# johannesulf/TabCorr

Hardware: AMD Instinct MI355X
Metric: predict_calls_per_sec (higher is better)
Workload: dtype f64; 1 GPU; BASELINE configs[1]: Zheng07 predict(), synthetic auto table 50 mass bins x {cen,sat} (G=100, P=5050), 19 rp bins, n_gauss_prim=10, batch of 10000 draws per GPU per step, draws and results resident in HBM; n_tables=1, gather=none, gather_payload=ngal + xi (160 B per draw), gather_every_steps=32, lanes=4, rccl_ranks=0

## Files before the change

include/tabcorr_amd_testing.h:

```cpp
#ifndef TABCORR_AMD_TESTING_H
#define TABCORR_AMD_TESTING_H

#include "tabcorr_amd.h"

#ifdef __cplusplus
extern "C" {
#endif

int tc_debug_fastmath(int kind, int64_t n, const double* x, double* y);

int tc_debug_central_series(int n_gauss, double log_min, double log_max, double dist_index,
                            int64_t n, const double* log_m_min, const double* sigma,
                            double* series, double* nodes, int32_t* terms);

int tc_debug_satellite_series(int n_gauss, double log_min, double log_max, double dist_index,
                              int64_t n, const double* log_m0, const double* log_m1,
                              const double* alpha, double* series, double* nodes,
                              int32_t* terms);

int tc_plan_debug(int mode, int n_bins, const uint8_t* is_central, int n_chunks,
                  int64_t* n_entries, int32_t* entry_pair, int32_t* entry_chunk,
                  int32_t* entry_class);

int tc_debug_quad_schedule(int n_bins, int n_central, int by_type, int n_tiles, int n_rtiles,
                           int n_tables, int separate, int max_waves, int min_units,
                           int order ,
                           int* n_waves, int* n_runs, int* n_slabs, int64_t* units_min,
                           int64_t* units_max);
int tc_debug_triangle_parts(int n_rb, int n_parts, int32_t* rb0, int32_t* cb0, int32_t* count);
int tc_debug_node_groups(int n_bins, int n_central, const double* log_min,
                         const double* log_max, int32_t* begin, int32_t* member,
                         int* n_groups, int* n_central_groups);
int tc_debug_quad_emulate(int n_bins, int n_r, const double* tpcf_matrix,
                          const uint8_t* is_central, int by_type, int separate,
                          const double* densities, int64_t ldb, int64_t n_draws,
                          int max_waves, int min_units, int order, double* out);

int tc_debug_trace(tc_table* table, uint64_t* out, int64_t capacity, int64_t* n_blocks);
int tc_debug_wave_trace(tc_table* table, uint64_t* out, int64_t capacity,
                        int64_t* n_waves);
int tc_debug_resident_ticks(tc_table* table, uint64_t* out, int64_t capacity, int64_t* n_blocks);
int tc_debug_ensemble_stamps(tc_table* table, uint64_t* out);
#ifdef __cplusplus
}
#endif

#endif
```

tabcorr_amd/_lib.py:

```python

import ctypes
import os

import numpy as np

HERE = os.path.dirname(os.path.abspath(__file__))
LIBRARY = os.path.join(HERE, 'libtabcorr_hip.so')

TC_OK = 0
TC_ERR_INVALID = 1
TC_ERR_HIP = 2
TC_ERR_UNSUPPORTED = 3
TC_ERR_RCCL = 4

MODE = {'auto': 0, 'cross': 1}
DTYPE_F64 = 0
DTYPE_F32 = 1

FLAG_SEPARATE_GAL_TYPE = 1
FLAG_MODULATE_WITH_CENOCC = 2
FLAG_ASSEMBIAS = 4
FLAG_LEAUTHAUD11 = 16

UNIQUE_ID_BYTES = 128

c_double_p = ctypes.POINTER(ctypes.c_double)
c_int_p = ctypes.POINTER(ctypes.c_int)
c_int32_p = ctypes.POINTER(ctypes.c_int32)
c_int64_p = ctypes.POINTER(ctypes.c_int64)
c_uint8_p = ctypes.POINTER(ctypes.c_uint8)
c_float_p = ctypes.POINTER(ctypes.c_float)
c_void_pp = ctypes.POINTER(ctypes.c_void_p)

SIGNATURES = {
    'tc_device_count': [c_int_p],
    'tc_set_device': [ctypes.c_int],
    'tc_get_device': [c_int_p],
    'tc_runtime_version': [c_int_p],
    'tc_device_name': [ctypes.c_char_p, ctypes.c_size_t],
    'tc_device_synchronize': [],
    'tc_device_malloc': [c_void_pp, ctypes.c_size_t],
    'tc_device_free': [ctypes.c_void_p],
    'tc_memcpy_h2d': [ctypes.c_void_p, ctypes.c_void_p, ctypes.c_size_t],
    'tc_memcpy_d2h': [ctypes.c_void_p, ctypes.c_void_p, ctypes.c_size_t],
    'tc_host_alloc': [c_void_pp, ctypes.c_size_t],
    'tc_host_free': [ctypes.c_void_p],
    'tc_host_register': [ctypes.c_void_p, ctypes.c_size_t],
    'tc_host_unregister': [ctypes.c_void_p],
    'tc_host_is_pinned': [ctypes.c_void_p, ctypes.c_size_t, c_int_p],
    'tc_gauss_legendre': [ctypes.c_int, c_double_p, c_double_p],
    'tc_debug_fastmath': [ctypes.c_int, ctypes.c_int64, c_double_p,
                          c_double_p],
    'tc_pair_indices': [ctypes.c_int, c_int32_p, c_int32_p, c_int32_p],
    'tc_spline_interpolation_matrix': [ctypes.c_int, c_double_p, c_double_p],
    'tc_plan_debug': [ctypes.c_int, ctypes.c_int, c_uint8_p, ctypes.c_int,
                      c_int64_p, c_int32_p, c_int32_p, c_int32_p],
    'tc_debug_triangle_parts': [ctypes.c_int, ctypes.c_int, c_int_p, c_int_p, c_int_p],
    'tc_debug_central_series': [ctypes.c_int, ctypes.c_double, ctypes.c_double, ctypes.c_double,
                                ctypes.c_int64, c_double_p, c_double_p, c_double_p, c_double_p,
                                c_int32_p],
    'tc_debug_satellite_series': [ctypes.c_int, ctypes.c_double, ctypes.c_double,
                                  ctypes.c_double, ctypes.c_int64, c_double_p, c_double_p,
                                  c_double_p, c_double_p, c_double_p, c_int32_p],
    'tc_debug_node_groups': [ctypes.c_int, ctypes.c_int, c_double_p, c_double_p,
                             c_int32_p, c_int32_p, c_int_p, c_int_p],
    'tc_debug_quad_schedule': [ctypes.c_int] * 10 + [c_int_p, c_int_p, c_int_p,
                                                     c_int64_p, c_int64_p],
    'tc_debug_quad_emulate': [ctypes.c_int, ctypes.c_int, c_double_p, c_uint8_p,
                              ctypes.c_int, ctypes.c_int, c_double_p,
                              ctypes.c_int64, ctypes.c_int64, ctypes.c_int,
                              ctypes.c_int, ctypes.c_int, c_double_p],
    'tc_table_create': [
        ctypes.c_int, ctypes.c_int, ctypes.c_int, ctypes.c_int64,
        ctypes.c_void_p, ctypes.c_int, c_double_p, c_double_p, c_double_p,
        c_double_p, c_double_p, c_uint8_p, ctypes.c_int, c_void_pp],
    'tc_table_destroy': [ctypes.c_void_p],
    'tc_table_autotune_result': [ctypes.c_void_p, ctypes.c_uint, ctypes.c_int, c_int_p,
                                 c_int64_p, c_int_p, c_float_p],
    'tc_table_batch_invariant': [ctypes.c_void_p, ctypes.c_int, ctypes.c_uint, c_int_p],
    'tc_set_copy_threads': [ctypes.c_int, ctypes.c_int],
    'tc_table_resident_stats': [ctypes.c_void_p, c_int64_p, c_int64_p, c_int64_p, c_int_p],
    'tc_table_synchronize': [ctypes.c_void_p],
    'tc_table_info': [ctypes.c_void_p, c_int_p, c_int_p, c_int_p, c_int64_p,
                      c_int_p, c_int64_p],
    'tc_mean_occupation_zheng07_batch': [
        ctypes.c_void_p, c_double_p, ctypes.c_int, ctypes.c_int64,
        ctypes.c_int, ctypes.c_uint, c_double_p],
    'tc_predict_zheng07_batch': [
        ctypes.c_void_p, c_double_p, ctypes.c_int, ctypes.c_int64,
        ctypes.c_int, ctypes.c_uint, c_double_p, c_double_p],
    'tc_predict_zheng07_batch_device': [
        ctypes.c_void_p, ctypes.c_void_p, ctypes.c_int, ctypes.c_int64,
        ctypes.c_int, ctypes.c_uint, ctypes.c_void_p, ctypes.c_void_p],
    'tc_chi2_zheng07_batch': [
        ctypes.c_void_p, c_double_p, ctypes.c_int, ctypes.c_int64,
        ctypes.c_int, ctypes.c_uint, c_double_p, c_double_p, c_double_p,
        c_double_p],
    'tc_chi2_zheng07_batch_device': [
        ctypes.c_void_p, ctypes.c_void_p, ctypes.c_int, ctypes.c_int64,
        ctypes.c_int, ctypes.c_uint, c_double_p, c_double_p, ctypes.c_void_p,
        ctypes.c_void_p],
    'tc_predict_zheng07_many': [
        ctypes.c_void_p, c_double_p, ctypes.c_int, ctypes.c_int,
        ctypes.c_int, ctypes.c_uint, c_double_p, c_double_p],
    'tc_predict_zheng07_joint': [
        ctypes.POINTER(ctypes.c_void_p), ctypes.c_int, c_double_p, ctypes.c_int,
        ctypes.c_int, ctypes.c_uint, c_double_p, ctypes.POINTER(c_double_p)],
    'tc_predict_zheng07_batch_async': [
        ctypes.c_void_p, c_double_p, ctypes.c_int, ctypes.c_int64,
        ctypes.c_int, ctypes.c_uint, c_double_p, c_double_p, c_int64_p],
    'tc_chi2_zheng07_batch_async': [
        ctypes.c_void_p, c_double_p, ctypes.c_int, ctypes.c_int64,
        ctypes.c_int, ctypes.c_uint, c_double_p, c_double_p, c_double_p,
        c_double_p, c_int64_p],
    'tc_table_wait': [ctypes.c_void_p, ctypes.c_int64],
    'tc_table_query': [ctypes.c_void_p, ctypes.c_int64, c_int_p],
    'tc_interp_predict_zheng07_batch_async': [
        ctypes.c_void_p, c_double_p, ctypes.c_int, c_double_p,
        ctypes.c_int64, ctypes.c_int, ctypes.c_uint, c_double_p, c_double_p,
        c_int64_p],
    'tc_interp_chi2_zheng07_batch_async': [
        ctypes.c_void_p, c_double_p, ctypes.c_int, c_double_p,
        ctypes.c_int64, ctypes.c_int, ctypes.c_uint, c_double_p, c_double_p,
        c_double_p, c_double_p, c_int64_p],
    'tc_interp_wait': [ctypes.c_void_p, ctypes.c_int64],
    'tc_interp_query': [ctypes.c_void_p, ctypes.c_int64, c_int_p],
    'tc_predict_occupation_batch': [
        ctypes.c_void_p, c_double_p, ctypes.c_int64, ctypes.c_uint,
        c_double_p, c_double_p],
    'tc_interp_create': [c_void_pp, ctypes.c_int, ctypes.c_int, c_double_p,
                         c_void_pp],
    'tc_interp_destroy': [ctypes.c_void_p],
    'tc_interp_synchronize': [ctypes.c_void_p],
    'tc_interp_axis': [ctypes.c_void_p, ctypes.c_int, c_int_p, c_double_p,
                       ctypes.c_int],
    'tc_interp_predict_zheng07_batch': [
        ctypes.c_void_p, c_double_p, ctypes.c_int, c_double_p,
        ctypes.c_int64, ctypes.c_int, ctypes.c_uint, c_double_p, c_double_p],
    'tc_interp_predict_zheng07_batch_device': [
        ctypes.c_void_p, ctypes.c_void_p, ctypes.c_int, ctypes.c_void_p,
        ctypes.c_int64, ctypes.c_int, ctypes.c_uint, ctypes.c_void_p,
        ctypes.c_void_p],
    'tc_interp_chi2_zheng07_batch': [
        ctypes.c_void_p, c_double_p, ctypes.c_int, c_double_p,
        ctypes.c_int64, ctypes.c_int, ctypes.c_uint, c_double_p, c_double_p,
        c_double_p, c_double_p],
    'tc_interp_chi2_zheng07_batch_device': [
        ctypes.c_void_p, ctypes.c_void_p, ctypes.c_int, ctypes.c_void_p,
        ctypes.c_int64, ctypes.c_int, ctypes.c_uint, c_double_p, c_double_p,
        ctypes.c_void_p, ctypes.c_void_p],
    'tc_table_set_option': [ctypes.c_void_p, ctypes.c_char_p, ctypes.c_int],
    'tc_table_timer_begin': [ctypes.c_void_p, ctypes.c_int],
    'tc_table_timer_end': [ctypes.c_void_p, c_float_p],
    'tc_table_kernel_time': [ctypes.c_void_p, c_int_p, c_float_p],
    'tc_debug_trace': [ctypes.c_void_p, ctypes.POINTER(ctypes.c_uint64),
                       ctypes.c_int64, c_int64_p],
    'tc_debug_wave_trace': [ctypes.c_void_p, ctypes.POINTER(ctypes.c_uint64),
                            ctypes.c_int64, c_int64_p],
    'tc_debug_resident_ticks': [ctypes.c_void_p, ctypes.POINTER(ctypes.c_uint64),
                                ctypes.c_int64, c_int64_p],
    'tc_debug_ensemble_stamps': [ctypes.c_void_p,
                                 ctypes.POINTER(ctypes.c_uint64)],
    'tc_table_last_launch': [ctypes.c_void_p, c_int_p, c_int_p, c_int_p,
                             c_int_p],
    'tc_pair_count_rppi': [c_double_p, ctypes.c_int64, c_double_p,
                           ctypes.c_int64, c_double_p, c_double_p, ctypes.c_int,
                           ctypes.c_double, ctypes.c_int,
                           ctypes.POINTER(ctypes.c_uint64)],
    'tc_pair_count_smu': [c_double_p, ctypes.c_int64, c_double_p,
                          ctypes.c_int64, c_double_p, c_double_p, ctypes.c_int,
                          ctypes.c_int, ctypes.POINTER(ctypes.c_uint64)],
    'tc_pair_count_rppi_labelled': [c_double_p, c_int32_p, ctypes.c_int64,
                                    c_double_p, c_int32_p, ctypes.c_int64,
                                    ctypes.c_int, c_double_p, c_double_p,
                                    ctypes.c_int, ctypes.c_double,
                                    ctypes.POINTER(ctypes.c_uint64)],
    'tc_pair_count_smu_labelled': [c_double_p, c_int32_p, ctypes.c_int64,
                                   c_double_p, c_int32_p, ctypes.c_int64,
                                   ctypes.c_int, c_double_p, c_double_p,
                                   ctypes.c_int, ctypes.c_int,
                                   ctypes.POINTER(ctypes.c_uint64)],
    'tc_mass_in_cylinders': [c_double_p, ctypes.c_int64, c_double_p,
                             ctypes.c_int64, c_double_p, c_double_p, c_double_p,
                             ctypes.c_int, c_double_p],
    'tc_comm_unique_id': [ctypes.c_void_p],
    'tc_comm_create': [ctypes.c_void_p, ctypes.c_int, ctypes.c_int,
                       c_void_pp],
    'tc_comm_destroy': [ctypes.c_void_p],
    'tc_comm_gather': [ctypes.c_void_p, ctypes.c_void_p, ctypes.c_void_p,
                       ctypes.c_void_p, ctypes.c_int64, ctypes.c_int,
                       ctypes.c_int],
    'tc_comm_release': [ctypes.c_void_p, ctypes.c_void_p, ctypes.c_int],
    'tc_comm_gather_interp': [ctypes.c_void_p, ctypes.c_void_p, ctypes.c_void_p,
                              ctypes.c_void_p, ctypes.c_int64, ctypes.c_int,
                              ctypes.c_int],
    'tc_comm_release_interp': [ctypes.c_void_p, ctypes.c_void_p,
                               ctypes.c_int],
    'tc_comm_barrier': [ctypes.c_void_p],
    'tc_comm_synchronize': [ctypes.c_void_p],
}

_lib = None


class TabCorrHipError(RuntimeError):
    """The HIP backend failed (no device, launch error, RCCL error)."""


def load():
    global _lib
    if _lib is not None:
        return _lib
    library = os.environ.get('TABCORR_AMD_LIBRARY') or LIBRARY
    if not os.path.exists(library):
        raise TabCorrHipError(
            'libtabcorr_hip.so is missing: build it with '
            '`python -m tabcorr_amd.build` (needs hipcc). There is no CPU '
            'fallback.')
    mode = os.RTLD_NOW | os.RTLD_LOCAL | getattr(os, 'RTLD_DEEPBIND', 0)
    lib = ctypes.CDLL(library, mode=mode)
    lib.tc_last_error.restype = ctypes.c_char_p
    lib.tc_last_error.argtypes = []
    for name, argtypes in SIGNATURES.items():
        function = getattr(lib, name)
        function.restype = ctypes.c_int
        function.argtypes = argtypes
    _lib = lib
    return lib


def check(status):
    if status == TC_OK:
        return
    message = load().tc_last_error().decode(errors='replace')
    if status == TC_ERR_INVALID:
        raise ValueError(message)
    if status == TC_ERR_UNSUPPORTED:
        raise NotImplementedError(message)
    raise TabCorrHipError(message)


def as_double_p(array):
    try:
        return ctypes.byref(ctypes.c_double.from_buffer(array))
    except (TypeError, ValueError, BufferError):
        return array.ctypes.data_as(c_double_p)


def device_count():
    lib = load()
    count = ctypes.c_int(0)
    status = lib.tc_device_count(ctypes.byref(count))
    if status != TC_OK:
        return 0
    return count.value


def require_device():
    lib = load()
    count = ctypes.c_int(0)
    check(lib.tc_device_count(ctypes.byref(count)))
    if count.value < 1:
        raise TabCorrHipError('no HIP device found; tabcorr_amd has no CPU '
                              'fallback')
    return count.value


def runtime_version():
    version = ctypes.c_int(0)
    check(load().tc_runtime_version(ctypes.byref(version)))
    return version.value


def device_name():
    buffer = ctypes.create_string_buffer(256)
    check(load().tc_device_name(buffer, 256))
    return buffer.value.decode()


def contiguous(array, dtype=np.float64):
    return np.ascontiguousarray(array, dtype=dtype)
```

tabcorr_amd/csrc/inst_fused.hip:

```cpp
#include "inst_fused.h"

namespace tc {
namespace host {

int launch_fused_instance(const FusedInstance& in, int device, int n_u, dim3 grid, dim3 block,
                       int lds, hipStream_t stream, hipEvent_t k0, hipEvent_t k1,
                       const tc::FusedArgs& fa) {
  const bool assembias = in.assembias, modulate = in.modulate;
  if (in.draws == 40) return launch_fused_instance_40(in, TC_FUSED_ARGS);
  if (in.draws == 32) return launch_fused_instance_32(in, TC_FUSED_ARGS);
  if (in.waves == 16) return launch_fused_instance_16(in, TC_FUSED_ARGS);
#define TC_FUSED(NG, AB, MO, LE) launch_fused<NG, AB, MO, LE, 8>(TC_FUSED_ARGS)
#define TC_FUSED_GROUPED(AB, MO) launch_fused<10, AB, MO, false, 8, 64, true>(TC_FUSED_ARGS)
  if (in.grouped)
    return assembias ? (modulate ? TC_FUSED_GROUPED(true, true) : TC_FUSED_GROUPED(true, false))
                     : (modulate ? TC_FUSED_GROUPED(false, true) : TC_FUSED_GROUPED(false, false));
  if (in.leauthaud) return modulate ? TC_FUSED(0, false, true, true) : TC_FUSED(0, false, false, true);
  if (in.n_gauss != 10) return TC_FUSED(0, false, false, false);
  if (!assembias && !modulate && in.defer == 2)
    return launch_fused<10, false, false, false, 8, 64, false, 2>(TC_FUSED_ARGS);
  if (!assembias && !modulate && in.defer == 1)
    return launch_fused<10, false, false, false, 8, 64, false, 1>(TC_FUSED_ARGS);
  if (!assembias && !modulate) return TC_FUSED(10, false, false, false);
  if (!assembias) return TC_FUSED(10, false, true, false);
  if (!modulate) return TC_FUSED(10, true, false, false);
  return TC_FUSED(10, true, true, false);
#undef TC_FUSED
#undef TC_FUSED_GROUPED
}

}
}
```

tabcorr_amd/csrc/internal.h:

```cpp
#pragma once

#include <hip/hip_runtime.h>
#include <hip/hip_ext.h>

#include <algorithm>
#include <chrono>
#include <cmath>
#include <cstdarg>
#include <cstdio>
#include <cstdlib>
#include <cstring>
#include <map>
#include <memory>
#include <string>
#include <utility>
#include <vector>

#include "../../include/tabcorr_amd.h"
#include "../../include/tabcorr_amd_testing.h"
#include "fastmath.h"
#include "hostmath.h"
#include "kernel_args.h"

namespace tc {
// ... 80 lines not shown
  return fallback;
}
inline size_t stage_limit() {
  static const size_t limit = (size_t)env_int_early("TC_STAGE_LIMIT_MB", 1) << 20;
  return limit;
}

inline size_t zero_copy_limit() {
  static const size_t limit = (size_t)env_int_early("TC_ZERO_COPY_KB", 512) << 10;
  return limit;
}

int create_lane_streams(int count, hipStream_t* streams);

struct SingleWorkspace {
  PinnedBuffer buffer;
  unsigned long long epoch = 0;
  int jobs = 0, blocks = 0;
  size_t partial_offset = 0, theta_offset = 0, done_offset = 0;
  int prepare(int n_jobs, int n_blocks, int rt, int extra_doubles);
  double* ngal() const { return (double*)buffer.ptr; }
  double* partial() const { return (double*)buffer.ptr + partial_offset; }
  double* theta() const { return (double*)buffer.ptr + theta_offset; }
  unsigned long long* done() const {
    return (unsigned long long*)((double*)buffer.ptr + done_offset);
  }
};

template <typename T>
int upload(const std::vector<T>& host, void** device) {
  size_t bytes = std::max<size_t>(1, host.size()) * sizeof(T);
  TC_HIP(hipMalloc(device, bytes));
  if (!host.empty())
    TC_HIP(hipMemcpy(*device, host.data(), host.size() * sizeof(T),
                     hipMemcpyHostToDevice));
  return TC_OK;
}

struct DeviceChunking {
  tc::Chunking host;
  void* chunks = nullptr;
  void* groups = nullptr;
};

struct Quadrature {
  int n_gauss = 0;
  void* log_m = nullptr;
  void* m = nullptr;
  void* weight = nullptr;
  void* group_log_m = nullptr;
  void* group_m = nullptr;
  void* group_weight = nullptr;
  void* series = nullptr;
  void* series_thr = nullptr;
  void* group_series = nullptr;
  void* group_series_thr = nullptr;
  void* sat_series = nullptr;
  void* sat_series_thr = nullptr;
  void* group_sat_series = nullptr;
  void* group_sat_series_thr = nullptr;
  void* cen_records = nullptr;
  void* sat_records = nullptr;
  void* group_records = nullptr;
};

struct DeviceQuadSchedule {
  int n_waves = 0;
  int n_slabs = 0;
  int n_groups = 0;
  int n_runs = 0;
  void* runs = nullptr;
  void* wave_runs = nullptr;
  void* wave_head = nullptr;
  void* group_begin = nullptr;
  void* merge_range = nullptr;
  void* merges = nullptr;
  int lds_bytes = 0;
};

struct QuadTable {
  tc::QuadLayout layout;
  void* d_table = nullptr;
  void* d_comps = nullptr;
  bool finite = false;
  size_t rtile_bytes = 0;
  size_t bytes = 0;
  std::map<std::vector<int64_t>, std::unique_ptr<DeviceQuadSchedule>> schedules;
  void release();
  void drop_schedules();
};

struct CrossFused {
  bool tried = false;
  int rows = 0;
  int n_tables = 0;
  void* d_rows = nullptr;
  void* d_chunk_group = nullptr;
  void* d_chunk_block = nullptr;
  void* d_bin_operand = nullptr;
  std::vector<int32_t> chunk_group_host;
  int n_chunks = 0, n_central_chunks = 0;
  void release() {
    if (d_rows != nullptr) (void)hipFree(d_rows);
    if (d_chunk_group != nullptr) (void)hipFree(d_chunk_group);
    if (d_chunk_block != nullptr) (void)hipFree(d_chunk_block);
    if (d_bin_operand != nullptr) (void)hipFree(d_bin_operand);
    d_rows = d_chunk_group = d_chunk_block = d_bin_operand = nullptr;
    rows = 0;
    tried = false;
  }
};

inline int env_int(const char* name, int fallback) {
#ifdef TC_DEVELOPER_KNOBS
  const char* value = getenv(name);
  if (value == nullptr || *value == 0) return fallback;
  return atoi(value);
#else
  (void)name;
  return fallback;
#endif
}

struct Tuning {
  int lanes = 4;
  int pipeline = 1;
  int single_draw = 1;
  int many_blocks = 256;
  int single_round = 1;
  int poll_done = 1;
  int quad_waves = 0;
  int quad_waves_f32 = 3;
  int quad_merge = 1;
  int quad_order = -1;
  int prio_occ = 2, prio_contract = 1, prio_finalize = 3;
  int finalize_threads = 0;
  int finalize_row_blocks = 0;
  int occ_splits = 0;
  int occ_per_cu = 4;
  int n_groups = 0, n_waves = 0, lds_min = 0, min_chunk_entries = 32;
  int k_splits = 0;
  int trace = 0;
  int autotune_after = 0;
  int sync_chunks = 0;
  int sync_form = 32;
  int sync_stagger = 10;
  int sync_direct_out = 2;
  int async_direct_in = 1;
  int async_direct_out = 2;
  int series = -1;
  int cross_defer = 1;
  int fused_defer = 2;
  int fused_sat_cap = 6;
  int cross_wide_min_draws = 4096;
  int cross_target = 160;
  int resident_aperture = 1;
  int cross_min_draws = 192;
  int fused = 1;
  int fused_min_draws = 0;
  int fused_max_draws = 30720;
  int fused_waves = 0;
  int fused_draws = 0;
  int fused_spread = 1, fused_spread_min = 8192, fused_spread_rounds = 1;
  int prio_fused = 1, prio_fused_occ = 2, prio_fused_out = 3;
  int deterministic = 0;
  int skip_occ = 0, skip_finalize = 0;
  void load() {
    fused = env_int("TC_FUSED", fused);
    fused_min_draws = env_int("TC_FUSED_MIN_DRAWS", fused_min_draws);
    fused_max_draws = env_int("TC_FUSED_MAX_DRAWS", fused_max_draws);
    prio_fused = env_int("TC_PRIO_FUSED", prio_fused);
    prio_fused_occ = env_int("TC_PRIO_FUSED_OCC", prio_fused_occ);
    prio_fused_out = env_int("TC_PRIO_FUSED_OUT", prio_fused_out);
    lanes = env_int("TC_LANES", lanes);
    pipeline = env_int("TC_PIPELINE", pipeline);
    single_draw = env_int("TC_SINGLE_DRAW", single_draw);
    quad_waves = env_int("TC_QUAD_WAVES", quad_waves);
    quad_waves_f32 = env_int("TC_QUAD_WAVES_F32", quad_waves_f32);
    quad_merge = env_int("TC_QUAD_MERGE", quad_merge);
    prio_occ = env_int("TC_PRIO_O", prio_occ);
    prio_contract = env_int("TC_PRIO_C", prio_contract);
    prio_finalize = env_int("TC_PRIO_F", prio_finalize);
    finalize_threads = env_int("TC_FINALIZE_THREADS", finalize_threads);
    finalize_row_blocks = env_int("TC_FINALIZE_ROW_BLOCKS", finalize_row_blocks);
    occ_splits = env_int("TC_OCC_SPLITS", occ_splits);
    occ_per_cu = env_int("TC_OCC_PER_CU", occ_per_cu);
    n_groups = env_int("TC_NGROUPS", n_groups);
    n_waves = env_int("TC_NWAVES", n_waves);
    lds_min = env_int("TC_LDS_MIN", lds_min);
    min_chunk_entries = env_int("TC_MIN_CHUNK_ENTRIES", min_chunk_entries);
    k_splits = env_int("TC_KSPLITS", k_splits);
    trace = env_int("TC_TRACE", trace);
    skip_occ = env_int("TC_SKIP_OCC", skip_occ);
    skip_finalize = env_int("TC_SKIP_FINALIZE", skip_finalize);
  }
};

}
}

struct AutoChoice {
  static constexpr int kSizes = 9;
  static constexpr int64_t size(int i) { return (int64_t)256 << i; }
  int form[kSizes] = {};
  float us[kSizes][3] = {};
  int form_for(int64_t n_draws) const {
    if (n_draws <= size(0)) return form[0];
    if (n_draws >= size(kSizes - 1)) return form[kSizes - 1];
    int i = 0;
    while (size(i + 1) < n_draws) ++i;
    const double w = (double)(n_draws - size(i)) / (double)(size(i + 1) - size(i));
    static const int shape[3] = {0, 64, 32};
    int best = 0;
    double best_us = (1.0 - w) * us[i][0] + w * us[i + 1][0];
    for (int k = 1; k < 3; ++k) {
      if (us[i][k] <= 0.0f || us[i + 1][k] <= 0.0f) continue;
      const double value = (1.0 - w) * us[i][k] + w * us[i + 1][k];
      if (value < (best == 0 ? 0.98 : 1.0) * best_us) {
        best_us = value;
        best = shape[k];
      }
    }
    return best;
  }
};

struct tc_table {
  int device = 0;
  int mode = 0;
  int n_bins = 0;
  int n_r = 0;
  int64_t n_pairs = 0;
  int compute_dtype = TC_DTYPE_F64;
  bool legacy = false;
  tc::Plan plan;
  int rt = 0;
  int n_rtiles = 0;
  hipStream_t stream = nullptr;
  hipEvent_t ev_begin = nullptr, ev_end = nullptr;

  std::vector<double> n_h, log_min, log_max, percentile, dist_index;

  void* d_table = nullptr;
  size_t table_bytes = 0;
  void* d_n_h = nullptr;
  void* d_percentile = nullptr;
  void* d_perm = nullptr;
  tc::NodeGroups node_groups;
  void* d_group_begin = nullptr;
  void* d_group_member = nullptr;
  void* d_group_n_h = nullptr;
  void* d_group_percentile = nullptr;
  bool grouped = false;
  void* d_math_table = nullptr;
  void* d_pos_ij = nullptr;
  void* d_pos_off = nullptr;
  std::vector<double> cross_host;
  tc::host::CrossFused cross_fused, cross_fused_wide;
  int sync_cross_target = 0;
  std::vector<hipEvent_t> chunk_events;
  bool sync_spread = false;
  bool quad = false;
  tc::QuadTiling quad_tiling;
  tc::host::QuadTable quad_by_type, quad_total;
  int n_cus = 256;
  int n_xcds = 8;
  tc::host::Tuning tuning;
  std::map<unsigned, AutoChoice> autotuned;
  std::map<unsigned, int> pipelined_calls;
  bool autotuning = false;
  std::map<int, tc::host::Quadrature> quadrature;
  std::map<std::pair<int, int>, std::unique_ptr<tc::host::DeviceChunking>> chunkings;
  std::map<int64_t, tc::host::DeviceChunking*> choices;

  struct Lane {
    hipStream_t stream = nullptr;
    hipEvent_t finished = nullptr;
    tc::host::DeviceBuffer nbuf, ngal2, partial;
    tc::host::DeviceBuffer nbuf32;
    tc::host::DeviceBuffer xi;
    tc::host::DeviceBuffer in_theta, out;
    tc::host::DeviceBuffer cross_counters;
    int ngal_parts = 1;
  };
  static constexpr int kMaxLanes = 8;
  Lane lanes[kMaxLanes];
  int n_lanes = 2;
  int prev = -1;
  int cur = 0;
  int force_lane = -1;
  int async_lane = -1;
  bool chain = false;
  struct Ticket {
    hipEvent_t done = nullptr;
    int64_t id = -1;
  };
  static constexpr int kMaxTickets = 64;
  Ticket tickets[kMaxTickets];
  int64_t next_ticket = 0;
  const double* fuse_chi2_data = nullptr;
  double* fuse_chi2_out = nullptr;
  bool chi2_fused = false;
  uint64_t device_calls = 0;
  tc::host::DeviceBuffer theta, out_ngal, out_xi, occupation, trace, wave_trace;
  tc::host::DeviceBuffer chi2_data;
  std::vector<double> chi2_host;
  size_t wave_trace_count = 0;
  tc::host::PinnedBuffer h_in, h_out;
  tc::host::SingleWorkspace single_ws;
  struct Resident {
    int enabled = 0;
    int idle_us = 2000;
    int auto_mode = 1;
    int auto_idle_us = 250, auto_gap_us = 300, auto_streak_min = 8, auto_backoff_calls = 4096;
    int auto_streak = 0, auto_backoff = 0, auto_window = 0, auto_relaunches = 0;
    int auto_failures = 0;
    int inject_failures = 0;
    long long auto_last_ns = 0;
    bool auto_serving = false;
    unsigned long long relaunches = 0;
    int running_idle_us = 0;
    int poll_waves = 1;
    bool running = false;
    unsigned long long launch_id = 0;
    hipStream_t stream = nullptr;
    tc::host::PinnedBuffer mailbox;
    tc::host::DeviceBuffer single_aperture;
    bool single_aperture_decided = false;
    tc::host::SingleWorkspace ws;
    int n_theta = 0, n_gauss = 0, blocks = 0;
    unsigned flags = 0;
    bool ensemble = false;
    unsigned long long ens_epoch = 0;
    int ens_grid = 0;
    tc::host::PinnedBuffer ens_mailbox, ens_out;
    tc::host::DeviceBuffer ens_device;
    tc::host::DeviceBuffer ens_aperture;
    unsigned long long ens_host_ns[3] = {0, 0, 0};
    int wait_us = 20000;
    int min_walkers = 24;
    int ens_failures = 0;
    bool ens_disabled = false;
  } resident;
  size_t trace_blocks = 0;
  size_t trace_launches = 0;

  bool profile_kernels = false;
  int profile_every = 1;
  size_t profile_launches = 0;
  std::vector<std::pair<hipEvent_t, hipEvent_t>> kernel_events;
  size_t kernel_events_used = 0;
  int last_workgroups = 0, last_waves = 0, last_splits = 0, last_lds = 0;
};

namespace tc {
namespace host {

constexpr size_t kDirectOutBytes = 256 * 1024;
constexpr size_t kSyncDirectOutBytes = 1024 * 1024;
constexpr int kMaxLdsBytes = 160 * 1024;
constexpr int64_t kMaxSlab = 1 << 18;

int get_quadrature(tc_table* t, int n_gauss, Quadrature** out);
tc::GroupArgs group_args(const tc_table* t, const Quadrature& q);
int get_chunking(tc_table* t, int n_chunks, int waves, DeviceChunking** out);
int lds_bytes_for(const Chunking& chunking, int rt, int elem = 8);
int wave_slots(const tc_table* t, bool interp);
int blocks_per_cu(int lds_bytes, int waves, int slots);
int choose_chunking(tc_table* t, int64_t n_draws, int tables_per_block, DeviceChunking** out,
                    int* lds_bytes);
int launch_contract_rt(int rt, dim3 grid, dim3 block, int lds, hipStream_t stream,
                       const ContractArgs& args, hipEvent_t start = nullptr,
                       hipEvent_t stop = nullptr);
int set_lds_limit_rt(int rt, int lds);
int launch_contract_f32(dim3 grid, dim3 block, int lds, hipStream_t stream,
                        const ContractArgs& args, hipEvent_t start = nullptr,
                        hipEvent_t stop = nullptr);
int run_occupation(tc_table* t, const double* theta_device, int n_theta, int64_t n_draws,
                   int64_t ldb, int n_gauss, unsigned flags, double* occupation_device,
                   DeviceBuffer* nbuf = nullptr, DeviceBuffer* ngal2 = nullptr,
                   hipStream_t stream = nullptr, int* ngal_parts = nullptr,
                   DeviceBuffer* nbuf32 = nullptr);
int run_contraction(tc_table* t, int64_t n_draws, int64_t ldb, unsigned flags,
                    double* ngal_device, double* xi_device);
bool fused_eligible(const tc_table* t, int64_t n_draws, int n_gauss, unsigned flags);
bool batch_invariant_form(tc_table* t, int n_gauss, unsigned flags);
int fused_dens_rows(const tc_table* t, bool separate);
int fused_lds_bytes(const tc_table* t, bool separate, int waves, int draws);
int fused_waves(const tc_table* t, bool separate, unsigned flags);
int series_mask(const tc_table* t);
bool fused_half_tiles(const tc_table* t, bool separate, int64_t n_draws, int n_gauss,
                      unsigned flags);
bool fused_wide_tables(const tc_table* t, bool separate, int n_gauss, unsigned flags);
bool fused_spread_eligible(const tc_table* t, int64_t n_draws, int n_gauss, unsigned flags);
int run_fused(tc_table* t, const double* theta_device, int n_theta, int64_t n_draws, int n_gauss,
              unsigned flags, double* ngal_device, double* xi_device);
int check_predict_args(const tc_table* t, const void* theta, int n_theta, int64_t n_draws,
                       int n_gauss, unsigned flags);
int build_cross_fused(tc_table* const* tables, int n_tables, CrossFused* cf, bool wide = false);
CrossFused* choose_cross_fused(tc_table* const* tables, int n_tables, CrossFused* narrow,
                               CrossFused* wide, int64_t n_draws, unsigned flags, int* status);
bool cross_fused_eligible(const tc_table* t0, const CrossFused& cf, int64_t n_draws, int n_gauss,
                          unsigned flags, bool alone);
int run_cross_fused(tc_table* t0, const CrossFused& cf, const tc::CrossFusedArgs* interp,
                    const double* theta_device, int n_theta, int64_t n_draws, unsigned flags,
                    double* ngal_device, double* xi_device, hipStream_t stream,
                    DeviceBuffer* partial, DeviceBuffer* counters);
int launch_finalize(const FinalizeArgs& args, const Tuning& tuning, hipStream_t stream);
int build_quad_table(tc_table* t, bool by_type, const void* matrix, int matrix_dtype,
                     QuadTable* out);
int get_quad_schedule(tc_table* t, QuadTable* q, int64_t n_tiles, int n_tables, bool separate,
                      DeviceQuadSchedule** out);
int launch_contract_quad(int n_u, bool interp, const QuadArgs& args, int lds_bytes,
                         hipStream_t stream, hipEvent_t start, hipEvent_t stop);
int launch_finalize_quad(const FinalizeQuadArgs& args, const Tuning& tuning, hipStream_t stream,
                         bool f32 = false);
int launch_contract_quad_f32_interp(int n_u, const tc::QuadArgs& args, int lds_bytes,
                                    hipStream_t stream, hipEvent_t start, hipEvent_t stop);
int launch_contract_quad_f32(int n_u, const QuadArgs& args, int lds_bytes, hipStream_t stream,
                             hipEvent_t start, hipEvent_t stop);
hipStream_t interp_stream(tc_interp* interp);
int interp_join_lanes(tc_interp* interp, hipStream_t stream);
int interp_lanes_wait(tc_interp* interp, hipEvent_t event);
int next_kernel_events(tc_table* t, hipEvent_t* start, hipEvent_t* stop);
int64_t max_slab(const tc_table* t);
bool single_draw_eligible(const tc_table* t, int64_t n_draws, int n_gauss, unsigned flags);
constexpr int kSingleMaxBlocks = 64;
constexpr int kSingleMaxWalkers = 64;
inline int64_t many_walkers_limit() {
  static const int64_t limit =
      std::min<int64_t>(kSingleMaxWalkers, env_int_early("TC_MANY_WALKERS", 64));
  return limit;
}
int resident_predict(tc_table* t, const double* theta, int n_theta, int n_gauss, unsigned flags,
                     double* ngal, double* xi);
int resident_post(tc_table* t, const double* theta, int n_theta, int n_gauss, unsigned flags);
int resident_collect(tc_table* t, const double* theta, int n_theta, int n_gauss, unsigned flags,
                     double* ngal, double* xi);
int resident_stop(tc_table* t);
bool resident_eligible(const tc_table* t, int n_gauss);
bool other_resident_running(const tc_table* t);
bool ensemble_eligible(const tc_table* t, int64_t n_walkers, int n_gauss, unsigned flags);
int ensemble_predict(tc_table* t, const double* theta, int n_theta, int n_walkers, int n_gauss,
                     unsigned flags, double* ngal, double* xi);
int launch_single_draw(tc_table* t, const double* theta, int n_theta, int n_walkers, int n_gauss,
                       unsigned flags, SingleWorkspace* ws, hipStream_t stream);
int wait_single_done(SingleWorkspace* ws, hipStream_t stream, bool poll = true);
void combine_single_draw(const tc_table* t, const SingleWorkspace& ws, int walker, double* ngal,
                         double* xi);
int single_draw_blocks(const tc_table* t);
int launch_single_draw_tables(tc_table* t0, const SingleArgs& prepared, int n_tables,
                              int blocks_per_table, hipStream_t stream);
int launch_interp_coef(const InterpArgs& args, hipStream_t stream);
int launch_occ_from_array(tc_table* t, const double* occupation_device, int64_t n_draws,
                          int64_t ldb, double* nbuf, double* ngal2, hipStream_t stream);
int launch_chi2(const double* xi, int64_t n_draws, int n_r, const double* data,
                const double* precision, double* chi2, hipStream_t stream);

int launch_occupation(const tc::OccArgs& oa, unsigned flags, int n_gauss, bool grouped,
                      int64_t grid_blocks, hipStream_t stream);
int launch_occ_from_array_kernel(const double* occupation_device, int64_t n_draws, int64_t ldb,
                                 int n_bins, int n_central, const double* n_h,
                                 const int32_t* perm, double* nbuf, double* ngal2, float* nbuf32,
                                 hipStream_t stream);
struct FusedInstance {
  int n_gauss = 10;
  bool assembias = false, modulate = false, leauthaud = false, grouped = false;
  int waves = 8, draws = 64;
  int defer = 0;
};
int launch_fused_instance(const FusedInstance& instance, int device, int n_u, dim3 grid,
                          dim3 block, int lds, hipStream_t stream, hipEvent_t k0, hipEvent_t k1,
                          const tc::FusedArgs& fa);
int launch_cross_instance(bool assembias, bool modulate, bool defer, int device, int rows,
                          dim3 grid, dim3 block, int lds, hipStream_t stream, hipEvent_t k0,
                          hipEvent_t k1, const tc::CrossFusedArgs& ca);
int launch_single_kernel(int blocks, hipStream_t stream, const tc::SingleArgs& sa);
int launch_resident_kernel(int blocks, hipStream_t stream, const tc::SingleArgs& sa);
int launch_ensemble_kernel(int device, int grid, int lds_bytes, hipStream_t stream,
                           const tc::EnsembleArgs& ea);

int copy_in(PinnedBuffer* stage, void* device, const void* host, size_t bytes,
            hipStream_t stream);
int copy_out(PinnedBuffer* stage, double* ngal, size_t ngal_count, const void* d_ngal,
             double* xi, size_t xi_count, const void* d_xi, hipStream_t stream);

}
}
```

tabcorr_amd/csrc/kernel_args.h:

```cpp
#pragma once

#include <cstdint>

#include "hostmath.h"

namespace tc {

constexpr int kLanes = 64;
constexpr unsigned kFlagSeparate = 1u;
constexpr unsigned kFlagModulate = 2u;
constexpr unsigned kFlagAssembias = 4u;
constexpr int kOccWaves = 4;
constexpr int kF32Block = 8;
constexpr int kF64Block = 8;
constexpr int kF32Tile = 32;
constexpr int kFinalizeRows = 32;
constexpr int kMaxInterpDim = 8;
constexpr int kMaxInterpAxis = 32;

struct GroupArgs {
  const int32_t* begin;
  const int32_t* member;
  const double* log_m;
  const double* m;
// ... 107 lines not shown
  int dens_stride;
  double* dens;
  unsigned long long* flag_a;
  double* partial;
  unsigned long long* flag_b;
  unsigned long long* callword;
  const unsigned long long* mailbox;
  int direct;
  double* out;
  unsigned long long* done;
  unsigned long long* exited;
  unsigned long long epoch;
  unsigned long long launch_id;
  unsigned long long idle_ticks, life_ticks, call_ticks;
  int lds_area, lds_dens, lds_t, lds_ij;
  int skip;
};
constexpr int kEnsembleThreads = 512;
constexpr int kEnsembleMaxWalkers = 256;
constexpr int kEnsembleDensPad = 65;

struct ContractArgs {
  const double* nbuf;
  int64_t ldb;
  const void* table;
  int64_t n_positions;
  const Chunk* chunks;
  const Group* groups;
  int mode;
  int n_central;
  int r_stride;
  int n_tiles;
  int xcd_map;
  int n_slabs;
  const int32_t* pos_ij;
  const int32_t* pos_off;
  unsigned long long* trace;
  unsigned long long* wave_trace;
  double* partial;
  int n_tables;
  int k_splits;
  const double* const* tables;
  const double* const* nbufs;
  const int32_t* table_class;
  const double* coef;
};

constexpr int kQuadMaxU = 5;
constexpr int kQuadTile = 32;
constexpr int kQuadWavesPerBlock = 4;

struct QuadCompArgs {
  int32_t triangular;
  int32_t i_bin0;
  int32_t j_bin0;
  int32_t n_cb;
  uint32_t unit_base;
  int32_t pad[3];
};

constexpr int kQuadTileF32 = 64;
constexpr int kQuadMaxUF32 = 4;

struct QuadArgs {
  const float* nbuf32;
  const double* nbuf;
  const double* const* nbufs;
  const float* const* nbufs32;
  int64_t ldb;
  int n_bins;
  const void* table;
  const double* const* tables;
  const int32_t* table_class;
  const double* coef;
  uint32_t rtile_bytes;
  const QuadRun* runs;
  const QuadCompArgs* comps;
  const int32_t* wave_runs;
  const int32_t* wave_head;
  int n_waves;
  int priority;
  void* partial;
  const int32_t* merge_range;
  const int32_t* merges;
  unsigned long long* stamps;
};

struct FinalizeQuadArgs {
  const void* partial;
  const int32_t* group_begin;
  const double* ngal_part;
  int n_ngal_parts;
  int n_rtiles;
  int r_per_tile;
  int rt;
  int groups_per_rtile;
  int n_comp;
  int n_r;
  int mode;
  int priority;
  int64_t ldb;
  int64_t n_draws;
  double* ngal;
  double* xi;
  const double* chi2_data;
  double* chi2;
};

constexpr int kFusedWaves = 8;
constexpr int kFusedMaxParts = 8;

struct FusedArgs {
  const double* theta;
  int n_theta;
  int n_bins;
  int n_central;
  int n_gauss;
  int dens_rows;
  int part_rb0[kFusedMaxParts];
  int part_cb0[kFusedMaxParts];
  int part_count[kFusedMaxParts];
  int part_triangular[kFusedMaxParts];
  int part_n_cb[kFusedMaxParts];
  int part_i_row0[kFusedMaxParts];
  int part_j_row0[kFusedMaxParts];
  int part_unit_base[kFusedMaxParts];
  int separate;
  int n_r;
  int priority;
  int64_t n_draws;
  const double* log_m;
  const double* m;
  const double* weight;
  const double* n_h;
  const double* percentile;
  double split;
  const double* math_table;
  const void* table;
  uint32_t table_bytes;
  double* ngal;
  double* xi;
  const double* chi2_data;
  double* chi2;
  int n_groups;
  int n_central_groups;
  GroupArgs group;
  const double* series;
  const int32_t* series_thr;
  const double* sat_series;
  const int32_t* sat_series_thr;
  int sat_cap;
  const double* sat_records;
  const double* cen_records;
};

constexpr int kCrossWaves = 8;
constexpr int kCrossChunkBins = 48;
constexpr int kCrossMaxRows = 128;
constexpr int kCrossTableDoubles = 2306;
constexpr int kCrossSmallRows = 16, kCrossSmallChunk = 8;
constexpr int kCrossMaxSplits = 8;
constexpr int cross_small_lds_doubles(int n_comp) {
  return kCrossTableDoubles + kCrossWaves * kCrossSmallChunk * kLanes +
         n_comp * kCrossSmallRows * kLanes;
}
constexpr int cross_buffer_doubles(int rows) {
  return 2 * kCrossChunkBins * kLanes > rows * kLanes ? 2 * kCrossChunkBins * kLanes
                                                      : rows * kLanes;
}

struct CrossFusedArgs {
  const double* theta;
  int n_theta;
  int64_t n_draws;
  int n_bins;
  int n_groups, n_central_groups;
  GroupArgs group;
  const double* math_table;
  const double* rows;
  const int32_t* chunk_block;
  int defer;
  int lds_bitmap, lds_list;
  const int32_t* bin_operand;
  const int32_t* chunk_group;
  int n_chunks, n_central_chunks;
  int n_tables;
  int n_r;
  int separate;
  int row_stride;
  int cen_waves;
  int n_splits;
  int split_all[kCrossMaxSplits + 1], split_cen[kCrossMaxSplits + 1],
      split_sat[kCrossMaxSplits + 1];
  double* partial;
  int* counters;
  int lds_res0;
  int lds_tile;
  int interp;
  int n_dim;
  int n_axis[kMaxInterpDim];
  int axis_offset[kMaxInterpDim];
  int a_offset[kMaxInterpDim];
  const double* xp;
  const double* a;
  const int32_t* table_node;
  const double* x;
  double split;
  int priority;
  double* ngal;
  double* xi;
  const double* chi2_data;
  double* chi2;
};

struct FinalizeArgs {
  const double* partial;
  const Group* groups;
  const double* ngal_part;
  int n_ngal_parts;
  int n_groups;
  int k_splits;
  int n_comp;
  int r_stride;
  int n_r;
  int mode;
  int64_t ldb;
  int64_t n_draws;
  double* ngal;
  double* xi;
};

struct InterpArgs {
  int n_dim;
  int n_tables;
  int n_classes;
  int mode;
  int separate;
  int n_axis[kMaxInterpDim];
  int axis_offset[kMaxInterpDim];
  int a_offset[kMaxInterpDim];
  const double* xp;
  const double* a;
  const int32_t* table_node;
  const int32_t* table_class;
  const double* x;
  const double* const* ngal_parts;
  int n_ngal_parts;
  int64_t ldb;
  int64_t n_draws;
  double* coef;
  double* ngal;
};

}
```

tabcorr_amd/csrc/kernels.hip.h:

```cpp
#pragma once

#include <hip/hip_runtime.h>

#include <cstdint>
#include <utility>

#include "fastmath.h"
#include "hostmath.h"
#include "kernel_args.h"
#include "series.h"

#ifdef TC_DEVELOPER_KNOBS
#define TC_TRACE(pointer) ((pointer) != nullptr)
#else
#define TC_TRACE(pointer) false
#endif

namespace tc {

static_assert(sizeof(QuadRun) == 32 && sizeof(QuadCompArgs) == 32, "read as 8 x int32");

typedef const __attribute__((address_space(4))) double* sc_f64;
typedef const __attribute__((address_space(4))) float* sc_f32;
typedef const __attribute__((address_space(4))) int32_t* sc_i32;
// ... 1669 lines not shown
          for (int v = 0; v < 4; ++v) F[u][s] = fmaf(D[u][s][v], e[v][s], F[u][s]);
      ++rb;
      cb = 0;
    }
    if (slab != -1) {
      float* out = slab >= 0
                       ? (float*)a.partial + ((int64_t)slab * (4 * U) + kq) * kQuadTileF32 + 4 * c
                       : stage32 + ((-2 - slab) * (4 * U) + kq) * kQuadTileF32 + 4 * c;
#pragma unroll
      for (int u = 0; u < U; ++u) {
        const f32x4 value = {F[u][0], F[u][1], F[u][2], F[u][3]};
        *(f32x4*)(out + (4 * u) * kQuadTileF32) = value;
#pragma unroll
        for (int s = 0; s < 4; ++s) F[u][s] = 0.0f;
      }
    }
  }
  sc_i32 merge_range = (sc_i32)a.merge_range;
  const int merge_begin = merge_range[2 * blockIdx.x], merge_end = merge_range[2 * blockIdx.x + 1];
  if (merge_begin == merge_end) return;
  __syncthreads();
  sc_i32 merges = (sc_i32)a.merges;
  for (int e = merge_begin + wave_in_block; e < merge_end; e += kQuadWavesPerBlock) {
    const int slab = merges[4 * e], first = merges[4 * e + 1], n_slots = merges[4 * e + 2];
    float* out = (float*)a.partial + ((int64_t)slab * (4 * U) + kq) * kQuadTileF32 + 4 * c;
    const float* in = stage32 + (first * (4 * U) + kq) * kQuadTileF32 + 4 * c;
#pragma unroll
    for (int u = 0; u < U; ++u) {
      f32x4 sum = *(const f32x4*)(in + (4 * u) * kQuadTileF32);
      for (int s = 1; s < n_slots; ++s)
        sum += *(const f32x4*)(in + (s * (4 * U) + 4 * u) * kQuadTileF32);
      *(f32x4*)(out + (4 * u) * kQuadTileF32) = sum;
    }
  }
}

template <typename P, int TILE>
__global__ __launch_bounds__(1024) void finalize_quad_kernel(FinalizeQuadArgs a) {
  __shared__ double tile[kFinalizeRows][kLanes + 1];
  __shared__ double part_sum[16][kLanes];
  __shared__ double norm_inv[kLanes];
  __shared__ double chi2_lds[kFinalizeRows * (kFinalizeRows + 1)];
  set_priority(a.priority);
  if (a.chi2 != nullptr) {
    const int count = a.n_r * (a.n_r + 1);
    for (int idx = threadIdx.x; idx < count; idx += blockDim.x) chi2_lds[idx] = a.chi2_data[idx];
  }
  const int lane = threadIdx.x & 63;
  const int wave = __builtin_amdgcn_readfirstlane(threadIdx.x >> 6);
  const int64_t col = (int64_t)blockIdx.x * kLanes;
  const int64_t n_valid = a.n_draws - col < kLanes ? a.n_draws - col : kLanes;

  if (wave == 0 && a.ngal_part == nullptr) norm_inv[lane] = 1.0;
  if (wave == 0 && a.ngal_part != nullptr) {
    double n_cen = 0.0, n_sat = 0.0;
    for (int p = 0; p < a.n_ngal_parts; ++p) {
      n_cen += a.ngal_part[((int64_t)p * 2 + 0) * a.ldb + col + lane];
      n_sat += a.ngal_part[((int64_t)p * 2 + 1) * a.ldb + col + lane];
    }
    const double total = n_cen + n_sat;
    norm_inv[lane] = a.mode == 0 ? total * total : total;
    if (lane < n_valid && blockIdx.y == 0) {
      if (a.n_comp == 1) {
        a.ngal[col + lane] = total;
      } else {
        a.ngal[2 * (col + lane)] = n_cen;
        a.ngal[2 * (col + lane) + 1] = n_sat;
      }
    }
  }
  __syncthreads();
  const double norm = norm_inv[lane];
  const bool poisoned = a.n_comp > 1 && !(fabs(norm) <= 1.79769313486231570815e308);
  auto normalise = [&](double sum) { return poisoned ? __builtin_nan("") : sum / norm; };

  const int n_rows = a.n_comp * a.n_r;
  const int n_waves = blockDim.x >> 6;
  const int rows_per_block = (n_rows + gridDim.y - 1) / gridDim.y;
  const int row_begin = blockIdx.y * rows_per_block;
  const int row_end = row_begin + rows_per_block < n_rows ? row_begin + rows_per_block : n_rows;
  const int64_t tile32 = TILE == 32 ? (int64_t)blockIdx.x * 2 + (lane >> 5) : (int64_t)blockIdx.x;
  const int64_t slab_stride = (int64_t)a.rt * TILE;
  auto sum_slabs = [&](int row, int part, int parts) {
    const int comp = row / a.n_r, r = row % a.n_r;
    const int rtile = r / a.r_per_tile, r_local = r % a.r_per_tile;
    const int64_t group = (tile32 * a.n_rtiles + rtile) * a.groups_per_rtile +
                          (a.groups_per_rtile > 1 ? comp : 0);
    const int first = a.group_begin[group], count = a.group_begin[group + 1] - first;
    const int begin = first + (int)((int64_t)count * part / parts);
    const int end = first + (int)((int64_t)count * (part + 1) / parts);
    const P* src = (const P*)a.partial + ((int64_t)begin * a.rt + r_local) * TILE + (lane & (TILE - 1));
    double sum = 0.0;
    for (int s0 = begin; s0 < end; s0 += 8) {
      double v[8];
#pragma unroll
      for (int u = 0; u < 8; ++u)
        v[u] = s0 + u < end ? (double)src[(s0 - begin + u) * slab_stride] : 0.0;
#pragma unroll
      for (int u = 0; u < 8; ++u) sum += v[u];
    }
    return sum;
  };
  for (int row0 = row_begin; row0 < row_end; row0 += kFinalizeRows) {
    const int rows = row_end - row0 < kFinalizeRows ? row_end - row0 : kFinalizeRows;
    if (rows * 2 <= n_waves) {
      const int parts = n_waves / rows;
      const int rr = wave / parts, part = wave % parts;
      if (rr < rows) part_sum[wave][lane] = sum_slabs(row0 + rr, part, parts);
      __syncthreads();
      if (wave < rows) {
        double sum = 0.0;
        for (int p = 0; p < parts; ++p) sum += part_sum[wave * parts + p][lane];
        tile[wave][lane] = normalise(sum);
      }
    } else {
      for (int rr = wave; rr < rows; rr += n_waves)
        tile[rr][lane] = normalise(sum_slabs(row0 + rr, 0, 1));
    }
    __syncthreads();
    if (a.chi2 != nullptr) {
      const double* data = chi2_lds;
      const double* matrix = chi2_lds + rows;
      double part = 0.0;
      for (int i = wave; i < rows; i += n_waves) {
        double inner = 0.0;
        for (int j = 0; j < rows; ++j)
          inner = fma(matrix[i * rows + j], tile[j][lane] - data[j], inner);
        part = fma(tile[i][lane] - data[i], inner, part);
      }
      part_sum[wave][lane] = part;
      __syncthreads();
      if (wave == 0 && lane < n_valid) {
        double total = 0.0;
        for (int w = 0; w < n_waves; ++w) total += part_sum[w][lane];
        a.chi2[col + lane] = total;
      }
      __syncthreads();
      continue;
    }
    for (int idx = threadIdx.x; idx < rows * kLanes; idx += blockDim.x) {
      const int d = idx / rows, rr = idx % rows;
      if (d < n_valid) a.xi[(col + d) * (int64_t)n_rows + row0 + rr] = tile[rr][d];
    }
    __syncthreads();
  }
}

constexpr int fused_slot_doubles(int waves, int draws = 64) {
  return waves * 4 * kQuadMaxU * (draws == 40 ? 40 : kQuadTile);
}
__device__ __forceinline__ constexpr int dens40(int row, int draw) {
  return row * 40 + (draw & 3) * 10 + (draw >> 2);
}
constexpr int fused_scratch_doubles(int waves) { return fm::kTableDoubles + 2 * waves * kLanes; }
static_assert(kFusedWaves == 8 && kFusedMaxParts == 8, "8 or 16 waves: 4 or 8 parts per tile");
static_assert(20 * (kLanes + 1) + 20 * 21 <= fm::kTableDoubles,
              "results tile + likelihood data in the place of the math table");

template <int UU, int DL>
__device__ __forceinline__ void fused_quad_pass(__amdgpu_buffer_rsrc_t rs_t, unsigned off_a,
                                                unsigned unit_bytes, const double* dens_b,
                                                const double* dens_e, int rb, int cb, int left,
                                                bool triangular, int n_cb, unsigned unit_base,
                                                double (&F)[2][2]) {
  unsigned ua = (unit_base + (unsigned)(triangular ? rb * (rb + 1) / 2 + cb : rb * n_cb + cb)) *
                unit_bytes;
  f64x2 t0, t1, b0, b1;
  f64x4 D[UU][2];
  auto fetch = [&](f64x2& t, f64x2& b, int column) {
    t = buffer_load16<0>(rs_t, off_a, ua);
    b = *(const f64x2*)(dens_b + 4 * column * DL);
    ua += unit_bytes;
  };
  auto mma = [&](const f64x2& t, const f64x2& b, bool first) {
    if (first) {
      const f64x4 zero = {0.0, 0.0, 0.0, 0.0};
#pragma unroll
      for (int u = 0; u < UU; ++u) {
        const double av = u ? t.y : t.x;
        D[u][0] = __builtin_amdgcn_mfma_f64_16x16x4f64(av, b.x, zero, 0, 0, 0);
        D[u][1] = __builtin_amdgcn_mfma_f64_16x16x4f64(av, b.y, zero, 0, 0, 0);
      }
    } else {
#pragma unroll
      for (int u = 0; u < UU; ++u) {
        const double av = u ? t.y : t.x;
        D[u][0] = __builtin_amdgcn_mfma_f64_16x16x4f64(av, b.x, D[u][0], 0, 0, 0);
        D[u][1] = __builtin_amdgcn_mfma_f64_16x16x4f64(av, b.y, D[u][1], 0, 0, 0);
      }
    }
  };
  fetch(t0, b0, cb);
  while (left > 0) {
    const int row_length = triangular ? rb + 1 : n_cb;
    const int n = row_length - cb < left ? row_length - cb : left;
    left -= n;
    f64x2 e[4];
#pragma unroll
    for (int v = 0; v < 4; ++v) e[v] = *(const f64x2*)(dens_e + (4 * rb + v) * DL);
    fetch(t1, b1, n > 1 ? cb + 1 : 0);
    __builtin_amdgcn_sched_barrier(0);
    mma(t0, b0, true);
    __builtin_amdgcn_sched_barrier(0);
    int t = 1;
    for (; t + 1 < n; t += 2) {
      fetch(t0, b0, cb + t + 1);
      __builtin_amdgcn_sched_barrier(0);
      mma(t1, b1, false);
      __builtin_amdgcn_sched_barrier(0);
      fetch(t1, b1, t + 2 < n ? cb + t + 2 : 0);
      __builtin_amdgcn_sched_barrier(0);
      mma(t0, b0, false);
      __builtin_amdgcn_sched_barrier(0);
    }
    if (t < n) {
      fetch(t0, b0, 0);
      __builtin_amdgcn_sched_barrier(0);
      mma(t1, b1, false);
      __builtin_amdgcn_sched_barrier(0);
    } else {
      t0 = t1;
      b0 = b1;
    }
#pragma unroll
    for (int u = 0; u < UU; ++u)
#pragma unroll
      for (int v = 0; v < 4; ++v) {
        F[u][0] = fma(D[u][0][v], e[v].x, F[u][0]);
        F[u][1] = fma(D[u][1][v], e[v].y, F[u][1]);
      }
    ++rb;
    cb = 0;
  }
}

__device__ __forceinline__ int wave_prefix_sum(int value) {
  auto shifted = [](int x, auto control, auto rows) {
    return __builtin_amdgcn_update_dpp(0, x, decltype(control)::value, decltype(rows)::value, 0xf,
                                       false);
  };
  typedef std::integral_constant<int, 0xf> all_rows;
  value += shifted(value, std::integral_constant<int, 0x111>(), all_rows());
  value += shifted(value, std::integral_constant<int, 0x112>(), all_rows());
  value += shifted(value, std::integral_constant<int, 0x114>(), all_rows());
  value += shifted(value, std::integral_constant<int, 0x118>(), all_rows());
  value += shifted(value, std::integral_constant<int, 0x142>(), std::integral_constant<int, 0xa>());
  value += shifted(value, std::integral_constant<int, 0x143>(), std::integral_constant<int, 0xc>());
  return value;
}

__device__ __forceinline__ double fused_quad_rows40(double select, double value, double sums) {
  return __builtin_amdgcn_mfma_f64_4x4x4f64(select, value, sums, 0, 0, 0);
}

template <int S0, int NS>
__device__ __forceinline__ void fused_quad_pass40(__amdgpu_buffer_rsrc_t rs_t, unsigned off_a,
                                                  unsigned unit_bytes, const double* dens_b,
                                                  const double* dens_e, int rb, int cb, int left,
                                                  bool triangular, int n_cb, unsigned unit_base,
                                                  double (&F)[NS][10]) {
  unsigned ua = (unit_base + (unsigned)(triangular ? rb * (rb + 1) / 2 + cb : rb * n_cb + cb)) *
                unit_bytes;
  double ta[2][NS];
  f64x2 tb[2][5];
  double D[NS][10];
  auto fetch = [&](int set, int column) {
#pragma unroll
    for (int s = 0; s < NS; ++s) {
      constexpr int kPairBytes = 1024;
      const int sub = S0 + s;
      const bool first_of_pair = (sub & 1) == 0 && s + 1 < NS;
      const bool second_of_pair = (sub & 1) == 1 && s >= 1;
      if (first_of_pair) {
        const f64x2 word = __builtin_bit_cast(
            f64x2, __builtin_amdgcn_raw_buffer_load_b128(rs_t, off_a + (sub / 2) * kPairBytes, ua,
                                                         0));
        ta[set][s] = word.x;
        ta[set][s + 1 < NS ? s + 1 : s] = word.y;
      } else if (!second_of_pair) {
        ta[set][s] = __builtin_bit_cast(
            double, __builtin_amdgcn_raw_buffer_load_b64(
                        rs_t, off_a + (sub / 2) * kPairBytes + (sub & 1) * 8, ua, 0));
      }
    }
#pragma unroll
    for (int q = 0; q < 5; ++q) tb[set][q] = *(const f64x2*)(dens_b + 4 * column * 40 + 2 * q);
    ua += unit_bytes;
  };
  auto mma = [&](int set, bool first) {
    if (first) {
#pragma unroll
      for (int q = 0; q < 5; ++q)
#pragma unroll
        for (int s = 0; s < NS; ++s) {
          const double av = ta[set][s];
          D[s][2 * q] = __builtin_amdgcn_mfma_f64_4x4x4f64(av, tb[set][q].x, 0.0, 0, 0, 0);
          D[s][2 * q + 1] = __builtin_amdgcn_mfma_f64_4x4x4f64(av, tb[set][q].y, 0.0, 0, 0, 0);
        }
    } else {
#pragma unroll
      for (int q = 0; q < 5; ++q)
#pragma unroll
        for (int s = 0; s < NS; ++s) {
          const double av = ta[set][s];
          D[s][2 * q] = __builtin_amdgcn_mfma_f64_4x4x4f64(av, tb[set][q].x, D[s][2 * q], 0, 0, 0);
          D[s][2 * q + 1] =
              __builtin_amdgcn_mfma_f64_4x4x4f64(av, tb[set][q].y, D[s][2 * q + 1], 0, 0, 0);
        }
    }
  };
  fetch(0, cb);
  while (left > 0) {
    const int row_length = triangular ? rb + 1 : n_cb;
    const int n = row_length - cb < left ? row_length - cb : left;
    left -= n;
    f64x2 e[5];
#pragma unroll
    for (int q = 0; q < 5; ++q) e[q] = *(const f64x2*)(dens_e + 4 * rb * 40 + 2 * q);
    int t = 0;
    if (n > 1) {
      fetch(1, cb + 1);
      mma(0, true);
      fetch(0, 2 < n ? cb + 2 : 0);
      mma(1, false);
      t = 2;
    }
    for (; t + 1 < n; t += 2) {
      fetch(1, cb + t + 1);
      mma(0, false);
      fetch(0, t + 2 < n ? cb + t + 2 : 0);
      mma(1, false);
    }
    if (t < n) {
      fetch(1, 0);
      if (t == 0) mma(0, true); else mma(0, false);
#pragma unroll
      for (int s = 0; s < NS; ++s) ta[0][s] = ta[1][s];
#pragma unroll
      for (int q = 0; q < 5; ++q) tb[0][q] = tb[1][q];
    }
#pragma unroll
    for (int q = 0; q < 5; ++q)
#pragma unroll
      for (int s = 0; s < NS; ++s) {
        F[s][2 * q] = fma(D[s][2 * q], e[q].x, F[s][2 * q]);
        F[s][2 * q + 1] = fma(D[s][2 * q + 1], e[q].y, F[s][2 * q + 1]);
      }
    ++rb;
    cb = 0;
  }
}

template <int NGAUSS, int U, bool ASSEMBIAS, bool MODULATE, bool LEAUTHAUD = false,
          int W = kFusedWaves, int DL = 64, bool GROUPED = false, int SATDEFER = 0>
__global__ __launch_bounds__(64 * W, DL == 40 ? 2 : W == 8 ? (SATDEFER == 2 ? 4 : 2) : 1) void predict_fused_kernel(
    FusedArgs a) {
  static_assert(!SATDEFER || (NGAUSS == 10 && !ASSEMBIAS && !MODULATE && !LEAUTHAUD && DL != 32 &&
                              !GROUPED), "deferred pairs");
  static_assert(!GROUPED || (NGAUSS == 10 && !LEAUTHAUD), "groups of bins: Zheng07, ten nodes");
  static_assert((DL == 64 && (W == 8 || W == 16)) || ((DL == 32 || DL == 40) && W == 8),
                "workgroup shape");
  static_assert(DL == 64 || NGAUSS == 10 || LEAUTHAUD, "32 / 40 draws: ten nodes per bin");
  static_assert(DL != 40 || (!ASSEMBIAS && !MODULATE && !LEAUTHAUD && !GROUPED), "latency form");
  constexpr int PARTS = DL == 40 ? W : W * 32 / DL;
  static_assert(!LEAUTHAUD || (NGAUSS == 0 && !ASSEMBIAS), "Leauthaud11: any n_gauss, undecorated");
  constexpr int UP = (U + 1) / 2;
  extern __shared__ __attribute__((aligned(16))) double fused_lds[];
  constexpr int kSlotDoubles = fused_slot_doubles(W, DL);
  const int region_b = a.dens_rows * DL > kSlotDoubles ? a.dens_rows * DL : kSlotDoubles;
  double* dens = fused_lds;
  double* table = fused_lds + region_b;
  double(*red)[W][kLanes] = (double(*)[W][kLanes])(table + fm::kTableDoubles);
  const fm::Consts kc = fm::make_consts();
#ifdef TC_DEVELOPER_KNOBS
  const int skip = (a.priority >> 8) & 3;
  const int n_bins_occ = (skip & 1) ? 0 : a.n_bins;
  unsigned long long* const stamps =
      ((a.priority >> 10) & 1) && a.chi2 == nullptr ? (unsigned long long*)a.chi2_data : nullptr;
  auto wave_stamp = [&](int which) {
    if (stamps != nullptr && (threadIdx.x & 63) == 0 && W == 8 && ((threadIdx.x >> 6) & 3) == 0)
      stamps[blockIdx.x * 32 + 16 + 8 * (threadIdx.x >> 8) + which] =
          __builtin_amdgcn_s_memrealtime();
  };
  auto stamp = [&](int which) {
    if (stamps != nullptr && threadIdx.x == 0)
      stamps[blockIdx.x * 32 + which] = __builtin_amdgcn_s_memrealtime();
  };
  if (skip & 1)
    for (int idx = threadIdx.x; idx < a.n_bins * DL; idx += blockDim.x) fused_lds[idx] = 1e-3;
#else
  constexpr int skip = 0;
  const int n_bins_occ = a.n_bins;
  auto stamp = [](int) {};
  auto wave_stamp = [](int) {};
#endif
  stamp(0);
  set_priority((a.priority >> 2) & 3);
  const int lane = threadIdx.x & 63;
  const int wave = __builtin_amdgcn_readfirstlane(threadIdx.x >> 6);
  const int n_gauss = NGAUSS > 0 ? NGAUSS : a.n_gauss;
  {
    typedef double __attribute__((ext_vector_type(2))) double2v;
    const int hi = fm::kTableDoubles / 2;
    const double2v* src = (const double2v*)a.math_table;
    double2v* dst = (double2v*)table;
    for (int i = threadIdx.x; i < hi; i += blockDim.x) dst[i] = src[i];
  }
  for (int idx = a.n_bins * DL + threadIdx.x; idx < a.dens_rows * DL; idx += blockDim.x)
    dens[idx] = 0.0;
  __syncthreads();
  stamp(1);

  const int draw = DL != 32 ? lane : (lane & 31);
  const int half = DL != 32 ? 0 : (lane >> 5);
  const bool live = DL != 40 || lane < 40;
  auto dens_at = [&](int row, int d) -> double& {
    return dens[DL == 40 ? dens40(row, d) : row * DL + d];
  };
  const int64_t col = (int64_t)blockIdx.x * DL;
  const int64_t b0 = col + draw;
  const int64_t b = b0 < a.n_draws ? b0 : a.n_draws - 1;
  double norm;
  {
    const double* th = a.theta + b * a.n_theta;
    LeauthaudDraw ld;
    if (LEAUTHAUD) ld = prepare_leauthaud(table, kc, th);
    const DrawSetup d =
        LEAUTHAUD ? prepare_draw(table, kc, 12.0, 1.0, 12.0, 13.0, 1.0, 0.0, 0.0)
                  : prepare_draw(table, kc, th[0], th[1], th[2], th[3], th[4],
                                 ASSEMBIAS ? th[5] : 0.0, ASSEMBIAS ? th[6] : 0.0);
    DrawParams dp;
    dp.log_m_min = d.log_m_min;
    dp.inv_sigma = d.inv_sigma;
    dp.m0 = d.m0;
    dp.log2_m1 = d.log2_m1;
    dp.sat_scale = d.sat_scale;
    dp.alpha = d.alpha;
    dp.a_cen = d.a_cen;
    dp.a_sat = d.a_sat;
    dp.bad = d.bad;
    dp.any_bad = __builtin_amdgcn_ballot_w64(dp.bad != 0) != 0;
    series_setup<MODULATE>(dp, (GROUPED ? a.group.series : a.series) != nullptr && DL != 32,
                           (GROUPED ? a.group.sat_series : a.sat_series) != nullptr && DL != 32);
    sc_f64 log_m = (sc_f64)a.log_m;
    sc_f64 mass = (sc_f64)a.m;
    sc_f64 weight = (sc_f64)a.weight;
    sc_f64 weight_sum = weight + a.n_bins * n_gauss;
    sc_f64 n_h = (sc_f64)a.n_h;
    sc_f64 percentile = (sc_f64)a.percentile;
    const double f1 = (1.0 - a.split) / a.split, f2 = a.split / (1.0 - a.split);
    double sum_cen = 0.0, sum_sat = 0.0;
    stamp(2);
    if (GROUPED) {
      sc_i32 group_begin = (sc_i32)a.group.begin;
      sc_f64 n_h_m = (sc_f64)a.group.n_h;
      const GroupConsts gq{(sc_f64)a.group.log_m, (sc_f64)a.group.m, (sc_f64)a.group.weight,
                           (sc_f64)a.group.weight + a.n_bins * 10, (sc_f64)a.group.percentile,
                           (sc_i32)a.group.member,
                             SeriesConsts{(sc_f64)a.group.series, (sc_i32)a.group.series_thr,
                                          (sc_f64)a.group.sat_series, (sc_i32)a.group.sat_series_thr}};
      for (int gr = wave; gr < a.n_groups; gr += W) {
        const bool central = gr < a.n_central_groups;
        auto emit = [&](int mi, int g, double acc) {
          const double value = acc * n_h_m[mi];
          if (half == 0) dens[g * DL + draw] = value;
          if (central) sum_cen += value; else sum_sat += value;
        };
        if (DL == 32)
          occ_group_zheng07_halves<ASSEMBIAS, MODULATE>(
              table, kc, gr, group_begin[gr], group_begin[gr + 1], central, half, a.group.log_m,
              a.group.m, a.group.weight, gq, a.split, dp, emit);
        else
          occ_group_zheng07<ASSEMBIAS, MODULATE>(table, kc, gr, group_begin[gr],
                                                 group_begin[gr + 1], central, gq, a.split, dp,
                                                 emit);
      }
    }
    unsigned mine = 0;
    for (int g = wave; g < (GROUPED ? 0 : n_bins_occ); g += W) {
      const bool central = g < a.n_central;
      const bool above = ASSEMBIAS ? percentile[g] > a.split : false;
      bool deferred = false;
      const double acc =
          SATDEFER == 2 && central
              ? occ_cen_record(table, kc,
                               (sc_f64)a.cen_records + g * series::cen_record::kStride, dp,
                               &deferred) :
          SATDEFER && !central && (SATDEFER == 2 || a.sat_cap == series::sat::kShortest)
              ? occ_sat_record(table, kc,
                               (sc_f64)a.sat_records + g * series::sat_record::kStride, dp,
                               &deferred) :
          DL == 32 && LEAUTHAUD
              ? occ_bin_leauthaud11_halves<MODULATE>(table, kc, g, central, half, a.log_m, a.m,
                                                     a.weight, ld)
          : DL == 32  ? occ_bin_zheng07_halves<ASSEMBIAS, MODULATE>(table, kc, g, central, above,
                                                                    half, a.log_m, a.m, a.weight,
                                                                    log_m, weight_sum, dp)
          : LEAUTHAUD ? occ_bin_leauthaud11<MODULATE>(table, kc, g, n_gauss, central, log_m, mass,
                                                      weight, ld)
                      : occ_bin_zheng07<NGAUSS, ASSEMBIAS, MODULATE>(
                            table, kc, g, n_gauss, central, above, log_m, mass, weight,
                            weight_sum, dp, f1, f2,
                            SeriesConsts{(sc_f64)a.series, (sc_i32)a.series_thr, (sc_f64)a.sat_series,
                              (sc_i32)a.sat_series_thr,
                              SATDEFER ? a.sat_cap : series::sat::kSteps - 1},
                            SATDEFER ? &deferred : nullptr);
      if (SATDEFER && deferred && live) mine |= 1u << ((g - wave) / W);
      const double value = acc * n_h[g];
      if (half == 0 && live) dens_at(g, draw) = value;
      if (central) sum_cen += value; else sum_sat += value;
    }
    wave_stamp(0);
    if (SATDEFER) {
      unsigned* list = (unsigned*)&red[1][wave][0];
      const int count = __builtin_popcount(mine);
      const int inclusive = wave_prefix_sum(count);
      const int total = __builtin_amdgcn_readlane(inclusive, 63);
      wave_stamp(2);
      for (int base = 0; base < total; base += 64) {
        {
          unsigned left = mine;
          int position = inclusive - count - base;
          while (__builtin_amdgcn_ballot_w64(left != 0) != 0) {
            if (left != 0) {
              const int j = __builtin_ctz(left);
              left &= left - 1;
              if (position >= 0 && position < 64) list[position] = ((unsigned)j << 6) | (unsigned)lane;
              ++position;
            }
          }
        }
        wave_stamp(3);
        const int n = total - base < 64 ? total - base : 64;
        const bool active = lane < n;
        const unsigned entry = list[active ? lane : 0];
        const int g = wave + W * (int)(entry >> 6), from = (int)(entry & 63);
        const double m0 = __shfl(dp.m0, from, 64);
        const double log2_m1 = __shfl(dp.log2_m1, from, 64);
        const double sat_scale = __shfl(dp.sat_scale, from, 64);
        const double alpha = __shfl(dp.alpha, from, 64);
        const int bad = __shfl(dp.bad, from, 64);
        double acc = 0.0;
        const bool cen_pair = SATDEFER == 2 && g < a.n_central;
        if (SATDEFER == 2 && __builtin_amdgcn_ballot_w64(active && cen_pair) != 0) {
          const double log_m_min = __shfl(dp.log_m_min, from, 64);
          const double inv_sigma = __shfl(dp.inv_sigma, from, 64);
          double sum = 0.0;
          bool tie = false;
#pragma unroll 1
          for (int k0 = 0; k0 < 10; k0 += 5) {
            double node[5], w[5];
#pragma unroll
            for (int k = 0; k < 5; ++k) {
              node[k] = a.log_m[g * 10 + k0 + k];
              w[k] = a.weight[g * 10 + k0 + k];
            }
#pragma unroll
            for (int k = 0; k < 5; ++k) {
              sum = fma(w[k], fm::erf_fast(table, kc, (node[k] - log_m_min) * inv_sigma), sum);
              tie = tie || node[k] == log_m_min;
            }
          }
          sum = fma(0.5, sum, 0.5 * a.weight[a.n_bins * 10 + g]);
          if ((bad & kBadCen) || ((bad & kTieCen) && tie)) sum = __builtin_nan("");
          if (cen_pair) acc = sum;
        }
        if (SATDEFER != 2 || __builtin_amdgcn_ballot_w64(active && !cen_pair) != 0) {
        double sat = 0.0;
#pragma unroll 1
        for (int k0 = 0; k0 < 10; k0 += 5) {
          double node[5], w[5];
#pragma unroll
          for (int k = 0; k < 5; ++k) {
            node[k] = a.m[g * 10 + k0 + k];
            w[k] = a.weight[g * 10 + k0 + k];
          }
#pragma unroll
          for (int k = 0; k < 5; ++k) {
            const double x = node[k] - m0;
            sat = fma(w[k],
                      fm::exp2_fast(table, kc,
                                    alpha * fm::log2_fast_offset(
                                                table, kc, x > 1e-300 ? x : 1e-300, log2_m1),
                                    x > 0.0),
                      sat);
          }
        }
        sat *= sat_scale;
        if (bad != 0) {
          if ((bad & kInfSat) && sat != 0.0) sat = __builtin_huge_val();
          if ((bad & kBadSat) && sat != 0.0) sat = __builtin_nan("");
        }
        if (!cen_pair) acc = sat;
        }
        if (active) dens_at(g, from) = acc * a.n_h[g];
        wave_stamp(4);
      }
      for (unsigned left = mine; __builtin_amdgcn_ballot_w64(left != 0) != 0;) {
        if (left != 0) {
          const int j = __builtin_ctz(left);
          left &= left - 1;
          const double value = dens_at(wave + W * j, draw);
          if (SATDEFER == 2 && wave + W * j < a.n_central) sum_cen += value;
          else sum_sat += value;
        }
      }
    }
    wave_stamp(1);
    stamp(3);
    red[0][wave][lane] = sum_cen;
    red[1][wave][lane] = sum_sat;
    __syncthreads();
    stamp(4);
    double n_cen = 0.0, n_sat = 0.0;
#pragma unroll
    for (int w = 0; w < W; ++w) {
      n_cen += red[0][w][lane];
      n_sat += red[1][w][lane];
    }
    const double total = (skip & 1) ? 1.0 : n_cen + n_sat;
    norm = total * total;
    if (wave == 0 && half == 0 && live && b0 < a.n_draws) {
      if (a.separate) {
        a.ngal[2 * b0] = n_cen;
        a.ngal[2 * b0 + 1] = n_sat;
      } else {
        a.ngal[b0] = total;
      }
    }
  }

  set_priority(a.priority & 3);
  const int c = lane & 15, kq = lane >> 4;
  double F[UP][2][2];
  constexpr int UA = DL == 40 ? (U > 3 ? 3 : U) : 1, UB = DL == 40 && U > 3 ? U - 3 : 1;
  double F40a[UA][10], F40b[UB][10];
  if (DL == 40) {
    const int part = wave;
    const unsigned off_a = ((lane & 0x30) | ((lane & 3) << 2) | ((lane >> 2) & 3)) * 16;
    const double* dens_b = dens + (a.part_j_row0[part] + (lane >> 4)) * 40 + (lane & 3) * 10;
    const double* dens_e = dens + (a.part_i_row0[part] + (lane >> 4)) * 40 + (lane & 3) * 10;
    const __amdgpu_buffer_rsrc_t rs_t =
        __builtin_amdgcn_make_buffer_rsrc((void*)a.table, 0, a.table_bytes, kBufferFlags);
    const int rb = a.part_rb0[part], cb = a.part_cb0[part], count = a.part_count[part];
    const bool triangular = a.part_triangular[part] != 0;
    const int n_cb = a.part_n_cb[part];
    const unsigned unit_base = (unsigned)a.part_unit_base[part];
#pragma unroll
    for (int s = 0; s < UA; ++s)
#pragma unroll
      for (int g = 0; g < 10; ++g) F40a[s][g] = 0.0;
#pragma unroll
    for (int s = 0; s < UB; ++s)
#pragma unroll
      for (int g = 0; g < 10; ++g) F40b[s][g] = 0.0;
#ifdef TC_DEVELOPER_KNOBS
    const unsigned unit_bytes = ((a.priority >> 12) & 1) ? 0u : UP * 1024u;
    const unsigned first_unit = ((a.priority >> 12) & 1) ? 0u : unit_base;
#else
    constexpr unsigned unit_bytes = UP * 1024u;
    const unsigned first_unit = unit_base;
#endif
    if (!(skip & 2))
    fused_quad_pass40<0, UA>(rs_t, off_a, unit_bytes, dens_b, dens_e, rb, cb, count, triangular,
                             n_cb, first_unit, F40a);
    if (U > 3 && !(skip & 2))
      fused_quad_pass40<(U > 3 ? 3 : 0), UB>(rs_t, off_a, unit_bytes, dens_b, dens_e, rb, cb,
                                             count, triangular, n_cb, first_unit, F40b);
  } else {
    const int sub = wave / PARTS, part = wave % PARTS;
    const unsigned off_a = lane * 16;
    const double* dens_b =
        dens + (a.part_j_row0[part] + kq) * DL + sub * kQuadTile + 2 * c;
    const double* dens_e = dens + a.part_i_row0[part] * DL + sub * kQuadTile + 2 * c;
    const __amdgpu_buffer_rsrc_t rs_t =
        __builtin_amdgcn_make_buffer_rsrc((void*)a.table, 0, a.table_bytes, kBufferFlags);
    const int rb = a.part_rb0[part], cb = a.part_cb0[part], count = a.part_count[part];
    const bool triangular = a.part_triangular[part] != 0;
    const int n_cb = a.part_n_cb[part];
    const unsigned unit_base = (unsigned)a.part_unit_base[part];
#pragma unroll
    for (int p = 0; p < UP; ++p) {
      F[p][0][0] = F[p][0][1] = F[p][1][0] = F[p][1][1] = 0.0;
      if (skip & 2) continue;
      if (2 * p + 1 < U)
        fused_quad_pass<2, DL>(rs_t, off_a + p * 1024, UP * 1024, dens_b, dens_e, rb, cb, count,
                               triangular, n_cb, unit_base, F[p]);
      else
        fused_quad_pass<1, DL>(rs_t, off_a + p * 1024, UP * 1024, dens_b, dens_e, rb, cb, count,
                               triangular, n_cb, unit_base, F[p]);
    }
  }
  stamp(5);
  __syncthreads();
  stamp(8);
  if (DL == 40) {
    const int q = lane >> 4;
    auto share = [&](int sub, int g) {
      return sub < UA ? F40a[sub < UA ? sub : 0][g] : F40b[sub >= UA ? sub - UA : 0][g];
    };
    double* out = dens + (wave * (4 * U) + ((lane >> 2) & 3)) * 40 + (lane & 3);
    if (((a.priority >> 11) & 1) && __builtin_amdgcn_ballot_w64(!(norm < 1e280)) == 0) {
      double select[4];
#pragma unroll
      for (int m = 0; m < 4; ++m) select[m] = (lane & 3) == m ? 1.0 : 0.0;
#pragma unroll
      for (int sub = 0; sub < U; ++sub)
#pragma unroll
        for (int t = 0; t < 3; ++t) {
          double sums = 0.0;
#pragma unroll
          for (int m = 0; m < (t < 2 ? 4 : 2); ++m)
            sums = fused_quad_rows40(select[m], share(sub, 4 * t + m), sums);
          if (t < 2 || q < 2) out[(4 * sub) * 40 + 16 * t + 4 * q] = sums;
        }
    } else {
#pragma unroll
      for (int sub = 0; sub < U; ++sub)
#pragma unroll
        for (int g = 0; g < 10; ++g) {
          const double sum = fused_quad_rows40(1.0, share(sub, g), 0.0);
          if (q == 0) out[(4 * sub) * 40 + 4 * g] = sum;
        }
    }
  } else {
    double* out = dens + (wave * (4 * U) + kq) * kQuadTile + 2 * c;
#pragma unroll
    for (int u = 0; u < U; ++u) {
      const f64x2 value = {F[u >> 1][u & 1][0], F[u >> 1][u & 1][1]};
      *(f64x2*)(out + (4 * u) * kQuadTile) = value;
    }
  }
  stamp(9);
  set_priority((a.priority >> 4) & 3);
  double(*tile)[kLanes + 1] = (double(*)[kLanes + 1])table;
  if (a.separate) {
    const bool poisoned = !(fabs(norm) <= 1.79769313486231570815e308);
    const int64_t n_valid = a.n_draws - col < DL ? a.n_draws - col : DL;
    const int sub = lane >> 5, d = lane & 31;
    for (int comp = 0; comp < 3; ++comp) {
      __syncthreads();
      constexpr int Q = PARTS / 4;
      const int p_begin = comp == 0 ? 0 : comp == 1 ? Q : 3 * Q;
      const int p_count = comp == 1 ? 2 * Q : Q;
      for (int rr = wave; rr < a.n_r && lane < DL; rr += W) {
        const double* first = dens + ((PARTS * sub + p_begin) * (4 * U) + rr) * kQuadTile + d;
        double sum = first[0];
        for (int p = 1; p < p_count; ++p) sum += first[p * (4 * U) * kQuadTile];
        tile[rr][lane] = poisoned ? __builtin_nan("") : sum / norm;
      }
      __syncthreads();
      for (int idx = threadIdx.x; idx < a.n_r * DL; idx += blockDim.x) {
        const int dd = idx / a.n_r, rr = idx % a.n_r;
        if (dd < n_valid) a.xi[((col + dd) * 3 + comp) * (int64_t)a.n_r + rr] = tile[rr][dd];
      }
    }
    return;
  }
  double* chi2_lds = table + 20 * (kLanes + 1);
  if (a.chi2 != nullptr) {
    const int count = a.n_r * (a.n_r + 1);
    for (int idx = threadIdx.x; idx < count; idx += blockDim.x) chi2_lds[idx] = a.chi2_data[idx];
  }
  __syncthreads();
  stamp(10);
  if (DL == 40) {
    for (int rr = wave; rr < a.n_r && lane < DL; rr += W) {
      const double* first = dens + rr * 40 + lane;
      double sum = first[0];
#pragma unroll
      for (int part = 1; part < W; ++part) sum += first[part * (4 * U) * 40];
      tile[rr][lane] = sum / norm;
    }
  } else {
    const int sub = lane >> 5, d = lane & 31;
    for (int rr = wave; rr < a.n_r && lane < DL; rr += W) {
      const double* first = dens + ((PARTS * sub) * (4 * U) + rr) * kQuadTile + d;
      double sum = first[0];
#pragma unroll
      for (int part = 1; part < PARTS; ++part) sum += first[part * (4 * U) * kQuadTile];
      tile[rr][lane] = sum / norm;
    }
  }
  __syncthreads();
  stamp(6);
  const int64_t n_valid = a.n_draws - col < DL ? a.n_draws - col : DL;
  if (a.chi2 != nullptr) {
    const int rows = a.n_r;
    const double* data = chi2_lds;
    const double* matrix = chi2_lds + rows;
    double part = 0.0;
    for (int i = wave; i < rows; i += W) {
      double inner = 0.0;
      for (int j = 0; j < rows; ++j)
        inner = fma(matrix[i * rows + j], tile[j][lane] - data[j], inner);
      part = fma(tile[i][lane] - data[i], inner, part);
    }
    red[0][wave][lane] = part;
    __syncthreads();
    if (wave == 0 && lane < n_valid) {
      double total = 0.0;
      for (int w = 0; w < W; ++w) total += red[0][w][lane];
      a.chi2[col + lane] = total;
    }
    return;
  }
  for (int idx = threadIdx.x; idx < a.n_r * DL; idx += blockDim.x) {
    const int d = idx / a.n_r, rr = idx % a.n_r;
    if (d < n_valid) a.xi[(col + d) * (int64_t)a.n_r + rr] = tile[rr][d];
  }
  stamp(7);
}

template <int ROW_LANES, typename Coefficient>
__device__ __forceinline__ void cross_deferred_pairs(
    const CrossFusedArgs& a, const double* table, const fm::Consts& kc, const DrawParams& dp,
    const unsigned long long* bitmap, unsigned* list, int wave, int lane, int g_first, int g_last,
    int type, Coefficient&& coefficient, double* res) {
  constexpr int SHARES = 64 / ROW_LANES;
  constexpr int SLOTS = 8 / SHARES;
  const int row = lane % ROW_LANES, share = lane / ROW_LANES;
  const unsigned long long owner = 0x0101010101010101ull << wave;
  double extra[SLOTS];
#pragma unroll
  for (int slot = 0; slot < SLOTS; ++slot) extra[slot] = 0.0;
  auto evaluate = [&](int total) {
#ifdef TC_DEVELOPER_KNOBS
    if (((a.priority >> 10) & 1) && a.chi2 == nullptr && lane == 0) {
      atomicAdd((unsigned long long*)a.chi2_data + blockIdx.x * 16 + 12, (unsigned long long)total);
      atomicAdd((unsigned long long*)a.chi2_data + blockIdx.x * 16 + 13,
                (unsigned long long)((total + 63) / 64));
    }
#endif
    for (int e0 = 0; e0 < total; e0 += 64) {
      const int n = total - e0 < 64 ? total - e0 : 64;
      const bool active = lane < n;
      const unsigned entry = list[e0 + (active ? lane : 0)];
      const int g = (int)(entry >> 6), draw = (int)(entry & 63);
      const bool central = g < a.n_central_groups;
      const int m_begin = a.group.begin[g], m_end = a.group.begin[g + 1];
      const double log_m_min = __shfl(dp.log_m_min, draw, 64);
      const double inv_sigma = __shfl(dp.inv_sigma, draw, 64);
      const double m0 = __shfl(dp.m0, draw, 64);
      const double log2_m1 = __shfl(dp.log2_m1, draw, 64);
      const double sat_scale = __shfl(dp.sat_scale, draw, 64);
      const double alpha = __shfl(dp.alpha, draw, 64);
      const int bad = __shfl(dp.bad, draw, 64);
      for (int t = 0; __builtin_amdgcn_ballot_w64(active && m_begin + t < m_end) != 0; ++t) {
        const int mi = m_begin + t;
        const bool valid = active && mi < m_end && (type < 0 || central == (type == 0));
        const int mi_safe = valid ? mi : m_begin;
        const double* weight = a.group.weight + (int64_t)mi_safe * 10;
        double acc = 0.0;
        bool tie = false;
#pragma unroll 1
        for (int k0 = 0; k0 < 10; k0 += 5) {
          double node[5], w[5];
#pragma unroll
          for (int k = 0; k < 5; ++k) {
            node[k] = central ? a.group.log_m[g * 10 + k0 + k] : a.group.m[g * 10 + k0 + k];
            w[k] = weight[k0 + k];
          }
#pragma unroll
          for (int k = 0; k < 5; ++k) {
            double value;
            if (central) {
              value = fm::erf_fast(table, kc, (node[k] - log_m_min) * inv_sigma);
              tie = tie || node[k] == log_m_min;
            } else {
              const double x = node[k] - m0;
              value = fm::exp2_fast(
                  table, kc,
                  alpha * fm::log2_fast_offset(table, kc, x > 1e-300 ? x : 1e-300, log2_m1),
                  x > 0.0);
            }
            acc = fma(w[k], value, acc);
          }
        }
        const bool cen_nan = (bad & kBadCen) || ((bad & kTieCen) && tie);
        if (central) acc = fma(0.5, acc, 0.5 * a.group.weight[(int64_t)a.n_bins * 10 + mi_safe]);
        else acc *= sat_scale;
        if (bad != 0) {
          if (!central && (bad & kInfSat) && acc != 0.0) acc = __builtin_huge_val();
          if (central ? cen_nan : ((bad & kBadSat) && acc != 0.0)) acc = __builtin_nan("");
        }
        const double nbar_lane = valid ? acc : 0.0;
        for (int p0 = 0; p0 < n; p0 += 8) {
          double c[8];
#pragma unroll
          for (int u = 0; u < 8; ++u)
            c[u] = coefficient(__builtin_amdgcn_readlane(mi_safe, (p0 + u) & 63), row);
#pragma unroll
          for (int u = 0; u < 8; ++u) {
            if (p0 + u >= n) break;
            const double nbar = readlane_f64(nbar_lane, (p0 + u) & 63);
            const int j = __builtin_amdgcn_readlane(draw, (p0 + u) & 63) >> 3;
            const double mine = share == j % SHARES ? nbar : 0.0;
            const int slot_of_pair = j / SHARES;
            switch (slot_of_pair) {
#define TC_SLOT(K)                                                     \
  case K:                                                              \
    if constexpr (K < SLOTS) extra[K < SLOTS ? K : 0] = fma(c[u], mine, extra[K < SLOTS ? K : 0]); \
    break;
              TC_SLOT(0) TC_SLOT(1) TC_SLOT(2) TC_SLOT(3) TC_SLOT(4) TC_SLOT(5) TC_SLOT(6) TC_SLOT(7)
#undef TC_SLOT
              default: break;
            }
          }
        }
      }
    }
  };
  int gb = g_first;
  while (gb < g_last) {
    int filled = 0;
    for (; gb < g_last; gb += 64) {
      const int g_lane = gb + lane;
      unsigned long long word = g_lane < g_last ? bitmap[g_lane] & owner : 0ull;
      if (__builtin_amdgcn_ballot_w64(word != 0) == 0) continue;
      const int count = __builtin_popcountll(word);
      const int inclusive = wave_prefix_sum(count);
      const int total = __builtin_amdgcn_readlane(inclusive, 63);
      if (filled + total > 512) break;
      int slot_out = filled + inclusive - count;
      while (word != 0) {
        list[slot_out++] = (unsigned)(g_lane << 6) | (unsigned)__builtin_ctzll(word);
        word &= word - 1;
      }
      filled += total;
    }
    evaluate(filled);
  }
#pragma unroll
  for (int slot = 0; slot < SLOTS; ++slot)
    res[row * kLanes + wave + 8 * (share + SHARES * slot)] += extra[slot];
}

template <int RW, bool ASSEMBIAS, bool MODULATE, bool DEFER = false>
__global__ __launch_bounds__(64 * kCrossWaves, RW <= 8 ? 4 : 2) void predict_cross_fused_kernel(
    CrossFusedArgs a) {
  constexpr int W = kCrossWaves, ROWS = W * RW;
  constexpr int NT = ROWS / 16;
  constexpr int N_RB = RW >= 16 ? 2 : 1;
  constexpr int N_DB = RW >= 8 ? 2 : 1;
  constexpr int PF = 6;
  static_assert(ROWS <= kCrossMaxRows && fm::kTableDoubles == kCrossTableDoubles, "kernel_args.h");
  static_assert(N_RB * N_DB * 4 == RW && kCrossChunkBins % 4 == 0, "tiles per wave");
  extern __shared__ __attribute__((aligned(16))) double cross_lds[];
  double* table = cross_lds;
  double* buffers = cross_lds + kCrossTableDoubles;
  const fm::Consts kc = fm::make_consts();
#ifdef TC_DEVELOPER_KNOBS
  unsigned long long* const stamps =
      ((a.priority >> 10) & 1) && a.chi2 == nullptr ? (unsigned long long*)a.chi2_data : nullptr;
  auto stamp = [&](int which) {
    if (stamps != nullptr && threadIdx.x == 0)
      stamps[blockIdx.x * 16 + which] = __builtin_amdgcn_s_memrealtime();
  };
  unsigned long long ticks_a = 0, ticks_wait = 0, ticks_b = 0, lap_from = 0;
  auto lap = [&](unsigned long long& into) {
    if (stamps != nullptr) {
      const unsigned long long now = __builtin_amdgcn_s_memrealtime();
// ... 1679 lines not shown
```

tabcorr_amd/csrc/launch.hip:

```cpp
#include <immintrin.h>

#include <atomic>
#include <mutex>

#include "internal.h"
#include "kernels.hip.h"
#include "series.h"

namespace tc {
namespace host {

int get_quadrature(tc_table* t, int n_gauss, Quadrature** out) {
  auto it = t->quadrature.find(n_gauss);
  if (it != t->quadrature.end()) {
    *out = &it->second;
    return TC_OK;
  }
  std::vector<double> x, w;
  tc::gauss_legendre(n_gauss, x, w);
  const int g = t->n_bins;
  std::vector<double> log_m((size_t)g * n_gauss), m((size_t)g * n_gauss),
      weight((size_t)g * n_gauss + g);
  for (int i = 0; i < g; ++i) {
    const double d_log = t->log_max[i] - t->log_min[i];
// ... 755 lines not shown
  if (t->tuning.fused == 0) return false;
  const bool tuned_flags = n_gauss == 10 && t->tuning.fused == 1 &&
                           t->tuning.fused_min_draws == 0 && t->autotuned.count(flags) != 0;
  const bool invariant = t->tuning.deterministic >= 2;
  if (n_draws > t->tuning.fused_max_draws && t->async_lane < 0 && !tuned_flags && !invariant)
    return false;
  if (!t->quad || t->compute_dtype != TC_DTYPE_F64 || t->quad_total.d_table == nullptr)
    return false;
  if (t->quad_tiling.n_rtiles != 1 || t->n_r > 20 || t->chain || t->tuning.trace) return false;
  const bool leauthaud = (flags & TC_FLAG_LEAUTHAUD11) != 0;
  const bool separate = (flags & TC_FLAG_SEPARATE_GAL_TYPE) != 0;
  if (separate) {
    const tc::QuadLayout& layout = t->quad_by_type.layout;
    if (t->quad_by_type.d_table == nullptr || layout.comps.size() != 3 ||
        t->fuse_chi2_out != nullptr)
      return false;
    for (const tc::QuadComp& comp : layout.comps)
      if (comp.n_units <= 0) return false;
  }
  if (!leauthaud && (flags & (TC_FLAG_ASSEMBIAS | TC_FLAG_MODULATE_WITH_CENOCC)) && n_gauss != 10)
    return false;
  if (t->quad_total.layout.comps.size() != 1 || !t->quad_total.layout.comps[0].triangular)
    return false;
  if (!invariant && fused_spread_eligible(t, n_draws, n_gauss, flags)) return true;
  const bool wide = fused_wide_tables(t, separate, n_gauss, flags);
  if (n_gauss < 1 || (!wide && fused_waves(t, separate, flags) == 0)) return false;
  if (invariant) return true;
  if (n_gauss == 10 && t->tuning.fused == 1 && t->tuning.fused_min_draws == 0) {
    auto tuned = t->autotuned.find(flags);
    const bool alone = t->force_lane >= 0 || !t->tuning.pipeline || t->n_lanes == 1;
    if (tuned != t->autotuned.end() && !alone) return tuned->second.form_for(n_draws) != 0;
  }
  const bool alone = t->force_lane >= 0 || !t->tuning.pipeline || t->n_lanes == 1;
  {
    const tc::QuadLayout& layout = separate ? t->quad_by_type.layout : t->quad_total.layout;
    const double estimate = (5.0 + 10.0 * (t->n_bins / 100.0) * (n_gauss / 10.0) +
                             60.0 * ((double)layout.n_units / 325.0) * (t->quad_tiling.n_u / 5.0)) *
                            8.0 / (wide ? 16 : fused_waves(t, separate, flags));
    if (leauthaud && (flags & TC_FLAG_MODULATE_WITH_CENOCC) && t->tuning.fused < 2) return false;
    const int64_t min_draws = t->tuning.fused_min_draws > 0 ? t->tuning.fused_min_draws
                              : wide                        ? 15 * (int64_t)t->n_bins
                              : leauthaud && fused_half_tiles(t, separate, n_draws, n_gauss, flags)
                                  ? 3000
                              : fused_half_tiles(t, separate, n_draws, n_gauss, flags)
                                  ? (estimate <= 50.0 ? 256 : 12 * (int64_t)t->n_bins)
                              : leauthaud                   ? 8192
                              : estimate <= 28.0            ? 512
                                                            : (int64_t)(90.0 * estimate);
    if (alone && t->tuning.fused < 2) {
      if (leauthaud) return false;
      if (n_draws < 2048) return false;
      const double three = 22.0 + 0.0044 * (double)n_draws * estimate / 75.0;
      if (n_draws <= (int64_t)32 * t->n_cus && t->tuning.fused_draws == 0 && !wide &&
          fused_half_tiles(t, separate, n_draws, n_gauss, flags))
        return 0.56 * estimate < three;
      if (n_draws > (int64_t)40 * t->n_cus && n_draws <= (int64_t)64 * t->n_cus && !wide &&
          t->tuning.fused_draws == 0 && fused_waves(t, separate, flags) == 8)
        return 0.95 * estimate < three;
      return false;
    }
    if (n_draws < min_draws) return false;
  }
  return true;
}

bool batch_invariant_form(tc_table* t, int n_gauss, unsigned flags) {
  if (t->tuning.deterministic < 2) return false;
  if (t->mode == TC_MODE_CROSS && !t->cross_host.empty() && t->tuning.fused != 0) {
    int status = TC_OK;
    tc_table* self = t;
    const CrossFused& cf =
        *choose_cross_fused(&self, 1, &t->cross_fused, &t->cross_fused_wide, 1, flags, &status);
    return status == TC_OK && cross_fused_eligible(t, cf, 1, n_gauss, flags, true);
  }
  return fused_eligible(t, 1, n_gauss, flags);
}

int fused_dens_rows(const tc_table* t, bool separate) {
  if (!separate) return 4 * t->quad_total.layout.comps[0].n_rb;
  int rows = 0;
  for (const tc::QuadComp& comp : t->quad_by_type.layout.comps)
    rows = std::max(rows, std::max(comp.i_bin0 + 4 * comp.n_rb, comp.j_bin0 + 4 * comp.n_cb));
  return (rows + 3) / 4 * 4;
}

int fused_lds_bytes(const tc_table* t, bool separate, int waves, int draws) {
  const int dens_rows = fused_dens_rows(t, separate);
  return (std::max(dens_rows * draws, tc::fused_slot_doubles(waves, draws)) +
          tc::fused_scratch_doubles(waves)) * 8;
}

bool fused_spread_eligible(const tc_table* t, int64_t n_draws, int n_gauss, unsigned flags) {
  if (t->tuning.fused_spread == 0 || n_gauss != 10 || t->tuning.deterministic >= 2) return false;
  if (t->tuning.fused == 0 || !t->quad || t->compute_dtype != TC_DTYPE_F64 ||
      t->quad_total.d_table == nullptr || t->quad_tiling.n_rtiles != 1 || t->n_r > 20 ||
      t->chain || t->tuning.trace || t->quad_total.layout.comps.size() != 1 ||
      !t->quad_total.layout.comps[0].triangular)
    return false;
  if (flags & (TC_FLAG_SEPARATE_GAL_TYPE | TC_FLAG_ASSEMBIAS | TC_FLAG_MODULATE_WITH_CENOCC |
               TC_FLAG_LEAUTHAUD11))
    return false;
  if (t->grouped) return false;
  if (t->tuning.fused_draws != 0 && t->tuning.fused_draws != 40) return false;
  if (fused_lds_bytes(t, false, 8, 40) > kMaxLdsBytes) return false;
  if (t->tuning.fused_draws == 40) return true;
  const bool alone = t->force_lane >= 0 || !t->tuning.pipeline || t->n_lanes == 1 ||
                     t->sync_spread;
  if (alone && !t->sync_spread && n_draws <= (int64_t)32 * t->n_cus &&
      t->tuning.fused_draws == 0 && fused_half_tiles(t, false, n_draws, n_gauss, flags))
    return false;
  return alone && n_draws >= t->tuning.fused_spread_min &&
         n_draws <= (int64_t)40 * t->n_cus * std::max(1, t->tuning.fused_spread_rounds);
}

bool fused_half_tiles(const tc_table* t, bool separate, int64_t n_draws, int n_gauss,
                      unsigned flags) {
  if (t->tuning.deterministic >= 2)
    return t->tuning.fused_draws == 32 && n_gauss == 10 &&
           (t->tuning.fused_waves == 0 || t->tuning.fused_waves == 8) &&
           fused_lds_bytes(t, separate, 8, 32) <= 80 * 1024;
  if (t->tuning.fused_draws == 0 && n_gauss == 10 && t->tuning.fused == 1 &&
      t->tuning.fused_min_draws == 0) {
    auto tuned = t->autotuned.find(flags);
    if (tuned != t->autotuned.end() && tuned->second.form_for(n_draws) != 0)
      return tuned->second.form_for(n_draws) == 32 &&
             fused_lds_bytes(t, separate, 8, 32) <= 80 * 1024;
  }
  const bool alone = t->force_lane >= 0 || !t->tuning.pipeline || t->n_lanes == 1;
  if (t->tuning.fused_draws == 64 ||
      (t->tuning.fused_draws == 0 && n_draws >= 8192 && !(alone && n_draws <= (int64_t)32 * t->n_cus)))
    return false;
  if (n_gauss != 10) return false;
  if (t->tuning.fused_waves != 0 && t->tuning.fused_waves != 8) return false;
  return fused_lds_bytes(t, separate, 8, 32) <= 80 * 1024;
}

bool fused_wide_tables(const tc_table* t, bool separate, int n_gauss, unsigned flags) {
  if (n_gauss != 10) return false;
  if (t->tuning.fused_draws == 64 || t->tuning.fused_waves != 0) return false;
  return fused_lds_bytes(t, separate, 8, 64) > 80 * 1024 &&
         fused_lds_bytes(t, separate, 8, 32) <= 80 * 1024;
}

int fused_waves(const tc_table* t, bool separate, unsigned flags) {
  const bool fits8 = fused_lds_bytes(t, separate, 8, 64) <= 80 * 1024;
  const bool fits16 = fused_lds_bytes(t, separate, 16, 64) <= 160 * 1024;
  if (t->tuning.fused_waves == 8 && fused_lds_bytes(t, separate, 8, 64) <= 160 * 1024) return 8;
  if (t->tuning.fused_waves == 16 && fits16) return 16;
  return fits8 ? 8
               : (fits16 && (t->tuning.fused >= 2 || t->autotuned.count(flags) != 0 ||
                             t->tuning.deterministic >= 2)) ? 16 : 0;
}

int run_fused(tc_table* t, const double* theta_device, int n_theta, int64_t n_draws,
              int n_gauss, unsigned flags, double* ngal_device, double* xi_device) {
  Range range("occupation + contraction + finalisation (one launch)");
  tc_table::Lane& lane = t->lanes[t->cur];
  hipStream_t stream = lane.stream;
  Quadrature* q = nullptr;
  int status = get_quadrature(t, n_gauss, &q);
  if (status != TC_OK) return status;
  const bool separate = (flags & TC_FLAG_SEPARATE_GAL_TYPE) != 0;
  const QuadTable& q_table = separate ? t->quad_by_type : t->quad_total;
  tc::FusedArgs fa{};
  fa.theta = theta_device;
  fa.n_theta = n_theta;
  fa.n_bins = t->n_bins;
  fa.n_central = t->plan.n_central;
  fa.n_gauss = n_gauss;
  fa.dens_rows = fused_dens_rows(t, separate);
  fa.separate = separate ? 1 : 0;
  const bool spread = fused_spread_eligible(t, n_draws, n_gauss, flags);
  const bool wide = !spread && fused_wide_tables(t, separate, n_gauss, flags);
  const bool half_tiles = !spread && !wide && fused_half_tiles(t, separate, n_draws, n_gauss, flags);
  const int waves = spread || wide || half_tiles ? 8 : fused_waves(t, separate, flags);
  const int draws = spread ? 40 : wide || half_tiles ? 32 : 64;
  const int n_parts = spread ? 8 : waves * 32 / draws;
  if (!separate) {
    const tc::QuadComp& comp = q_table.layout.comps[0];
    tc::triangle_parts(comp.n_rb, n_parts, fa.part_rb0, fa.part_cb0, fa.part_count);
    for (int part = 0; part < n_parts; ++part) {
      fa.part_triangular[part] = 1;
      fa.part_n_cb[part] = comp.n_cb;
      fa.part_i_row0[part] = comp.i_bin0;
      fa.part_j_row0[part] = comp.j_bin0;
      fa.part_unit_base[part] = (int)comp.unit_base;
    }
  } else {
    const int quarter = n_parts / 4;
    for (int part = 0; part < n_parts; ++part) {
      const int c = part < quarter ? 0 : part < 3 * quarter ? 1 : 2;
      const int first = c == 0 ? 0 : c == 1 ? quarter : 3 * quarter;
      const int pieces = c == 1 ? 2 * quarter : quarter, piece = part - first;
      const tc::QuadComp& comp = q_table.layout.comps[c];
      fa.part_triangular[part] = comp.triangular;
      fa.part_n_cb[part] = comp.n_cb;
      fa.part_i_row0[part] = comp.i_bin0;
      fa.part_j_row0[part] = comp.j_bin0;
      fa.part_unit_base[part] = (int)comp.unit_base;
      if (comp.triangular) {
        int32_t rb0[tc::kFusedMaxParts], cb0[tc::kFusedMaxParts], count[tc::kFusedMaxParts];
        tc::triangle_parts(comp.n_rb, pieces, rb0, cb0, count);
        fa.part_rb0[part] = rb0[piece];
        fa.part_cb0[part] = cb0[piece];
        fa.part_count[part] = count[piece];
      } else {
        const int64_t begin = comp.n_units * piece / pieces;
        const int64_t end = comp.n_units * (piece + 1) / pieces;
        fa.part_rb0[part] = (int)(begin / comp.n_cb);
        fa.part_cb0[part] = (int)(begin % comp.n_cb);
        fa.part_count[part] = (int)(end - begin);
      }
    }
  }
  fa.n_r = t->n_r;
  fa.priority = (t->tuning.prio_fused & 3) | ((t->tuning.prio_fused_occ & 3) << 2) |
                ((t->tuning.prio_fused_out & 3) << 4) |
                ((env_int_early("TC_FUSED_SKIP", 0) & 3) << 8) |
                (q_table.finite ? 1 << 11 : 0);
  fa.n_draws = n_draws;
  fa.n_groups = t->node_groups.n_groups;
  fa.n_central_groups = t->node_groups.n_central_groups;
  fa.group = group_args(t, *q);
  fa.series = (series_mask(t) & 1) ? (const double*)q->series : nullptr;
  fa.series_thr = (const int32_t*)q->series_thr;
  fa.sat_series = (series_mask(t) & 2) ? (const double*)q->sat_series : nullptr;
  fa.sat_series_thr = (const int32_t*)q->sat_series_thr;
  fa.log_m = (const double*)q->log_m;
  fa.m = (const double*)q->m;
  fa.weight = (const double*)q->weight;
  fa.n_h = (const double*)t->d_n_h;
  fa.percentile = (const double*)t->d_percentile;
  fa.split = 0.5;
  fa.math_table = (const double*)t->d_math_table;
  fa.table = q_table.d_table;
  fa.table_bytes =
      (uint32_t)((size_t)q_table.layout.n_units * (size_t)((t->quad_tiling.n_u + 1) / 2) * 1024);
  fa.ngal = ngal_device;
  fa.xi = xi_device;
  t->chi2_fused = false;
  if (t->fuse_chi2_out != nullptr) {
    fa.chi2_data = t->fuse_chi2_data;
    fa.chi2 = t->fuse_chi2_out;
    fa.xi = nullptr;
    t->chi2_fused = true;
  }
  const int lds = fused_lds_bytes(t, separate, waves, draws);
  const dim3 grid((unsigned)((n_draws + draws - 1) / draws)), block(64 * waves);
#ifdef TC_DEVELOPER_KNOBS
  if (fa.chi2 == nullptr && env_int_early("TC_FUSED_STAMPS", 0) != 0) {
    t->trace_blocks = ((size_t)grid.x * 32 + 5) / 6;
    status = t->trace.reserve(t->trace_blocks * 6 * sizeof(unsigned long long), stream);
    if (status != TC_OK) return status;
    fa.chi2_data = (const double*)t->trace.ptr;
    fa.priority |= 1 << 10;
  }
  if (env_int_early("TC_FUSED_SAME_UNIT", 0) != 0) fa.priority |= 1 << 12;
#endif
  hipEvent_t k0 = nullptr, k1 = nullptr;
  status = next_kernel_events(t, &k0, &k1);
  if (status != TC_OK) return status;
  const bool assembias = (flags & TC_FLAG_ASSEMBIAS) != 0;
  const bool modulate = (flags & TC_FLAG_MODULATE_WITH_CENOCC) != 0;
  const bool sat_defer = t->tuning.fused_defer != 0 && !assembias && !modulate &&
                         !(flags & TC_FLAG_LEAUTHAUD11) && n_gauss == 10 && !wide &&
                         !half_tiles && waves == 8 && t->n_bins <= 256 &&
                         !(t->grouped && n_gauss == 10) && t->tuning.series != 0 &&
                         q->sat_series != nullptr && q->sat_records != nullptr;
  if (sat_defer) fa.sat_series = (const double*)q->sat_series;
  fa.sat_records = (const double*)q->sat_records;
  fa.cen_records = (const double*)q->cen_records;
  const bool cen_defer = sat_defer && t->tuning.fused_defer >= 2 && (series_mask(t) & 1) != 0 &&
                         q->cen_records != nullptr;
  fa.sat_cap = t->tuning.fused_sat_cap;
  tc::host::FusedInstance instance{};
  instance.n_gauss = n_gauss == 10 ? 10 : 0;
  instance.assembias = assembias;
  instance.modulate = modulate;
  instance.leauthaud = (flags & TC_FLAG_LEAUTHAUD11) != 0;
  instance.waves = waves;
  instance.draws = draws;
  instance.grouped = t->grouped && n_gauss == 10 && !(flags & TC_FLAG_LEAUTHAUD11);
  instance.defer = cen_defer ? 2 : sat_defer ? 1 : 0;
  status = launch_fused_instance(instance, t->device, t->quad_tiling.n_u, grid, block, lds, stream,
                                 k0, k1, fa);
  if (status != TC_OK) return status;
  t->last_workgroups = (int)grid.x;
  t->last_waves = waves;
  t->last_splits = 0;
  t->last_lds = lds;
  t->prev = t->force_lane >= 0 ? -1 : t->cur;
  return TC_OK;
}


CrossFused* choose_cross_fused(tc_table* const* tables, int n_tables, CrossFused* narrow,
                               CrossFused* wide, int64_t n_draws, unsigned flags, int* status) {
  const tc_table* t0 = tables[0];
  *status = TC_OK;
  if (!narrow->tried) *status = build_cross_fused(tables, n_tables, narrow);
  if (*status != TC_OK || narrow->rows == 0 || narrow->rows > tc::kCrossSmallRows) return narrow;
  const bool undecorated =
      !(flags & (TC_FLAG_ASSEMBIAS | TC_FLAG_MODULATE_WITH_CENOCC | TC_FLAG_LEAUTHAUD11));
  if (t0->tuning.deterministic >= 2) return narrow;
  if (!undecorated || t0->tuning.cross_defer == 0 || (series_mask(t0) & 1) == 0 ||
      t0->node_groups.largest > 2 || t0->tuning.cross_wide_min_draws <= 0 ||
      n_draws < t0->tuning.cross_wide_min_draws)
    return narrow;
  if (!wide->tried) *status = build_cross_fused(tables, n_tables, wide, true);
  return *status == TC_OK && wide->rows > 0 ? wide : narrow;
}

int build_cross_fused(tc_table* const* tables, int n_tables, CrossFused* cf, bool wide) {
  cf->tried = true;
  cf->rows = 0;
  cf->n_tables = n_tables;
  const tc_table* t0 = tables[0];
  if (t0->mode != TC_MODE_CROSS || t0->compute_dtype != TC_DTYPE_F64) return TC_OK;
  const int per_table = t0->n_r + 1;
  if ((int64_t)n_tables * per_table > tc::kCrossMaxRows) return TC_OK;
  for (int k = 0; k < n_tables; ++k) {
    const tc_table* t = tables[k];
    if (t->cross_host.empty() || t->n_bins != t0->n_bins || t->n_r != t0->n_r ||
        t->plan.perm != t0->plan.perm || t->log_min != t0->log_min ||
        t->log_max != t0->log_max || t->percentile != t0->percentile ||
        t->dist_index != t0->dist_index || t->legacy != t0->legacy)
      return TC_OK;
  }
  const int rows = n_tables * per_table;
  const int instance = rows <= 16 && !wide ? 16 : rows <= 32 ? 32 : rows <= 64 ? 64 : 128;
  const tc::NodeGroups& groups = t0->node_groups;
  if (groups.largest > tc::kCrossChunkBins) return TC_OK;
  std::vector<int32_t> chunk_group{0};
  cf->n_central_chunks = 0;
  for (int g = 0, members = 0; g < groups.n_groups; ++g) {
    const int size = groups.begin[g + 1] - groups.begin[g];
    if (g > chunk_group.back() &&
        (members + size > tc::kCrossChunkBins || g == groups.n_central_groups)) {
      chunk_group.push_back(g);
      members = 0;
    }
    if (g == groups.n_central_groups) cf->n_central_chunks = (int)chunk_group.size() - 1;
    members += size;
  }
  if (groups.n_central_groups == groups.n_groups) cf->n_central_chunks = (int)chunk_group.size();
  chunk_group.push_back(groups.n_groups);
  cf->n_chunks = (int)chunk_group.size() - 1;
  cf->chunk_group_host = chunk_group;
  std::vector<double> host((size_t)t0->n_bins * instance, 0.0);
  for (int mi = 0; mi < t0->n_bins; ++mi) {
    const int g = groups.member[mi];
    for (int k = 0; k < n_tables; ++k) {
      const tc_table* t = tables[k];
      double* row = host.data() + (size_t)mi * instance + (size_t)k * per_table;
      for (int r = 0; r < t->n_r; ++r) row[r] = t->cross_host[(size_t)g * t->n_r + r] * t->n_h[g];
      row[t->n_r] = t->n_h[g];
    }
  }
  std::vector<int32_t> chunk_block(cf->n_chunks + 1, 0);
  if (instance > tc::kCrossSmallRows) {
    const int row_blocks = instance / 16;
    for (int c = 0; c < cf->n_chunks; ++c) {
      const int bins = groups.begin[chunk_group[c + 1]] - groups.begin[chunk_group[c]];
      chunk_block[c + 1] = chunk_block[c] + (bins + 3) / 4;
    }
    std::vector<double> operands((size_t)chunk_block[cf->n_chunks] * row_blocks * 64, 0.0);
    for (int c = 0; c < cf->n_chunks; ++c) {
      const int m0 = groups.begin[chunk_group[c]], m1 = groups.begin[chunk_group[c + 1]];
      for (int mi = m0; mi < m1; ++mi) {
        const int step = chunk_block[c] + (mi - m0) / 4, k = (mi - m0) % 4;
        for (int row = 0; row < instance; ++row)
          operands[((size_t)step * row_blocks + row / 16) * 64 + k * 16 + row % 16] =
              host[(size_t)mi * instance + row];
      }
    }
    host.swap(operands);
    std::vector<int32_t> bin_operand(t0->n_bins, 0);
    for (int c = 0; c < cf->n_chunks; ++c) {
      const int m0 = groups.begin[chunk_group[c]], m1 = groups.begin[chunk_group[c + 1]];
      for (int mi = m0; mi < m1; ++mi)
        bin_operand[mi] = ((chunk_block[c] + (mi - m0) / 4) * row_blocks) * 64 + ((mi - m0) % 4) * 16;
    }
    const int uploaded = upload(bin_operand, &cf->d_bin_operand);
    if (uploaded != TC_OK) return uploaded;
  }
  int status = upload(host, &cf->d_rows);
  if (status == TC_OK) status = upload(chunk_group, &cf->d_chunk_group);
  if (status == TC_OK) status = upload(chunk_block, &cf->d_chunk_block);
  if (status != TC_OK) return status;
  cf->rows = instance;
  return TC_OK;
}

namespace {
struct CrossLds {
  int res0 = 0, tile = 0, bitmap = 0, list = 0, bytes = 0;
};
CrossLds cross_lds_layout(const CrossFused& cf, int n_r, bool separate, int defer_groups = 0) {
  CrossLds lds;
  int end = tc::kCrossTableDoubles + tc::cross_buffer_doubles(cf.rows);
  if (defer_groups > 0) {
    lds.list = tc::kCrossTableDoubles + cf.rows * 64;
    lds.bitmap = end;
    end += (defer_groups + 1) / 2 * 2;
  }
  if (separate) {
    lds.res0 = end;
    end += cf.rows * 64;
  }
  const int tile = cf.n_tables * 64 + (separate ? 2 : 1) * n_r * 65;
  if (tile <= tc::kCrossTableDoubles) {
    lds.tile = 0;
  } else {
    lds.tile = end;
    end += tile;
  }
  lds.bytes = end * 8;
  return lds;
}
}

bool cross_fused_eligible(const tc_table* t0, const CrossFused& cf, int64_t n_draws, int n_gauss,
                          unsigned flags, bool alone) {
  if (cf.rows == 0 || t0->tuning.fused == 0 || n_gauss != 10 || t0->chain || t0->tuning.trace)
    return false;
  if (flags & TC_FLAG_LEAUTHAUD11) return false;
  const bool separate = (flags & TC_FLAG_SEPARATE_GAL_TYPE) != 0;
  const tc::NodeGroups& groups = t0->node_groups;
  if (separate && (groups.n_central_groups == 0 || groups.n_central_groups == groups.n_groups ||
                   t0->fuse_chi2_out != nullptr))
    return false;
  if (cf.rows > tc::kCrossSmallRows &&
      cross_lds_layout(cf, t0->n_r, separate).bytes > kMaxLdsBytes - 256)
    return false;
  if (t0->fuse_chi2_out != nullptr && t0->n_r > 32) return false;
  if (t0->tuning.deterministic >= 2) return true;
// ... 792 lines not shown
```

tabcorr_amd/csrc/table.cpp:

```cpp
#include <cmath>

#include "internal.h"

using namespace tc::host;

extern "C" {

int tc_table_create(int mode, int n_bins, int n_r, int64_t n_pairs,
                    const void* tpcf_matrix, int matrix_dtype, const double* n_h,
                    const double* log_min, const double* log_max,
                    const double* percentile, const double* dist_index,
                    const uint8_t* is_central, int compute_dtype, tc_table** out) {
  TC_CHECK(out != nullptr, "table output pointer is NULL");
  *out = nullptr;
  TC_CHECK(mode == TC_MODE_AUTO || mode == TC_MODE_CROSS, "invalid mode %d", mode);
  TC_CHECK(n_bins >= 1 && n_bins < (1 << 20), "invalid number of bins %d", n_bins);
  TC_CHECK(n_r >= 1, "invalid number of correlation function bins %d", n_r);
  const int64_t expect =
      mode == TC_MODE_AUTO ? (int64_t)n_bins * (n_bins + 1) / 2 : n_bins;
  TC_CHECK(n_pairs == expect,
           "tpcf_matrix has %lld columns but %d bins in mode '%s' need %lld",
           (long long)n_pairs, n_bins, mode == TC_MODE_AUTO ? "auto" : "cross",
           (long long)expect);
  TC_CHECK(n_pairs < (1LL << 31), "too many pair columns");
// ... 31 lines not shown
    tc::build_plan(mode, n_bins, is_central, tc::kF32Block,
                   env_int("TC_ROW_BUDGET_F32", 128), t->plan);
  } else {
    int rt = (n_r + t->n_rtiles - 1) / t->n_rtiles;
    t->rt = (rt + 3) / 4 * 4;
    const int budget = std::max(56, std::min(128, n_bins / 2 + 6));
    tc::build_plan(mode, n_bins, is_central, tc::kF64Block,
                   env_int("TC_ROW_BUDGET", budget), t->plan);
  }

  for (int g = 0; g < n_bins; ++g) {
    const int src = t->plan.perm[g];
    t->n_h.push_back(n_h[src]);
    t->log_min.push_back(log_min[src]);
    t->log_max.push_back(log_max[src]);
    t->percentile.push_back(percentile[src]);
    t->dist_index.push_back(dist_index ? dist_index[src] : -1.0);
  }

  const int rt = t->rt;
  const int64_t n_positions = t->plan.n_positions;
  const size_t count = (size_t)t->n_rtiles * n_positions * rt;
  auto source = [&](int r, int64_t column) {
    return matrix_dtype == TC_DTYPE_F64
               ? ((const double*)tpcf_matrix)[(size_t)r * n_pairs + column]
               : (double)((const float*)tpcf_matrix)[(size_t)r * n_pairs + column];
  };
  std::vector<double> tmp64;
  std::vector<float> tmp32;
  std::vector<int32_t> pos_ij;
  if (compute_dtype == TC_DTYPE_F64) {
    t->table_bytes = count * sizeof(double);
    tmp64.assign(count, 0.0);
    for (int r = 0; r < n_r; ++r) {
      const int tile = r / rt, rr = r % rt;
      for (int64_t q = 0; q < n_positions; ++q) {
        const int64_t column = t->plan.column[q];
        if (column < 0) continue;
        const size_t index = ((size_t)tile * n_positions + q / 8 * 8) * rt +
                             (((rr / 4) * 16 + (q % 4) * 4 + rr % 4) * 2 + (q / 4) % 2);
        tmp64[index] = source(r, column) * t->plan.prefactor[q];
      }
    }
    pos_ij.assign((size_t)n_positions * 2, 0);
    for (int64_t q = 0; q < n_positions; ++q) {
      const size_t slot = ((size_t)(q / 8) * 4 + q % 4) * 4 + ((q / 4) % 2) * 2;
      pos_ij[slot] = std::max(t->plan.pos_i[q], 0) * 512;
      pos_ij[slot + 1] = t->plan.pos_j[q] * 512;
    }
  } else {
    t->table_bytes = count * sizeof(float);
    tmp32.assign(count, 0.0f);
    for (int r = 0; r < n_r; ++r) {
      const int tile = r / rt, rr = r % rt;
      for (int64_t q = 0; q < n_positions; ++q) {
        const int64_t column = t->plan.column[q];
        if (column < 0) continue;
        const int64_t block = q / 8;
        const int p = (int)(q % 8) / 2, k = (int)(q % 2);
        tmp32[((size_t)tile * n_positions + block * 8) * rt + (k * 32 + rr) * 4 + p] =
            (float)(source(r, column) * t->plan.prefactor[q]);
      }
    }
    pos_ij.assign((size_t)n_positions, 0);
    for (int64_t q = 0; q < n_positions; ++q) {
      const int64_t block = q / 8;
      const int p = (int)(q % 8) / 2, k = (int)(q % 2);
      const int i = t->plan.pos_i[q] < 0 ? 0 : t->plan.pos_i[q];
      pos_ij[(size_t)block * 8 + k * 4 + p] = (i << 16) | t->plan.pos_j[q];
    }
  }
  if (mode == TC_MODE_CROSS && compute_dtype == TC_DTYPE_F64 &&
      (int64_t)n_r + 1 <= tc::kCrossMaxRows) {
    t->cross_host.resize((size_t)n_bins * n_r);
    for (int g = 0; g < n_bins; ++g)
      for (int r = 0; r < n_r; ++r)
        t->cross_host[(size_t)g * n_r + r] = source(r, t->plan.perm[g]);
  }
  t->n_lanes = std::max(1, std::min(t->tuning.lanes, (int)tc_table::kMaxLanes));
  {
    hipStream_t streams[tc_table::kMaxLanes] = {};
    const int created = create_lane_streams(t->n_lanes, streams);
    for (int l = 0; l < t->n_lanes; ++l) t->lanes[l].stream = streams[l];
    if (created != TC_OK) return created;
    for (int l = 0; l < t->n_lanes; ++l)
      TC_HIP(hipEventCreateWithFlags(&t->lanes[l].finished, hipEventDisableTiming));
  }
  t->stream = t->lanes[0].stream;
  TC_HIP(hipEventCreate(&t->ev_begin));
  TC_HIP(hipEventCreate(&t->ev_end));
  int status = compute_dtype == TC_DTYPE_F64 ? upload(tmp64, &t->d_table)
                                             : upload(tmp32, &t->d_table);
  if (status == TC_OK && compute_dtype == TC_DTYPE_F32)
    status = upload(pos_ij, &t->d_pos_ij);
  if (status == TC_OK && compute_dtype == TC_DTYPE_F64)
    status = upload(pos_ij, &t->d_pos_off);
  if (status == TC_OK) status = upload(t->n_h, &t->d_n_h);
  if (status == TC_OK) status = upload(t->percentile, &t->d_percentile);
  if (status == TC_OK) status = upload(t->plan.perm, &t->d_perm);
  tc::find_node_groups(n_bins, t->plan.n_central, t->log_min.data(), t->log_max.data(),
                       t->node_groups);
  t->grouped = t->node_groups.largest > 1;
  if (status == TC_OK) status = upload(t->node_groups.begin, &t->d_group_begin);
  if (status == TC_OK) status = upload(t->node_groups.member, &t->d_group_member);
  {
    std::vector<double> n_h_m, percentile_m;
    for (int32_t g : t->node_groups.member) {
      n_h_m.push_back(t->n_h[g]);
      percentile_m.push_back(t->percentile[g]);
    }
    if (status == TC_OK) status = upload(n_h_m, &t->d_group_n_h);
    if (status == TC_OK) status = upload(percentile_m, &t->d_group_percentile);
  }
  if (status == TC_OK) {
    std::vector<double> math_table(tc::fm::kTableDoubles);
    tc::fm::build_tables(math_table.data());
    status = upload(math_table, &t->d_math_table);
  }
  const tc::QuadTiling quad_tiling = tc::quad_tiling(n_r);
  const double quad_blocks = (n_bins / 4.0 + 1.0) * (n_bins / 4.0 + 2.0) / 2.0;
  const double quad_bytes =
      quad_blocks * ((quad_tiling.n_u + 1) / 2) * 1024.0 * quad_tiling.n_rtiles;
  const tc::QuadTiling quad_tiling_f32 = tc::quad_tiling_f32(n_r);
  const bool quad_f32 = compute_dtype == TC_DTYPE_F32 && quad_blocks * 1024.0 <= 3.0 * 1024 * 1024;
  if (status == TC_OK && mode == TC_MODE_AUTO &&
      ((compute_dtype == TC_DTYPE_F64 && quad_bytes <= 256.0 * 1024 * 1024) || quad_f32)) {
    t->quad = true;
    t->quad_tiling = quad_f32 ? quad_tiling_f32 : quad_tiling;
    status = build_quad_table(t.get(), true, tpcf_matrix, matrix_dtype, &t->quad_by_type);
    const int n_central = t->plan.n_central;
    const bool fusable = !quad_f32 && quad_tiling.n_rtiles == 1 && n_r <= 20 && n_bins <= 248;
    if (status == TC_OK && ((n_central % 4 != 0 && n_central < n_bins) || fusable))
      status = build_quad_table(t.get(), false, tpcf_matrix, matrix_dtype, &t->quad_total);
  }
  if (status != TC_OK) return status;
  *out = t.release();
  return TC_OK;
}

int tc_table_destroy(tc_table* t) {
  if (t == nullptr) return TC_OK;
  (void)hipSetDevice(t->device);
  (void)resident_stop(t);
  if (t->resident.stream) (void)hipStreamDestroy(t->resident.stream);
  t->resident.mailbox.release();
  t->resident.ens_mailbox.release();
  t->resident.ens_out.release();
  t->resident.ens_device.release();
  t->resident.ens_aperture.release();
  t->resident.single_aperture.release();
  t->resident.ws.buffer.release();
  for (tc_table::Lane& lane : t->lanes)
    if (lane.stream) (void)hipStreamSynchronize(lane.stream);
  for (void* p : {t->d_table, t->d_n_h, t->d_percentile, t->d_perm, t->d_math_table,
                  t->d_pos_ij, t->d_pos_off, t->d_group_begin, t->d_group_member,
                  t->d_group_n_h, t->d_group_percentile})
    if (p) (void)hipFree(p);
  for (auto& kv : t->quadrature)
    for (void* p : {kv.second.log_m, kv.second.m, kv.second.weight, kv.second.group_log_m,
                    kv.second.group_m, kv.second.group_weight, kv.second.series,
                    kv.second.series_thr, kv.second.group_series, kv.second.group_series_thr,
                    kv.second.sat_series, kv.second.sat_series_thr, kv.second.group_sat_series,
                    kv.second.group_sat_series_thr, kv.second.group_records, kv.second.sat_records, kv.second.cen_records})
      if (p) (void)hipFree(p);
  for (auto& kv : t->chunkings)
    for (void* p : {kv.second->chunks, kv.second->groups})
      if (p) (void)hipFree(p);
  t->quad_by_type.release();
  t->quad_total.release();
  t->cross_fused.release();
  t->cross_fused_wide.release();
  for (DeviceBuffer* b : {&t->theta, &t->out_ngal, &t->out_xi, &t->occupation,
                          &t->trace, &t->wave_trace, &t->chi2_data})
    b->release();
  for (tc_table::Lane& lane : t->lanes) {
    lane.nbuf.release();
    lane.ngal2.release();
    lane.partial.release();
    lane.xi.release();
    lane.nbuf32.release();
    lane.in_theta.release();
    lane.out.release();
    lane.cross_counters.release();
    if (lane.finished) (void)hipEventDestroy(lane.finished);
  }
  for (tc_table::Ticket& ticket : t->tickets)
    if (ticket.done) (void)hipEventDestroy(ticket.done);
  t->h_in.release();
  t->h_out.release();
  t->single_ws.buffer.release();
  for (auto& ev : t->kernel_events) {
    (void)hipEventDestroy(ev.first);
    (void)hipEventDestroy(ev.second);
  }
  for (hipEvent_t event : t->chunk_events) (void)hipEventDestroy(event);
  if (t->ev_begin) (void)hipEventDestroy(t->ev_begin);
  if (t->ev_end) (void)hipEventDestroy(t->ev_end);
  for (tc_table::Lane& lane : t->lanes)
    if (lane.stream) (void)hipStreamDestroy(lane.stream);
  delete t;
  return TC_OK;
}

int tc_table_synchronize(tc_table* t) {
  TC_CHECK(t != nullptr, "table handle is NULL");
  for (tc_table::Lane& lane : t->lanes)
    if (lane.stream) TC_HIP(hipStreamSynchronize(lane.stream));
  return TC_OK;
}

int tc_table_info(const tc_table* t, int* mode, int* n_bins, int* n_r,
                  int64_t* n_pairs, int* n_components, int64_t* device_bytes) {
  TC_CHECK(t != nullptr, "table handle is NULL");
  if (mode) *mode = t->mode;
  if (n_bins) *n_bins = t->n_bins;
  if (n_r) *n_r = t->n_r;
  if (n_pairs) *n_pairs = t->n_pairs;
  if (n_components) *n_components = t->plan.n_components;
  if (device_bytes) *device_bytes = (int64_t)t->table_bytes;
  return TC_OK;
}

}

namespace {
int autotune(tc_table* t, unsigned flags);

int maybe_autotune(tc_table* t, int n_gauss, unsigned flags) {
  if (t->autotuning || t->tuning.autotune_after <= 0 || t->tuning.deterministic != 0 ||
      n_gauss != 10 || t->tuning.fused != 1 ||
      t->tuning.fused_min_draws != 0 || t->tuning.fused_draws != 0 || t->tuning.fused_waves != 0)
    return TC_OK;
  const bool pipelined = t->async_lane >= 0 || (t->force_lane < 0 && t->tuning.pipeline &&
                                                t->n_lanes > 1);
  if (!pipelined || !t->quad || t->compute_dtype != TC_DTYPE_F64 || t->mode != TC_MODE_AUTO ||
      t->quad_tiling.n_rtiles != 1 || t->n_r > 20 || t->chain || t->tuning.trace ||
      t->fuse_chi2_out != nullptr)
    return TC_OK;
  const unsigned key = flags & (TC_FLAG_SEPARATE_GAL_TYPE | TC_FLAG_MODULATE_WITH_CENOCC |
                                TC_FLAG_ASSEMBIAS | TC_FLAG_LEAUTHAUD11);
  if (t->autotuned.count(key) != 0) return TC_OK;
  if (++t->pipelined_calls[key] < t->tuning.autotune_after) return TC_OK;
  t->pipelined_calls[key] = 0;
  const int saved_force = t->force_lane, saved_async = t->async_lane, saved_cur = t->cur;
  t->autotuning = true;
  t->force_lane = t->async_lane = -1;
  const int status = autotune(t, key);
  t->autotuning = false;
  t->force_lane = saved_force;
  t->async_lane = saved_async;
  t->cur = saved_cur;
  if (status != TC_OK) {
    t->tuning.autotune_after = 0;
    (void)tc_table_synchronize(t);
  }
  return TC_OK;
}
}

extern "C" {

int tc_predict_zheng07_batch_device(tc_table* t, const double* theta_device,
                                    int n_theta, int64_t n_draws, int n_gauss,
                                    unsigned flags, double* ngal_device,
                                    double* xi_device) {
  int status = check_predict_args(t, theta_device, n_theta, n_draws, n_gauss, flags);
  if (status != TC_OK) return status;
  if (n_draws == 0) return TC_OK;
  TC_CHECK(ngal_device && xi_device, "output pointer is NULL");
  TC_HIP(hipSetDevice(t->device));
  if (t->resident.running && (status = resident_stop(t)) != TC_OK) return status;
  const bool separate = (flags & TC_FLAG_SEPARATE_GAL_TYPE) != 0;
  const int n_comp = separate ? t->plan.n_components : 1;
  t->chi2_fused = false;
  if (t->force_lane >= 0)
    t->cur = t->force_lane;
  else if (t->async_lane >= 0)
    t->cur = t->async_lane;
  else
    t->cur = t->tuning.pipeline ? (int)(t->device_calls++ % t->n_lanes) : 0;
  if ((status = maybe_autotune(t, n_gauss, flags)) != TC_OK) return status;
  const int64_t slab = max_slab(t);
  for (int64_t begin = 0; begin < n_draws; begin += slab) {
    const int64_t n = std::min(slab, n_draws - begin);
    const int64_t ldb = (n + 63) / 64 * 64;
    if (t->mode == TC_MODE_CROSS && !t->cross_host.empty() && t->tuning.fused != 0) {
      tc_table* self = t;
      const CrossFused& cf = *choose_cross_fused(&self, 1, &t->cross_fused, &t->cross_fused_wide,
                                                 n, flags, &status);
      if (status != TC_OK) return status;
      const bool alone = t->force_lane >= 0 || !t->tuning.pipeline || t->n_lanes == 1;
      if (cross_fused_eligible(t, cf, n, n_gauss, flags, alone)) {
        status = run_cross_fused(t, cf, nullptr, theta_device + begin * n_theta,
                                 n_theta, n, flags, ngal_device + begin * (separate ? 2 : 1),
                                 xi_device + begin * n_comp * t->n_r, t->lanes[t->cur].stream,
                                 &t->lanes[t->cur].partial, &t->lanes[t->cur].cross_counters);
        if (status != TC_OK) return status;
        t->prev = t->force_lane >= 0 ? -1 : t->cur;
        continue;
      }
    }
    if (fused_eligible(t, n, n_gauss, flags)) {
      status = run_fused(t, theta_device + begin * n_theta, n_theta, n, n_gauss, flags,
                         ngal_device + begin * (separate ? 2 : 1),
                         xi_device + begin * n_comp * t->n_r);
      if (status != TC_OK) return status;
      continue;
    }
    status = run_occupation(t, theta_device + begin * n_theta, n_theta, n, ldb,
                            n_gauss, flags, nullptr);
    if (status != TC_OK) return status;
    status = run_contraction(t, n, ldb, flags,
                             ngal_device + begin * (separate ? 2 : 1),
                             xi_device + begin * n_comp * t->n_r);
    if (status != TC_OK) return status;
  }
  return TC_OK;
}

}

namespace tc {
namespace host {

int copy_in(PinnedBuffer* stage, void* device, const void* host, size_t bytes,
            hipStream_t stream) {
  Range range("upload");
  if (bytes <= stage_limit() && stage->reserve(bytes) == TC_OK) {
    memcpy(stage->ptr, host, bytes);
    host = stage->ptr;
  }
  TC_HIP(hipMemcpyAsync(device, host, bytes, hipMemcpyHostToDevice, stream));
  return TC_OK;
}

int copy_out(PinnedBuffer* stage, double* ngal, size_t ngal_count, const void* d_ngal,
// ... 409 lines not shown
                           : 0;
  tc_table::Lane& lane = t->lanes[lane_index];
  status = lane.xi.reserve((size_t)n_draws * t->n_r * 8, lane.stream);
  if (status != TC_OK) return status;
  const double* d_data = (const double*)t->chi2_data.ptr;
  t->fuse_chi2_data = d_data;
  t->fuse_chi2_out = chi2_device;
  status = tc_predict_zheng07_batch_device(t, theta_device, n_theta, n_draws, n_gauss, flags,
                                           ngal_device, (double*)lane.xi.ptr);
  t->fuse_chi2_out = nullptr;
  if (status != TC_OK) return status;
  if (t->chi2_fused) return TC_OK;
  status = launch_chi2((const double*)lane.xi.ptr, n_draws, t->n_r, d_data, d_data + t->n_r,
                       chi2_device, lane.stream);
  if (status != TC_OK) return status;
  if (t->force_lane < 0 && t->chain) TC_HIP(hipEventRecord(lane.finished, lane.stream));
  return TC_OK;
}

int tc_chi2_zheng07_batch(tc_table* t, const double* theta, int n_theta,
                          int64_t n_draws, int n_gauss, unsigned flags,
                          const double* data, const double* precision, double* ngal,
                          double* chi2) {
  int status = check_predict_args(t, theta, n_theta, n_draws, n_gauss, flags);
  if (status != TC_OK) return status;
  TC_CHECK(!(flags & TC_FLAG_SEPARATE_GAL_TYPE),
           "chi2 is defined for the total correlation function only");
  if (n_draws == 0) return TC_OK;
  TC_CHECK(data && precision && ngal && chi2, "NULL pointer");
  TC_HIP(hipSetDevice(t->device));
  const int n_r = t->n_r;
  const size_t xi_count = (size_t)n_draws * n_r;
  const size_t theta_bytes = (size_t)n_draws * n_theta * sizeof(double);
  status = t->out_xi.reserve(xi_count * 8, t->stream);
  if (status == TC_OK) status = upload_chi2_data(t, data, precision);
  if (status != TC_OK) return status;
  double* d_data = (double*)t->chi2_data.ptr;
  double* d_precision = d_data + n_r;
  const bool direct = theta_bytes + (size_t)n_draws * 16 <= zero_copy_limit() &&
                      t->h_in.reserve(theta_bytes) == TC_OK &&
                      t->h_out.reserve((size_t)n_draws * 16) == TC_OK;
  const double* theta_device = nullptr;
  double* d_ngal = nullptr;
  if (direct) {
    memcpy(t->h_in.ptr, theta, theta_bytes);
    theta_device = (const double*)t->h_in.ptr;
    d_ngal = (double*)t->h_out.ptr;
  } else {
    status = t->theta.reserve(theta_bytes, t->stream);
    if (status == TC_OK) status = t->out_ngal.reserve((size_t)n_draws * 2 * 8, t->stream);
    if (status != TC_OK) return status;
    status = copy_in(&t->h_in, t->theta.ptr, theta, theta_bytes, t->stream);
    if (status != TC_OK) return status;
    theta_device = (const double*)t->theta.ptr;
    d_ngal = (double*)t->out_ngal.ptr;
  }
  double* d_chi2 = d_ngal + n_draws;
  const bool fuse = n_draws <= max_slab(t);
  t->force_lane = 0;
  t->fuse_chi2_data = d_data;
  t->fuse_chi2_out = fuse ? d_chi2 : nullptr;
  status = tc_predict_zheng07_batch_device(t, theta_device, n_theta, n_draws, n_gauss, flags,
                                           d_ngal, (double*)t->out_xi.ptr);
  t->fuse_chi2_out = nullptr;
  t->force_lane = -1;
  if (status != TC_OK) return status;
  if (!(fuse && t->chi2_fused))
    status = launch_chi2((const double*)t->out_xi.ptr, n_draws, n_r, d_data, d_precision,
                         d_chi2, t->stream);
  if (status != TC_OK) return status;
  if (direct) {
    TC_HIP(hipStreamSynchronize(t->stream));
    memcpy(ngal, d_ngal, (size_t)n_draws * 8);
    memcpy(chi2, d_chi2, (size_t)n_draws * 8);
    return TC_OK;
  }
  return copy_out(&t->h_out, ngal, (size_t)n_draws, d_ngal, chi2, (size_t)n_draws,
                  d_chi2, t->stream);
}

namespace {

int next_ticket(tc_table* t, tc_table::Ticket** out) {
  tc_table::Ticket& slot = t->tickets[t->next_ticket % tc_table::kMaxTickets];
  if (slot.done == nullptr)
    TC_HIP(hipEventCreateWithFlags(&slot.done, hipEventDisableTiming));
  slot.id = t->next_ticket++;
  *out = &slot;
  return TC_OK;
}

int predict_async(tc_table* t, const double* theta, int n_theta, int64_t n_draws, int n_gauss,
                  unsigned flags, const double* data, const double* precision, double* ngal,
                  double* second, bool chi2, int64_t* ticket_out, bool staging,
                  hipEvent_t wait_for, hipEvent_t kernels_done) {
  int status = check_predict_args(t, theta, n_theta, n_draws, n_gauss, flags);
  if (status != TC_OK) return status;
  TC_CHECK(ticket_out != nullptr, "ticket is NULL");
  TC_CHECK(n_draws == 0 || (ngal && second), "output pointer is NULL");
  const bool separate = (flags & TC_FLAG_SEPARATE_GAL_TYPE) != 0;
  TC_CHECK(!(chi2 && separate), "chi2 is defined for the total correlation function only");
  TC_CHECK(!chi2 || (data && precision), "NULL pointer");
  TC_CHECK(!chi2 || n_draws <= max_slab(t), "at most %lld draws per call",
           (long long)max_slab(t));
  const int n_comp = separate ? t->plan.n_components : 1;
  const size_t ngal_count = (size_t)n_draws * (separate ? 2 : 1);
  const size_t second_count = chi2 ? (size_t)n_draws : (size_t)n_draws * n_comp * t->n_r;
  const size_t theta_bytes = (size_t)n_draws * n_theta * sizeof(double);
  void *theta_seen = nullptr, *ngal_seen = nullptr, *second_seen = nullptr;
  if (staging) {
    theta_seen = (void*)theta;
    ngal_seen = ngal;
    second_seen = second;
  } else {
    TC_CHECK(n_draws == 0 || (is_pinned(theta, theta_bytes, &theta_seen) &&
                              is_pinned(ngal, ngal_count * 8, &ngal_seen) &&
                              is_pinned(second, second_count * 8, &second_seen)),
             "asynchronous calls need page-locked buffers (tc_host_alloc / tc_host_register)");
  }
  TC_HIP(hipSetDevice(t->device));
  if (t->resident.running) {
    const int stopped = resident_stop(t);
    if (stopped != TC_OK) return stopped;
  }
  tc_table::Ticket* ticket = nullptr;
  const int lane_index = t->tuning.pipeline ? (int)(t->device_calls++ % t->n_lanes) : 0;
  tc_table::Lane& lane = t->lanes[lane_index];
  if (n_draws > 0) {
    const int mode = staging ? t->tuning.sync_direct_out : t->tuning.async_direct_out;
    const size_t direct_bytes = staging ? kSyncDirectOutBytes : kDirectOutBytes;
    auto direct = [mode, direct_bytes](void* seen, size_t count) {
      return seen != nullptr && (mode == 1 || (mode == 2 && count * 8 <= direct_bytes));
    };
    const bool direct_in = t->tuning.async_direct_in && theta_seen != nullptr;
    const bool direct_ngal = direct(ngal_seen, ngal_count);
    const bool direct_second = direct(second_seen, second_count);
    if (!direct_in) status = lane.in_theta.reserve(theta_bytes, lane.stream);
    if (status == TC_OK && !(direct_ngal && direct_second))
      status = lane.out.reserve((ngal_count + second_count) * 8, lane.stream);
    if (status != TC_OK) return status;
    const double* d_theta = direct_in ? (const double*)theta_seen
                                      : (const double*)lane.in_theta.ptr;
    double* d_ngal = direct_ngal ? (double*)ngal_seen : (double*)lane.out.ptr;
    double* d_second = direct_second ? (double*)second_seen
                                     : (double*)lane.out.ptr + ngal_count;
    if (!direct_in) {
      Range range("upload");
      TC_HIP(hipMemcpyAsync(lane.in_theta.ptr, theta, theta_bytes, hipMemcpyHostToDevice,
                            lane.stream));
    }
    if (wait_for != nullptr) TC_HIP(hipStreamWaitEvent(lane.stream, wait_for, 0));
    const bool saved_chain = t->chain;
    t->async_lane = lane_index;
    t->chain = false;
    status = chi2 ? tc_chi2_zheng07_batch_device(t, d_theta, n_theta, n_draws, n_gauss, flags,
                                                 data, precision, d_ngal, d_second)
                  : tc_predict_zheng07_batch_device(t, d_theta, n_theta, n_draws, n_gauss,
                                                    flags, d_ngal, d_second);
    t->async_lane = -1;
    t->chain = saved_chain;
    if (status != TC_OK) return status;
    if (kernels_done != nullptr) TC_HIP(hipEventRecord(kernels_done, lane.stream));
    Range range("download");
    if (!direct_ngal && !direct_second && second == ngal + ngal_count) {
      TC_HIP(hipMemcpyAsync(ngal, d_ngal, (ngal_count + second_count) * 8,
                            hipMemcpyDeviceToHost, lane.stream));
    } else {
      if (!direct_ngal)
        TC_HIP(hipMemcpyAsync(ngal, d_ngal, ngal_count * 8, hipMemcpyDeviceToHost,
                              lane.stream));
      if (!direct_second)
        TC_HIP(hipMemcpyAsync(second, d_second, second_count * 8, hipMemcpyDeviceToHost,
                              lane.stream));
    }
  }
  status = next_ticket(t, &ticket);
  if (status != TC_OK) return status;
  TC_HIP(hipEventRecord(ticket->done, lane.stream));
  *ticket_out = ticket->id;
  return TC_OK;
}

}

int tc_predict_zheng07_batch_async(tc_table* t, const double* theta, int n_theta,
                                   int64_t n_draws, int n_gauss, unsigned flags, double* ngal,
                                   double* xi, int64_t* ticket) {
  return predict_async(t, theta, n_theta, n_draws, n_gauss, flags, nullptr, nullptr, ngal, xi,
                       false, ticket, false);
}

int tc_chi2_zheng07_batch_async(tc_table* t, const double* theta, int n_theta, int64_t n_draws,
                                int n_gauss, unsigned flags, const double* data,
                                const double* precision, double* ngal, double* chi2,
                                int64_t* ticket) {
  return predict_async(t, theta, n_theta, n_draws, n_gauss, flags, data, precision, ngal, chi2,
                       true, ticket, false);
}

int tc_table_wait(tc_table* t, int64_t ticket) {
  TC_CHECK(t != nullptr, "table handle is NULL");
  TC_CHECK(ticket >= 0 && ticket < t->next_ticket, "unknown ticket %lld", (long long)ticket);
  const tc_table::Ticket& slot = t->tickets[ticket % tc_table::kMaxTickets];
  if (slot.id == ticket) {
    TC_HIP(hipEventSynchronize(slot.done));
    return TC_OK;
  }
  return tc_table_synchronize(t);
}

int tc_table_query(tc_table* t, int64_t ticket, int* done) {
  TC_CHECK(t != nullptr && done != nullptr, "NULL argument");
  TC_CHECK(ticket >= 0 && ticket < t->next_ticket, "unknown ticket %lld", (long long)ticket);
  const tc_table::Ticket& slot = t->tickets[ticket % tc_table::kMaxTickets];
  *done = 0;
  if (slot.id == ticket) {
    const hipError_t state = hipEventQuery(slot.done);
    if (state == hipSuccess) *done = 1;
    else if (state != hipErrorNotReady)
      return fail(TC_ERR_HIP, "hipEventQuery failed: %s", hipGetErrorString(state));
    return TC_OK;
  }
  *done = 1;
  for (tc_table::Lane& lane : t->lanes) {
    if (lane.stream == nullptr) continue;
    const hipError_t state = hipStreamQuery(lane.stream);
    if (state == hipErrorNotReady) *done = 0;
    else if (state != hipSuccess)
      return fail(TC_ERR_HIP, "hipStreamQuery failed: %s", hipGetErrorString(state));
  }
  return TC_OK;
}

int tc_mean_occupation_zheng07_batch(tc_table* t, const double* theta, int n_theta,
                                     int64_t n_draws, int n_gauss, unsigned flags,
                                     double* occupation) {
  int status = check_predict_args(t, theta, n_theta, n_draws, n_gauss, flags);
  if (status != TC_OK) return status;
  if (n_draws == 0) return TC_OK;
  TC_CHECK(occupation != nullptr, "output pointer is NULL");
  TC_HIP(hipSetDevice(t->device));
  if (t->resident.running) {
    const int stopped = resident_stop(t);
    if (stopped != TC_OK) return stopped;
  }
  const int64_t slab = max_slab(t);
  for (int64_t begin = 0; begin < n_draws; begin += slab) {
    const int64_t n = std::min(slab, n_draws - begin);
    const int64_t ldb = (n + 63) / 64 * 64;
    const size_t occ_bytes = (size_t)n * t->n_bins * 8;
    status = t->theta.reserve((size_t)n * n_theta * 8, t->stream);
    if (status == TC_OK) status = t->occupation.reserve(occ_bytes, t->stream);
    if (status != TC_OK) return status;
    TC_HIP(hipMemcpyAsync(t->theta.ptr, theta + begin * n_theta,
                          (size_t)n * n_theta * 8, hipMemcpyHostToDevice, t->stream));
    t->cur = 0;
    status = run_occupation(t, (const double*)t->theta.ptr, n_theta, n, ldb, n_gauss,
                            flags, (double*)t->occupation.ptr);
    if (status != TC_OK) return status;
    TC_HIP(hipMemcpyAsync(occupation + begin * t->n_bins, t->occupation.ptr,
                          occ_bytes, hipMemcpyDeviceToHost, t->stream));
    TC_HIP(hipStreamSynchronize(t->stream));
  }
  return TC_OK;
}

int tc_predict_occupation_batch(tc_table* t, const double* occupation,
                                int64_t n_draws, unsigned flags, double* ngal,
                                double* xi) {
  TC_CHECK(t != nullptr, "table handle is NULL");
  TC_CHECK(n_draws >= 0, "n_draws must be non-negative");
  if (n_draws == 0) return TC_OK;
  TC_CHECK(occupation && ngal && xi, "NULL array");
  TC_HIP(hipSetDevice(t->device));
  if (t->resident.running) {
    const int stopped = resident_stop(t);
    if (stopped != TC_OK) return stopped;
  }
  const bool separate = (flags & TC_FLAG_SEPARATE_GAL_TYPE) != 0;
  const int n_comp = separate ? t->plan.n_components : 1;
  const int64_t slab = max_slab(t);
  for (int64_t begin = 0; begin < n_draws; begin += slab) {
    const int64_t n = std::min(slab, n_draws - begin);
    const int64_t ldb = (n + 63) / 64 * 64;
    const size_t occ_bytes = (size_t)n * t->n_bins * 8;
    const size_t ngal_count = (size_t)n * (separate ? 2 : 1);
    const size_t xi_count = (size_t)n * n_comp * t->n_r;
    int status = t->occupation.reserve(occ_bytes, t->stream);
    if (status == TC_OK)
      status = t->lanes[0].nbuf.reserve((size_t)t->n_bins * ldb * 8, t->stream);
    if (status == TC_OK)
      status = t->lanes[0].ngal2.reserve(2 * ldb * 8, t->stream);
    if (status == TC_OK) status = t->out_ngal.reserve(ngal_count * 8, t->stream);
    if (status == TC_OK) status = t->out_xi.reserve(xi_count * 8, t->stream);
    if (status != TC_OK) return status;
    status = copy_in(&t->h_in, t->occupation.ptr, occupation + begin * t->n_bins,
                     occ_bytes, t->stream);
    if (status != TC_OK) return status;
    status = launch_occ_from_array(t, (const double*)t->occupation.ptr, n, ldb,
                                   (double*)t->lanes[0].nbuf.ptr,
                                   (double*)t->lanes[0].ngal2.ptr, t->stream);
    if (status != TC_OK) return status;
    t->cur = 0;
    t->lanes[0].ngal_parts = 1;
    status = run_contraction(t, n, ldb, flags, (double*)t->out_ngal.ptr,
                             (double*)t->out_xi.ptr);
    if (status != TC_OK) return status;
    status = copy_out(&t->h_out, ngal + begin * (separate ? 2 : 1), ngal_count,
                      t->out_ngal.ptr, xi + begin * n_comp * t->n_r, xi_count,
                      t->out_xi.ptr, t->stream);
    if (status != TC_OK) return status;
  }
// ... 47 lines not shown
  if (status != TC_OK) return status;
  TC_HIP(hipMemcpy(d_theta.ptr, theta.data(), theta.size() * 8, hipMemcpyHostToDevice));

  const Tuning saved = t->tuning;
  struct Restore {
    tc_table* t;
    Tuning saved;
    ~Restore() { t->tuning = saved; }
  } restore{t, saved};
  t->tuning.fused_min_draws = 1;
  t->tuning.fused_max_draws = 1 << 30;
  auto time_form = [&](int64_t n, float* us) -> int {
    auto call = [&]() {
      return tc_predict_zheng07_batch_device(t, (const double*)d_theta.ptr, n_theta, n, 10, flags,
                                             (double*)d_ngal.ptr, (double*)d_xi.ptr);
    };
    int st = TC_OK;
    for (int k = 0; k < 4 && st == TC_OK; ++k) st = call();
    if (st == TC_OK) st = tc_table_synchronize(t);
    if (st != TC_OK) return st;
    int calls = 8;
    double seconds = 0.0;
    for (;;) {
      const auto t0 = std::chrono::steady_clock::now();
      for (int k = 0; k < calls && st == TC_OK; ++k) st = call();
      if (st == TC_OK) st = tc_table_synchronize(t);
      if (st != TC_OK) return st;
      seconds = std::chrono::duration<double>(std::chrono::steady_clock::now() - t0).count();
      if (seconds >= 8e-3 || calls >= 400) break;
      calls = (int)std::min<double>(400.0, std::max<double>(calls * 2.0,
                                                            calls * 1e-2 / std::max(seconds, 1e-6)));
    }
    *us = (float)(seconds / calls * 1e6);
    return TC_OK;
  };
  AutoChoice choice;
  for (int i = 0; i < AutoChoice::kSizes; ++i) {
    const int64_t n = AutoChoice::size(i);
    t->tuning.fused = 0;
    status = time_form(n, &choice.us[i][0]);
    if (status != TC_OK) return status;
    choice.form[i] = 0;
    float best = choice.us[i][0];
    const int shapes[2] = {64, 32};
    for (int k = 0; k < 2; ++k) {
      t->tuning.fused = 2;
      t->tuning.fused_draws = shapes[k];
      choice.us[i][1 + k] = 0.0f;
      if (!fused_eligible(t, n, 10, flags)) continue;
      const bool half = fused_wide_tables(t, separate, 10, flags) ||
                        fused_half_tiles(t, separate, n, 10, flags);
      if (half != (shapes[k] == 32)) continue;
      status = time_form(n, &choice.us[i][1 + k]);
      if (status != TC_OK) return status;
      if (choice.us[i][1 + k] < 0.98f * best) {
        best = choice.us[i][1 + k];
        choice.form[i] = shapes[k];
      }
    }
  }
  t->autotuned[flags] = choice;
  return TC_OK;
}

}

int tc_table_autotune_result(const tc_table* t, unsigned flags, int capacity, int* count,
                             int64_t* sizes, int* forms, float* us) {
  TC_CHECK(t != nullptr && count && sizes && forms && us, "NULL argument");
  *count = 0;
  auto it = t->autotuned.find(flags);
  TC_CHECK(it != t->autotuned.end(), "no autotune result for these flags");
  TC_CHECK(capacity >= AutoChoice::kSizes, "capacity below %d", (int)AutoChoice::kSizes);
  for (int i = 0; i < AutoChoice::kSizes; ++i) {
    sizes[i] = AutoChoice::size(i);
    forms[i] = it->second.form[i];
    for (int k = 0; k < 3; ++k) us[3 * i + k] = it->second.us[i][k];
  }
  *count = AutoChoice::kSizes;
  return TC_OK;
}

int tc_table_resident_stats(const tc_table* t, int64_t* launches, int64_t* relaunches,
                            int64_t* failures, int* running) {
  TC_CHECK(t != nullptr, "table handle is NULL");
  const tc_table::Resident& r = t->resident;
  if (launches) *launches = (int64_t)r.launch_id;
  if (relaunches) *relaunches = (int64_t)r.relaunches;
  if (failures) *failures = (int64_t)r.auto_failures;
  if (running) *running = r.running ? (r.ensemble ? 2 : 1) : 0;
  return TC_OK;
}

int tc_table_batch_invariant(tc_table* t, int n_gauss, unsigned flags, int* out) {
  TC_CHECK(t != nullptr && out != nullptr, "NULL argument");
  TC_HIP(hipSetDevice(t->device));
  *out = batch_invariant_form(t, n_gauss, flags) ? 1 : 0;
  return TC_OK;
}

int tc_table_set_option(tc_table* t, const char* name, int value) {
  TC_CHECK(t != nullptr && name != nullptr, "NULL argument");
  TC_HIP(hipSetDevice(t->device));
  const std::string key(name);
  if (key == "pipeline") {
    t->tuning.pipeline = value != 0;
  } else if (key == "deterministic") {
    TC_CHECK(value >= 0 && value <= 2, "deterministic must be 0, 1 or 2");
    int status = resident_stop(t);
    if (status != TC_OK) return status;
    for (tc_table::Lane& lane : t->lanes)
      if (lane.stream) TC_HIP(hipStreamSynchronize(lane.stream));
    t->tuning.deterministic = value;
    if (value != 0) {
      t->autotuned.clear();
      t->tuning.autotune_after = 0;
    }
  } else if (key == "autotune_after") {
    TC_CHECK(value == 0 || t->tuning.deterministic == 0,
             "autotune_after: the measured dispatch is not available while \"deterministic\" is set");
    TC_CHECK(value >= 0, "autotune_after must be non-negative");
    t->tuning.autotune_after = value;
  } else if (key == "autotune") {
    if (value < 0) {
      t->autotuned.clear();
      return TC_OK;
    }
    TC_CHECK(t->tuning.deterministic == 0,
             "autotune: the measured dispatch is not available while \"deterministic\" is set");
    return autotune(t, (unsigned)value);
  } else if (key == "resident_min_walkers") {
    TC_CHECK(value >= 2 && value <= 256, "resident_min_walkers must be in [2, 256]");
    t->resident.min_walkers = value;
  } else if (key == "resident_wait_us") {
    TC_CHECK(value >= 1 && value <= 1000000, "resident_wait_us must be in [1, 1000000]");
    const int status = resident_stop(t);
    if (status != TC_OK) return status;
    t->resident.wait_us = value;
  } else if (key == "resident_aperture") {
    TC_CHECK(value == 0 || value == 1, "resident_aperture must be 0 or 1");
    const int status = resident_stop(t);
    if (status != TC_OK) return status;
    t->tuning.resident_aperture = value;
    t->resident.ens_grid = 0;
    t->resident.single_aperture_decided = false;
  } else if (key == "cross_min_draws") {
    TC_CHECK(value >= 1, "cross_min_draws must be positive");
    t->tuning.cross_min_draws = value;
  } else if (key == "cross_defer") {
    t->tuning.cross_defer = value != 0;
  } else if (key == "fused_defer") {
    TC_CHECK(value >= 0 && value <= 2, "fused_defer must be 0, 1 or 2");
    t->tuning.fused_defer = value;
  } else if (key == "fused_sat_cap") {
    TC_CHECK(value >= 0 && value <= 6, "fused_sat_cap must be in [0, 6]");
    t->tuning.fused_sat_cap = value;
  } else if (key == "cross_wide_min_draws") {
    TC_CHECK(value >= 0, "cross_wide_min_draws must not be negative");
    t->tuning.cross_wide_min_draws = value;
  } else if (key == "cross_target") {
    TC_CHECK(value >= 1 && value <= 4096, "cross_target must be in [1, 4096]");
    t->tuning.cross_target = value;
  } else if (key == "series") {
    TC_CHECK(value >= -1 && value <= 3, "series must be -1 .. 3");
    t->tuning.series = value;
  } else if (key == "grouped") {
    t->grouped = value != 0 && t->node_groups.largest > 1;
  } else if (key == "lanes") {
    TC_CHECK(value >= 1 && value <= (int)tc_table::kMaxLanes, "lanes must be in [1, %d]",
             (int)tc_table::kMaxLanes);
    for (tc_table::Lane& lane : t->lanes)
      if (lane.stream) TC_HIP(hipStreamSynchronize(lane.stream));
    for (int l = 0; l < value; ++l) {
      if (t->lanes[l].stream != nullptr) continue;
      TC_HIP(hipStreamCreateWithFlags(&t->lanes[l].stream, hipStreamNonBlocking));
      TC_HIP(hipEventCreateWithFlags(&t->lanes[l].finished, hipEventDisableTiming));
    }
    t->tuning.lanes = t->n_lanes = value;
    t->prev = -1;
  } else if (key == "ordered") {
    for (tc_table::Lane& lane : t->lanes)
      if (lane.stream) TC_HIP(hipStreamSynchronize(lane.stream));
    t->chain = value != 0;
    t->prev = -1;
  } else if (key == "sync_chunks") {
    TC_CHECK(value >= -1 && value <= 64, "sync_chunks must be in [-1, 64]");
    t->tuning.sync_chunks = value;
  } else if (key == "sync_stagger") {
    TC_CHECK(value >= 0 && value <= 100, "sync_stagger must be in [0, 100]");
    t->tuning.sync_stagger = value;
  } else if (key == "sync_form") {
    TC_CHECK(value == 0 || value == 32 || value == 64, "sync_form must be 0, 32 or 64");
    t->tuning.sync_form = value;
  } else if (key == "sync_direct_out") {
    TC_CHECK(value >= 0 && value <= 2, "sync_direct_out must be 0, 1 or 2");
    t->tuning.sync_direct_out = value;
  } else if (key == "async_direct_in" || key == "async_direct_out") {
    (key == "async_direct_in" ? t->tuning.async_direct_in : t->tuning.async_direct_out) =
        value;
  } else if (key == "fused") {
    TC_CHECK(value >= 0 && value <= 2, "fused must be 0, 1 or 2");
    t->tuning.fused = value;
  } else if (key == "fused_min_draws" || key == "fused_max_draws") {
    TC_CHECK(value >= (key == "fused_min_draws" ? 0 : 1), "%s must be positive", name);
    (key == "fused_min_draws" ? t->tuning.fused_min_draws : t->tuning.fused_max_draws) = value;
  } else if (key == "resident") {
    TC_CHECK(value >= 0 && value <= 2, "resident must be 0, 1 or 2");
    t->resident.enabled = value == 1;
    t->resident.auto_mode = value == 2;
    t->resident.auto_streak = t->resident.auto_backoff = 0;
    t->resident.auto_window = t->resident.auto_relaunches = 0;
    t->resident.auto_failures = 0;
    t->resident.ens_disabled = false;
    t->resident.ens_failures = 0;
    if (value != 1) return resident_stop(t);
  } else if (key == "resident_inject_failures") {
    TC_CHECK(value >= 0, "resident_inject_failures must not be negative");
    t->resident.inject_failures = value;
  } else if (key == "resident_auto_idle_us") {
    TC_CHECK(value >= 10 && value <= 100000, "resident_auto_idle_us must be in [10, 100000]");
    const int status = resident_stop(t);
    if (status != TC_OK) return status;
    t->resident.auto_idle_us = value;
  } else if (key == "resident_poll_waves") {
    TC_CHECK(value >= 1 && value <= 4, "resident_poll_waves must be in [1, 4]");
    const int status = resident_stop(t);
    if (status != TC_OK) return status;
    t->resident.poll_waves = value;
  } else if (key == "resident_idle_us") {
    TC_CHECK(value >= 10 && value <= 1000000, "resident_idle_us must be in [10, 1000000]");
    const int status = resident_stop(t);
    if (status != TC_OK) return status;
    t->resident.idle_us = value;
  } else if (key == "fused_draws") {
    TC_CHECK(value == 0 || value == 32 || value == 40 || value == 64,
             "fused_draws must be 0, 32, 40 or 64");
    t->tuning.fused_draws = value;
  } else if (key == "fused_spread") {
    t->tuning.fused_spread = value != 0;
  } else if (key == "fused_spread_min") {
    TC_CHECK(value >= 1, "fused_spread_min must be positive");
    t->tuning.fused_spread_min = value;
  } else if (key == "fused_spread_rounds") {
    TC_CHECK(value >= 1 && value <= 64, "fused_spread_rounds must be in [1, 64]");
    t->tuning.fused_spread_rounds = value;
  } else if (key == "fused_waves") {
    TC_CHECK(value == 0 || value == 8 || value == 16, "fused_waves must be 0, 8 or 16");
    t->tuning.fused_waves = value;
  } else if (key == "prio_fused") {
    t->tuning.prio_fused = value & 3;
  } else if (key == "prio_fused_occ") {
    t->tuning.prio_fused_occ = value & 3;
  } else if (key == "prio_fused_out") {
    t->tuning.prio_fused_out = value & 3;
  } else if (key == "single_draw") {
    t->tuning.single_draw = value != 0;
  } else if (key == "many_blocks") {
    TC_CHECK(value >= 2 && value <= 4096, "many_blocks must be in [2, 4096]");
    t->tuning.many_blocks = value;
  } else if (key == "single_round") {
    t->tuning.single_round = value != 0;
  } else if (key == "poll_done") {
    t->tuning.poll_done = value != 0;
  } else if (key == "trace") {
    t->tuning.trace = value;
  } else if (key == "occ_splits" || key == "occ_per_cu" || key == "finalize_threads" ||
             key == "finalize_row_blocks") {
    TC_CHECK(value >= 0 && value <= 4096, "invalid value");
    (key == "occ_splits" ? t->tuning.occ_splits
     : key == "occ_per_cu" ? t->tuning.occ_per_cu
     : key == "finalize_threads" ? t->tuning.finalize_threads
                                 : t->tuning.finalize_row_blocks) = value;
  } else if (key == "prio_occ" || key == "prio_contract" || key == "prio_finalize") {
    TC_CHECK(value >= 0 && value <= 3, "priorities are 0..3");
    (key == "prio_occ" ? t->tuning.prio_occ
                       : key == "prio_contract" ? t->tuning.prio_contract
                                                : t->tuning.prio_finalize) = value;
  } else if (key == "quad_merge" || key == "quad_waves" || key == "quad_order") {
    for (tc_table::Lane& lane : t->lanes)
      if (lane.stream) TC_HIP(hipStreamSynchronize(lane.stream));
    if (key == "quad_merge") t->tuning.quad_merge = value != 0;
    else if (key == "quad_order") t->tuning.quad_order = value;
    else t->tuning.quad_waves = t->tuning.quad_waves_f32 = value;
    for (tc::host::QuadTable* q : {&t->quad_by_type, &t->quad_total}) q->drop_schedules();
  } else {
    return fail(TC_ERR_INVALID, "unknown option '%s'", name);
  }
  return TC_OK;
}

int tc_table_timer_begin(tc_table* t, int profile_kernels) {
  TC_CHECK(t != nullptr, "table handle is NULL");
  TC_HIP(hipSetDevice(t->device));
  t->profile_kernels = profile_kernels != 0;
  t->profile_every = profile_kernels > 1 ? profile_kernels : 1;
  t->profile_launches = 0;
  t->kernel_events_used = 0;
  TC_HIP(hipEventRecord(t->ev_begin, t->stream));
  return TC_OK;
}

int tc_table_timer_end(tc_table* t, float* elapsed_ms) {
  TC_CHECK(t != nullptr && elapsed_ms != nullptr, "NULL argument");
  for (int l = 1; l < tc_table::kMaxLanes; ++l)
    if (t->lanes[l].stream) TC_HIP(hipStreamSynchronize(t->lanes[l].stream));
  TC_HIP(hipEventRecord(t->ev_end, t->stream));
  TC_HIP(hipEventSynchronize(t->ev_end));
  TC_HIP(hipEventElapsedTime(elapsed_ms, t->ev_begin, t->ev_end));
  t->profile_kernels = false;
  return TC_OK;
}

int tc_table_kernel_time(tc_table* t, int* n_launches, float* mean_ms) {
  TC_CHECK(t != nullptr && n_launches && mean_ms, "NULL argument");
  double total = 0.0;
  for (size_t i = 0; i < t->kernel_events_used; ++i) {
    float ms = 0.0f;
    TC_HIP(hipEventSynchronize(t->kernel_events[i].second));
    TC_HIP(hipEventElapsedTime(&ms, t->kernel_events[i].first,
                               t->kernel_events[i].second));
    total += ms;
  }
  *n_launches = (int)t->kernel_events_used;
  *mean_ms = t->kernel_events_used ? (float)(total / t->kernel_events_used) : 0.0f;
  return TC_OK;
}

int tc_debug_trace(tc_table* t, uint64_t* out, int64_t capacity, int64_t* n_blocks) {
  TC_CHECK(t != nullptr && n_blocks != nullptr, "NULL argument");
  *n_blocks = (int64_t)t->trace_blocks;
  if (out == nullptr || t->trace.ptr == nullptr) return TC_OK;
  for (tc_table::Lane& lane : t->lanes)
      if (lane.stream) TC_HIP(hipStreamSynchronize(lane.stream));
  const int64_t n = std::min<int64_t>(capacity, (int64_t)t->trace_blocks);
  TC_HIP(hipMemcpy(out, t->trace.ptr, (size_t)n * 6 * sizeof(uint64_t),
                   hipMemcpyDeviceToHost));
  return TC_OK;
}

int tc_debug_wave_trace(tc_table* t, uint64_t* out, int64_t capacity, int64_t* n_waves) {
  TC_CHECK(t != nullptr && n_waves != nullptr, "NULL argument");
  *n_waves = (int64_t)t->wave_trace_count;
  if (out == nullptr || t->wave_trace.ptr == nullptr) return TC_OK;
  for (tc_table::Lane& lane : t->lanes)
      if (lane.stream) TC_HIP(hipStreamSynchronize(lane.stream));
  const int64_t n = std::min<int64_t>(capacity, (int64_t)t->wave_trace_count);
  TC_HIP(hipMemcpy(out, t->wave_trace.ptr, (size_t)n * 6 * sizeof(uint64_t),
                   hipMemcpyDeviceToHost));
  return TC_OK;
}

int tc_debug_resident_ticks(tc_table* t, uint64_t* out, int64_t capacity, int64_t* n_blocks) {
  TC_CHECK(t != nullptr && n_blocks != nullptr, "NULL argument");
  *n_blocks = t->resident.mailbox.ptr != nullptr ? t->resident.blocks : 0;
  if (out == nullptr || t->resident.mailbox.ptr == nullptr) return TC_OK;
  const unsigned long long* words = (const unsigned long long*)t->resident.mailbox.ptr;
  for (int64_t b = 0; b < std::min<int64_t>(capacity, *n_blocks); ++b)
    out[b] = words[16 + kSingleMaxBlocks + b];
  return TC_OK;
}

int tc_debug_ensemble_stamps(tc_table* t, uint64_t* out) {
  TC_CHECK(t != nullptr && out != nullptr, "NULL argument");
  TC_CHECK(t->resident.ens_mailbox.ptr != nullptr, "no ensemble call has been made");
  const unsigned long long* words = (const unsigned long long*)t->resident.ens_mailbox.ptr;
  const size_t offset = 8 + (size_t)tc::kEnsembleMaxWalkers * 8 + t->resident.ens_grid;
  for (int i = 0; i < 8; ++i) out[i] = words[offset + i];
  for (int i = 0; i < 3; ++i) out[8 + i] = t->resident.ens_host_ns[i];
  return TC_OK;
}

int tc_table_last_launch(const tc_table* t, int* n_workgroups, int* waves,
                         int* n_splits, int* lds_bytes) {
  TC_CHECK(t != nullptr, "table handle is NULL");
  if (n_workgroups) *n_workgroups = t->last_workgroups;
  if (waves) *waves = t->last_waves;
  if (n_splits) *n_splits = t->last_splits;
  if (lds_bytes) *lds_bytes = t->last_lds;
  return TC_OK;
}

}
```

Measured before the change: 271.6 million calls/s.

## Regroup draws by satellite mass bucket and skip all-zero density blocks in contraction

A new pre-kernel computes a permutation that sorts draws within 16384-draw segments by which satellite bin top their log_M0 falls under. The fused kernel then processes draws in that order, scattering ngal, xi and chi2 back to the original indices. Grouping similar draws makes whole rows or columns of satellite densities zero across a 64-draw tile. A masked quadratic pass uses per-wave ballot masks to skip those zero blocks in the MFMA contraction. The cost is an extra kernel launch, a permutation buffer, and indirect (less coalesced) reads and writes. The masked pass is further gated on a priority bit.

```diff
diff --git a/include/tabcorr_amd_testing.h b/include/tabcorr_amd_testing.h
--- a/include/tabcorr_amd_testing.h
+++ b/include/tabcorr_amd_testing.h
@@ -41,6 +41,8 @@
                         int64_t* n_waves);
 int tc_debug_resident_ticks(tc_table* table, uint64_t* out, int64_t capacity, int64_t* n_blocks);
 int tc_debug_ensemble_stamps(tc_table* table, uint64_t* out);
+int tc_debug_regroup_perm(tc_table* table, int lane, int32_t* out, int64_t capacity,
+                          int64_t* n_draws);
 #ifdef __cplusplus
 }
 #endif
diff --git a/tabcorr_amd/_lib.py b/tabcorr_amd/_lib.py
--- a/tabcorr_amd/_lib.py
+++ b/tabcorr_amd/_lib.py
@@ -155,6 +155,8 @@
     'tc_table_kernel_time': [ctypes.c_void_p, c_int_p, c_float_p],
     'tc_debug_trace': [ctypes.c_void_p, ctypes.POINTER(ctypes.c_uint64),
                        ctypes.c_int64, c_int64_p],
+    'tc_debug_regroup_perm': [ctypes.c_void_p, ctypes.c_int, c_int32_p,
+                              ctypes.c_int64, c_int64_p],
     'tc_debug_wave_trace': [ctypes.c_void_p, ctypes.POINTER(ctypes.c_uint64),
                             ctypes.c_int64, c_int64_p],
     'tc_debug_resident_ticks': [ctypes.c_void_p, ctypes.POINTER(ctypes.c_uint64),
diff --git a/tabcorr_amd/csrc/inst_fused.hip b/tabcorr_amd/csrc/inst_fused.hip
--- a/tabcorr_amd/csrc/inst_fused.hip
+++ b/tabcorr_amd/csrc/inst_fused.hip
@@ -2,6 +2,14 @@
 
 namespace tc {
 namespace host {
+
+int launch_regroup_perm(const tc::RegroupArgs& args, hipStream_t stream) {
+  const dim3 grid((unsigned)((args.n_draws + tc::kRegroupThreads - 1) / tc::kRegroupThreads));
+  hipLaunchKernelGGL((tc::regroup_perm_kernel<tc::kRegroupThreads>), grid,
+                     dim3(tc::kRegroupThreads), 0, stream, args);
+  TC_HIP(hipGetLastError());
+  return TC_OK;
+}
 
 int launch_fused_instance(const FusedInstance& in, int device, int n_u, dim3 grid, dim3 block,
                        int lds, hipStream_t stream, hipEvent_t k0, hipEvent_t k1,
diff --git a/tabcorr_amd/csrc/internal.h b/tabcorr_amd/csrc/internal.h
--- a/tabcorr_amd/csrc/internal.h
+++ b/tabcorr_amd/csrc/internal.h
@@ -256,6 +256,7 @@
   int cross_defer = 1;
   int fused_defer = 2;
   int fused_sat_cap = 6;
+  int fused_regroup = 1;
   int cross_wide_min_draws = 4096;
   int cross_target = 160;
   int resident_aperture = 1;
@@ -357,6 +358,9 @@
   void* d_group_percentile = nullptr;
   bool grouped = false;
   void* d_math_table = nullptr;
+  void* d_sat_tops = nullptr;
+  int n_sat_tops = -1;
+  bool theta_in_host = false;
   void* d_pos_ij = nullptr;
   void* d_pos_off = nullptr;
   std::vector<double> cross_host;
@@ -385,6 +389,8 @@
     tc::host::DeviceBuffer xi;
     tc::host::DeviceBuffer in_theta, out;
     tc::host::DeviceBuffer cross_counters;
+    tc::host::DeviceBuffer perm;
+    int64_t perm_draws = 0;
     int ngal_parts = 1;
   };
   static constexpr int kMaxLanes = 8;
@@ -573,6 +579,7 @@
   int waves = 8, draws = 64;
   int defer = 0;
 };
+int launch_regroup_perm(const tc::RegroupArgs& args, hipStream_t stream);
 int launch_fused_instance(const FusedInstance& instance, int device, int n_u, dim3 grid,
                           dim3 block, int lds, hipStream_t stream, hipEvent_t k0, hipEvent_t k1,
                           const tc::FusedArgs& fa);
diff --git a/tabcorr_amd/csrc/kernel_args.h b/tabcorr_amd/csrc/kernel_args.h
--- a/tabcorr_amd/csrc/kernel_args.h
+++ b/tabcorr_amd/csrc/kernel_args.h
@@ -283,6 +283,20 @@
   int sat_cap;
   const double* sat_records;
   const double* cen_records;
+  const int32_t* perm;
+};
+
+constexpr int kRegroupSegment = 16384;
+constexpr int kRegroupThreads = 1024;
+constexpr int kRegroupMaxTops = 255;
+struct RegroupArgs {
+  const double* theta;
+  int n_theta;
+  int log_m0_index;
+  int64_t n_draws;
+  const double* tops;
+  int n_tops;
+  int32_t* perm;
 };
 
 constexpr int kCrossWaves = 8;
diff --git a/tabcorr_amd/csrc/kernels.hip.h b/tabcorr_amd/csrc/kernels.hip.h
--- a/tabcorr_amd/csrc/kernels.hip.h
+++ b/tabcorr_amd/csrc/kernels.hip.h
@@ -1845,7 +1845,9 @@
 __device__ __forceinline__ constexpr int dens40(int row, int draw) {
   return row * 40 + (draw & 3) * 10 + (draw >> 2);
 }
-constexpr int fused_scratch_doubles(int waves) { return fm::kTableDoubles + 2 * waves * kLanes; }
+constexpr int fused_scratch_doubles(int waves) {
+  return fm::kTableDoubles + 2 * waves * kLanes + 2 * waves + kLanes / 2;
+}
 static_assert(kFusedWaves == 8 && kFusedMaxParts == 8, "8 or 16 waves: 4 or 8 parts per tile");
 static_assert(20 * (kLanes + 1) + 20 * 21 <= fm::kTableDoubles,
               "results tile + likelihood data in the place of the math table");
@@ -1927,6 +1929,106 @@
   }
 }
 
+template <int UU, int DL>
+__device__ __forceinline__ void fused_quad_pass_masked(
+    __amdgpu_buffer_rsrc_t rs_t, unsigned off_a, unsigned unit_bytes, const double* dens_b,
+    const double* dens_e, int rb, int cb, int left, bool triangular, int n_cb, unsigned unit_base,
+    unsigned long long zero_rows, unsigned long long zero_cols, double (&F)[2][2]) {
+  f64x2 t0, t1, b0, b1;
+  f64x4 D[UU][2];
+  auto fetch = [&](f64x2& t, f64x2& b) {
+    const unsigned ua =
+        (unit_base + (unsigned)(triangular ? rb * (rb + 1) / 2 + cb : rb * n_cb + cb)) * unit_bytes;
+    t = buffer_load16<0>(rs_t, off_a, ua);
+    b = *(const f64x2*)(dens_b + 4 * cb * DL);
+  };
+  auto mma = [&](const f64x2& t, const f64x2& b, bool first) {
+    if (first) {
+      const f64x4 zero = {0.0, 0.0, 0.0, 0.0};
+#pragma unroll
+      for (int u = 0; u < UU; ++u) {
+        const double av = u ? t.y : t.x;
+        D[u][0] = __builtin_amdgcn_mfma_f64_16x16x4f64(av, b.x, zero, 0, 0, 0);
+        D[u][1] = __builtin_amdgcn_mfma_f64_16x16x4f64(av, b.y, zero, 0, 0, 0);
+      }
+    } else {
+#pragma unroll
+      for (int u = 0; u < UU; ++u) {
+        const double av = u ? t.y : t.x;
+        D[u][0] = __builtin_amdgcn_mfma_f64_16x16x4f64(av, b.x, D[u][0], 0, 0, 0);
+        D[u][1] = __builtin_amdgcn_mfma_f64_16x16x4f64(av, b.y, D[u][1], 0, 0, 0);
+      }
+    }
+  };
+  auto seek = [&]() {
+    while (left > 0) {
+      const int row_length = triangular ? rb + 1 : n_cb;
+      const int n = row_length - cb < left ? row_length - cb : left;
+      const unsigned long long open =
+          ((zero_rows >> rb) & 1) ? 0ull
+                                  : (~zero_cols >> cb) & (n >= 64 ? ~0ull : (1ull << n) - 1);
+      if (open != 0) {
+        const int step = __builtin_ctzll(open);
+        cb += step;
+        left -= step;
+        return;
+      }
+      left -= n;
+      ++rb;
+      cb = 0;
+    }
+  };
+  auto advance = [&]() {
+    ++cb;
+    --left;
+    seek();
+  };
+  seek();
+  if (left <= 0) return;
+  fetch(t0, b0);
+  t1 = t0;
+  b1 = b0;
+  while (left > 0) {
+    const int row = rb;
+    f64x2 e[4];
+#pragma unroll
+    for (int v = 0; v < 4; ++v) e[v] = *(const f64x2*)(dens_e + (4 * row + v) * DL);
+    advance();
+    if (left > 0) fetch(t1, b1);
+    __builtin_amdgcn_sched_barrier(0);
+    mma(t0, b0, true);
+    __builtin_amdgcn_sched_barrier(0);
+    bool next_in_t1 = true;
+    while (left > 0 && rb == row) {
+      advance();
+      if (left > 0) fetch(t0, b0);
+      __builtin_amdgcn_sched_barrier(0);
+      mma(t1, b1, false);
+      __builtin_amdgcn_sched_barrier(0);
+      if (!(left > 0 && rb == row)) {
+        next_in_t1 = false;
+        break;
+      }
+      advance();
+      if (left > 0) fetch(t1, b1);
+      __builtin_amdgcn_sched_barrier(0);
+      mma(t0, b0, false);
+      __builtin_amdgcn_sched_barrier(0);
+    }
+    if (next_in_t1) {
+      t0 = t1;
+      b0 = b1;
+    }
+#pragma unroll
+    for (int u = 0; u < UU; ++u)
+#pragma unroll
+      for (int v = 0; v < 4; ++v) {
+        F[u][0] = fma(D[u][0][v], e[v].x, F[u][0]);
+        F[u][1] = fma(D[u][1][v], e[v].y, F[u][1]);
+      }
+  }
+}
+
 __device__ __forceinline__ int wave_prefix_sum(int value) {
   auto shifted = [](int x, auto control, auto rows) {
     return __builtin_amdgcn_update_dpp(0, x, decltype(control)::value, decltype(rows)::value, 0xf,
@@ -1940,6 +2042,78 @@
   value += shifted(value, std::integral_constant<int, 0x142>(), std::integral_constant<int, 0xa>());
   value += shifted(value, std::integral_constant<int, 0x143>(), std::integral_constant<int, 0xc>());
   return value;
+}
+
+template <int THREADS>
+__global__ __launch_bounds__(THREADS) void regroup_perm_kernel(RegroupArgs a) {
+  constexpr int WAVES = THREADS / 64;
+  constexpr int K = kRegroupMaxTops + 1;
+  constexpr int ROUNDS = kRegroupSegment / THREADS;
+  __shared__ double tops[K];
+  __shared__ int total[K], ahead[K], first[K], wave_count[WAVES][K];
+  const int tid = threadIdx.x, lane = tid & 63;
+  const int wave = __builtin_amdgcn_readfirstlane(tid >> 6);
+  const int n_keys = a.n_tops + 1;
+  const int64_t chunk = (int64_t)blockIdx.x * THREADS;
+  const int64_t seg0 = chunk / kRegroupSegment * kRegroupSegment;
+  const int64_t seg1 = seg0 + kRegroupSegment < a.n_draws ? seg0 + kRegroupSegment : a.n_draws;
+  for (int i = tid; i < a.n_tops; i += THREADS) tops[i] = a.tops[i];
+  for (int i = tid; i < n_keys; i += THREADS) total[i] = ahead[i] = 0;
+  for (int i = tid; i < WAVES * K; i += THREADS) (&wave_count[0][0])[i] = 0;
+  double x[ROUNDS];
+#pragma unroll
+  for (int r = 0; r < ROUNDS; ++r) {
+    const int64_t d = seg0 + (int64_t)r * THREADS + tid;
+    x[r] = d < seg1 ? a.theta[d * a.n_theta + a.log_m0_index] : 0.0;
+  }
+  __syncthreads();
+  int key = -1;
+#pragma unroll
+  for (int r = 0; r < ROUNDS; ++r) {
+    const int64_t d = seg0 + (int64_t)r * THREADS + tid;
+    const bool valid = d < seg1;
+    int lo = 0, hi = a.n_tops;
+    while (lo < hi) {
+      const int mid = (lo + hi) >> 1;
+      if (tops[mid] <= x[r]) lo = mid + 1; else hi = mid;
+    }
+    const bool is_ahead = d < chunk;
+    if (d == chunk + tid && valid) key = lo;
+    const unsigned long long live = __builtin_amdgcn_ballot_w64(valid);
+    if (live == 0) continue;
+    const int leader = __builtin_ctzll(live);
+    const int k0 = __builtin_amdgcn_readlane(lo, leader);
+    const unsigned long long same = __builtin_amdgcn_ballot_w64(valid && lo == k0);
+    if (lane == leader) {
+      atomicAdd(&total[k0], __builtin_popcountll(same));
+      if (is_ahead) atomicAdd(&ahead[k0], __builtin_popcountll(same));
+    } else if (valid && lo != k0) {
+      atomicAdd(&total[lo], 1);
+      if (is_ahead) atomicAdd(&ahead[lo], 1);
+    }
+  }
+  const bool mine = key >= 0;
+  int rank = 0;
+  for (unsigned long long todo = __builtin_amdgcn_ballot_w64(mine); todo != 0;) {
+    const int leader = __builtin_ctzll(todo);
+    const int k0 = __builtin_amdgcn_readlane(key, leader);
+    const unsigned long long same = __builtin_amdgcn_ballot_w64(mine && key == k0);
+    if (mine && key == k0) rank = __builtin_popcountll(same & ((1ull << lane) - 1));
+    if (lane == leader) wave_count[wave][k0] = __builtin_popcountll(same);
+    todo &= ~same;
+  }
+  __syncthreads();
+  for (int k = tid; k < n_keys; k += THREADS) {
+    int sum = 0;
+    for (int j = 0; j < k; ++j) sum += total[j];
+    first[k] = sum;
+  }
+  __syncthreads();
+  if (mine) {
+    int position = first[key] + ahead[key] + rank;
+    for (int w = 0; w < wave; ++w) position += wave_count[w][key];
+    a.perm[seg0 + position] = (int32_t)(chunk + tid);
+  }
 }
 
 __device__ __forceinline__ double fused_quad_rows40(double select, double value, double sums) {
@@ -2064,6 +2238,10 @@
   double* dens = fused_lds;
   double* table = fused_lds + region_b;
   double(*red)[W][kLanes] = (double(*)[W][kLanes])(table + fm::kTableDoubles);
+  const bool regroup = DL != 40 && a.perm != nullptr;
+  const bool masks = regroup && !GROUPED;
+  unsigned* const wave_words = (unsigned*)(table + fm::kTableDoubles + 2 * W * kLanes);
+  int* const slot_draw = (int*)(wave_words + 4 * W);
   const fm::Consts kc = fm::make_consts();
 #ifdef TC_DEVELOPER_KNOBS
   const int skip = (a.priority >> 8) & 3;
@@ -2112,7 +2290,9 @@
   };
   const int64_t col = (int64_t)blockIdx.x * DL;
   const int64_t b0 = col + draw;
-  const int64_t b = b0 < a.n_draws ? b0 : a.n_draws - 1;
+  const int64_t slot = b0 < a.n_draws ? b0 : a.n_draws - 1;
+  const int64_t b = regroup ? (int64_t)a.perm[slot] : slot;
+  if (regroup && wave == 0 && half == 0) slot_draw[draw] = (int)b;
   double norm;
   {
     const double* th = a.theta + b * a.n_theta;
@@ -2299,6 +2479,30 @@
         }
       }
     }
+    if (masks) {
+      unsigned zero_lo = 0, zero_hi = 0, odd_lo = 0, odd_hi = 0;
+      int j = 0;
+      for (int g = wave; g < a.n_bins; g += W, ++j) {
+        const double value = dens[g * DL + draw];
+        const unsigned long long zero = __builtin_amdgcn_ballot_w64(value == 0.0);
+        const unsigned long long odd = __builtin_amdgcn_ballot_w64(!(fabs(value) <= 1e100));
+        if (DL == 64) {
+          zero_lo |= ((unsigned)zero == 0xffffffffu ? 1u : 0u) << j;
+          zero_hi |= ((unsigned)(zero >> 32) == 0xffffffffu ? 1u : 0u) << j;
+          odd_lo |= (unsigned)odd;
+          odd_hi |= (unsigned)(odd >> 32);
+        } else {
+          zero_lo |= (zero == ~0ull ? 1u : 0u) << j;
+          odd_lo |= odd != 0 ? 1u : 0u;
+        }
+      }
+      if (lane == 0) {
+        wave_words[4 * wave] = zero_lo;
+        wave_words[4 * wave + 1] = zero_hi;
+        wave_words[4 * wave + 2] = odd_lo;
+        wave_words[4 * wave + 3] = odd_hi;
+      }
+    }
     wave_stamp(1);
     stamp(3);
     red[0][wave][lane] = sum_cen;
@@ -2315,21 +2519,25 @@
     norm = total * total;
     if (wave == 0 && half == 0 && live && b0 < a.n_draws) {
       if (a.separate) {
-        a.ngal[2 * b0] = n_cen;
-        a.ngal[2 * b0 + 1] = n_sat;
+        a.ngal[2 * b] = n_cen;
+        a.ngal[2 * b + 1] = n_sat;
       } else {
-        a.ngal[b0] = total;
+        a.ngal[b] = total;
       }
     }
   }
 
   set_priority(a.priority & 3);
   const int c = lane & 15, kq = lane >> 4;
+  const int sub = DL == 40 ? 0 : wave / PARTS;
+  const int part = DL == 40 ? wave
+                   : masks && W == 8 && DL == 64 ? ((wave & 3) ^ (wave >> 2))
+                                                 : wave % PARTS;
+  const int sum_slot = DL == 40 ? wave : sub * PARTS + part;
   double F[UP][2][2];
   constexpr int UA = DL == 40 ? (U > 3 ? 3 : U) : 1, UB = DL == 40 && U > 3 ? U - 3 : 1;
   double F40a[UA][10], F40b[UB][10];
   if (DL == 40) {
-    const int part = wave;
     const unsigned off_a = ((lane & 0x30) | ((lane & 3) << 2) | ((lane >> 2) & 3)) * 16;
     const double* dens_b = dens + (a.part_j_row0[part] + (lane >> 4)) * 40 + (lane & 3) * 10;
     const double* dens_e = dens + (a.part_i_row0[part] + (lane >> 4)) * 40 + (lane & 3) * 10;
@@ -2361,7 +2569,6 @@
       fused_quad_pass40<(U > 3 ? 3 : 0), UB>(rs_t, off_a, unit_bytes, dens_b, dens_e, rb, cb,
                                              count, triangular, n_cb, first_unit, F40b);
   } else {
-    const int sub = wave / PARTS, part = wave % PARTS;
     const unsigned off_a = lane * 16;
     const double* dens_b =
         dens + (a.part_j_row0[part] + kq) * DL + sub * kQuadTile + 2 * c;
@@ -2372,10 +2579,38 @@
     const bool triangular = a.part_triangular[part] != 0;
     const int n_cb = a.part_n_cb[part];
     const unsigned unit_base = (unsigned)a.part_unit_base[part];
+    unsigned long long zero_rows = 0, zero_cols = 0;
+    if (masks && ((a.priority >> 11) & 1) &&
+        __builtin_amdgcn_ballot_w64(lane < W && wave_words[4 * (lane < W ? lane : 0) + 2 + sub] != 0) == 0) {
+      auto blocks = [&](int row0) {
+        bool zero = true;
+#pragma unroll
+        for (int v = 0; v < 4; ++v) {
+          const int row = row0 + 4 * lane + v;
+          zero = zero && (row < a.n_bins ? ((wave_words[4 * (row % W) + sub] >> (row / W)) & 1) != 0
+                                         : row < a.dens_rows);
+        }
+        return (unsigned long long)__builtin_amdgcn_ballot_w64(zero);
+      };
+      zero_rows = blocks(a.part_i_row0[part]);
+      zero_cols = a.part_j_row0[part] == a.part_i_row0[part] ? zero_rows
+                                                             : blocks(a.part_j_row0[part]);
+    }
 #pragma unroll
     for (int p = 0; p < UP; ++p) {
       F[p][0][0] = F[p][0][1] = F[p][1][0] = F[p][1][1] = 0.0;
       if (skip & 2) continue;
+      if ((zero_rows | zero_cols) != 0) {
+        if (2 * p + 1 < U)
+          fused_quad_pass_masked<2, DL>(rs_t, off_a + p * 1024, UP * 1024, dens_b, dens_e, rb, cb,
+                                        count, triangular, n_cb, unit_base, zero_rows, zero_cols,
+                                        F[p]);
+        else
+          fused_quad_pass_masked<1, DL>(rs_t, off_a + p * 1024, UP * 1024, dens_b, dens_e, rb, cb,
+                                        count, triangular, n_cb, unit_base, zero_rows, zero_cols,
+                                        F[p]);
+        continue;
+      }
       if (2 * p + 1 < U)
         fused_quad_pass<2, DL>(rs_t, off_a + p * 1024, UP * 1024, dens_b, dens_e, rb, cb, count,
                                triangular, n_cb, unit_base, F[p]);
@@ -2417,7 +2652,7 @@
         }
     }
   } else {
-    double* out = dens + (wave * (4 * U) + kq) * kQuadTile + 2 * c;
+    double* out = dens + (sum_slot * (4 * U) + kq) * kQuadTile + 2 * c;
 #pragma unroll
     for (int u = 0; u < U; ++u) {
       const f64x2 value = {F[u >> 1][u & 1][0], F[u >> 1][u & 1][1]};
@@ -2445,7 +2680,8 @@
       __syncthreads();
       for (int idx = threadIdx.x; idx < a.n_r * DL; idx += blockDim.x) {
         const int dd = idx / a.n_r, rr = idx % a.n_r;
-        if (dd < n_valid) a.xi[((col + dd) * 3 + comp) * (int64_t)a.n_r + rr] = tile[rr][dd];
+        const int64_t row = regroup ? (int64_t)slot_draw[dd] : col + dd;
+        if (dd < n_valid) a.xi[(row * 3 + comp) * (int64_t)a.n_r + rr] = tile[rr][dd];
       }
     }
     return;
@@ -2494,13 +2730,14 @@
     if (wave == 0 && lane < n_valid) {
       double total = 0.0;
       for (int w = 0; w < W; ++w) total += red[0][w][lane];
-      a.chi2[col + lane] = total;
+      a.chi2[b] = total;
     }
     return;
   }
   for (int idx = threadIdx.x; idx < a.n_r * DL; idx += blockDim.x) {
     const int d = idx / a.n_r, rr = idx % a.n_r;
-    if (d < n_valid) a.xi[(col + d) * (int64_t)a.n_r + rr] = tile[rr][d];
+    const int64_t row = regroup ? (int64_t)slot_draw[d] : col + d;
+    if (d < n_valid) a.xi[row * (int64_t)a.n_r + rr] = tile[rr][d];
   }
   stamp(7);
 }
diff --git a/tabcorr_amd/csrc/launch.hip b/tabcorr_amd/csrc/launch.hip
--- a/tabcorr_amd/csrc/launch.hip
+++ b/tabcorr_amd/csrc/launch.hip
@@ -931,6 +931,16 @@
                              t->tuning.deterministic >= 2)) ? 16 : 0;
 }
 
+constexpr int64_t kRegroupMinDraws = 4096;
+static bool fused_regroup(const tc_table* t, int64_t n_draws, int draws, bool grouped,
+                          unsigned flags) {
+  if (t->tuning.fused_regroup == 0 || draws != 64 || grouped || t->theta_in_host) return false;
+  if (flags & TC_FLAG_LEAUTHAUD11) return false;
+  if (t->n_bins - t->plan.n_central > tc::kRegroupMaxTops) return false;
+  if (n_draws > INT32_MAX) return false;
+  return t->tuning.fused_regroup >= 2 || n_draws >= kRegroupMinDraws;
+}
+
 int run_fused(tc_table* t, const double* theta_device, int n_theta, int64_t n_draws,
               int n_gauss, unsigned flags, double* ngal_device, double* xi_device) {
   Range range("occupation + contraction + finalisation (one launch)");
@@ -1061,6 +1071,29 @@
   instance.draws = draws;
   instance.grouped = t->grouped && n_gauss == 10 && !(flags & TC_FLAG_LEAUTHAUD11);
   instance.defer = cen_defer ? 2 : sat_defer ? 1 : 0;
+  if (fused_regroup(t, n_draws, draws, instance.grouped, flags)) {
+    if (t->n_sat_tops < 0) {
+      std::vector<double> tops(t->log_max.begin() + t->plan.n_central, t->log_max.end());
+      std::sort(tops.begin(), tops.end());
+      status = upload(tops, &t->d_sat_tops);
+      if (status != TC_OK) return status;
+      t->n_sat_tops = (int)tops.size();
+    }
+    status = lane.perm.reserve((size_t)n_draws * sizeof(int32_t), stream);
+    if (status != TC_OK) return status;
+    tc::RegroupArgs ra{};
+    ra.theta = theta_device;
+    ra.n_theta = n_theta;
+    ra.log_m0_index = 2;
+    ra.n_draws = n_draws;
+    ra.tops = (const double*)t->d_sat_tops;
+    ra.n_tops = t->n_sat_tops;
+    ra.perm = (int32_t*)lane.perm.ptr;
+    status = launch_regroup_perm(ra, stream);
+    if (status != TC_OK) return status;
+    lane.perm_draws = n_draws;
+    fa.perm = ra.perm;
+  }
   status = launch_fused_instance(instance, t->device, t->quad_tiling.n_u, grid, block, lds, stream,
                                  k0, k1, fa);
   if (status != TC_OK) return status;
diff --git a/tabcorr_amd/csrc/table.cpp b/tabcorr_amd/csrc/table.cpp
--- a/tabcorr_amd/csrc/table.cpp
+++ b/tabcorr_amd/csrc/table.cpp
@@ -207,6 +207,7 @@
   t->resident.ws.buffer.release();
   for (tc_table::Lane& lane : t->lanes)
     if (lane.stream) (void)hipStreamSynchronize(lane.stream);
+  if (t->d_sat_tops != nullptr) (void)hipFree(t->d_sat_tops);
   for (void* p : {t->d_table, t->d_n_h, t->d_percentile, t->d_perm, t->d_math_table,
                   t->d_pos_ij, t->d_pos_off, t->d_group_begin, t->d_group_member,
                   t->d_group_n_h, t->d_group_percentile})
@@ -237,6 +238,7 @@
     lane.in_theta.release();
     lane.out.release();
     lane.cross_counters.release();
+    lane.perm.release();
     if (lane.finished) (void)hipEventDestroy(lane.finished);
   }
   for (tc_table::Ticket& ticket : t->tickets)
@@ -952,12 +954,14 @@
     if (wait_for != nullptr) TC_HIP(hipStreamWaitEvent(lane.stream, wait_for, 0));
     const bool saved_chain = t->chain;
     t->async_lane = lane_index;
+    t->theta_in_host = direct_in;
     t->chain = false;
     status = chi2 ? tc_chi2_zheng07_batch_device(t, d_theta, n_theta, n_draws, n_gauss, flags,
                                                  data, precision, d_ngal, d_second)
                   : tc_predict_zheng07_batch_device(t, d_theta, n_theta, n_draws, n_gauss,
                                                     flags, d_ngal, d_second);
     t->async_lane = -1;
+    t->theta_in_host = false;
     t->chain = saved_chain;
     if (status != TC_OK) return status;
     if (kernels_done != nullptr) TC_HIP(hipEventRecord(kernels_done, lane.stream));
@@ -1311,6 +1315,9 @@
   } else if (key == "fused_defer") {
     TC_CHECK(value >= 0 && value <= 2, "fused_defer must be 0, 1 or 2");
     t->tuning.fused_defer = value;
+  } else if (key == "fused_regroup") {
+    TC_CHECK(value >= 0 && value <= 2, "fused_regroup must be 0, 1 or 2");
+    t->tuning.fused_regroup = value;
   } else if (key == "fused_sat_cap") {
     TC_CHECK(value >= 0 && value <= 6, "fused_sat_cap must be in [0, 6]");
     t->tuning.fused_sat_cap = value;
@@ -1497,6 +1504,19 @@
   return TC_OK;
 }
 
+int tc_debug_regroup_perm(tc_table* t, int lane, int32_t* out, int64_t capacity,
+                          int64_t* n_draws) {
+  TC_CHECK(t != nullptr && n_draws != nullptr, "NULL argument");
+  TC_CHECK(lane >= 0 && lane < (int)tc_table::kMaxLanes, "no such lane");
+  tc_table::Lane& l = t->lanes[lane];
+  *n_draws = l.perm.ptr != nullptr ? l.perm_draws : 0;
+  if (out == nullptr || *n_draws == 0) return TC_OK;
+  if (l.stream) TC_HIP(hipStreamSynchronize(l.stream));
+  const int64_t n = std::min<int64_t>(capacity, *n_draws);
+  TC_HIP(hipMemcpy(out, l.perm.ptr, (size_t)n * sizeof(int32_t), hipMemcpyDeviceToHost));
+  return TC_OK;
+}
+
 int tc_debug_wave_trace(tc_table* t, uint64_t* out, int64_t capacity, int64_t* n_waves) {
   TC_CHECK(t != nullptr && n_waves != nullptr, "NULL argument");
   *n_waves = (int64_t)t->wave_trace_count;
```

New measurement: 201.0 million calls/s. 26.0% lower.
